# TencentARC/BlobCtrl

Measured on AMD Instinct MI355X. Metric: 512x512_50step_blobctrl_edits_per_sec, higher is better.
Workload: dtype fp16

## Files before the change

### blobctrl_amd/_lib.py

```python
import ctypes as C
import os

_HERE = os.path.dirname(os.path.abspath(__file__))
LIB_PATH = os.environ.get("BLOBCTRL_HIP_LIB") or os.path.join(_HERE, "libblobctrl_hip.so")

A_DENSE, A_CONV3X3 = 0, 1
ACT_NONE, ACT_GELU, ACT_GEGLU, ACT_SILU, ACT_QUICK_GELU = 0, 1, 2, 3, 4
OUT_F16, OUT_F16_T, OUT_F32 = 0, 1, 2
TILE_NAMES = ["auto", "256x128", "128x128_s3", "128x128_s2", "256x64_s2", "256x64_s3", "128x64", "64x64", "halo128x160", "wreg128x160",
              "gw64x128", "gw64x256", "gw64x320", "g256x256"]
TILE_HALO = 8
TILE_WREG = 9
TILE_GW64x128, TILE_GW64x256, TILE_GW64x320 = 10, 11, 12
TILE_G256 = 13
GW_TILES = {TILE_GW64x128: 2, TILE_GW64x256: 4, TILE_GW64x320: 5}


class BcGemm(C.Structure):
    _fields_ = [
        ("A", C.c_void_p), ("A2", C.c_void_p), ("a_mode", C.c_int),
        ("M", C.c_int), ("N", C.c_int), ("K", C.c_int),
        ("lda", C.c_int), ("lda2", C.c_int), ("C1", C.c_int), ("Cin", C.c_int),
        ("Hin", C.c_int), ("Win", C.c_int), ("Hv", C.c_int), ("Wv", C.c_int),
        ("Hout", C.c_int), ("Wout", C.c_int), ("stride", C.c_int), ("conv_nopad_lo", C.c_int),
        ("W", C.c_void_p), ("ldw", C.c_int),
        ("bias", C.c_void_p), ("rowvec", C.c_void_p), ("ld_rowvec", C.c_int), ("rows_per_batch", C.c_int),
        ("rowvec_idx", C.c_void_p), ("rowvec_step", C.c_int),
        ("act", C.c_int), ("colscale", C.c_void_p), ("alpha", C.c_float),
        ("alpha_dev", C.c_void_p), ("alpha_idx", C.c_void_p), ("alpha_bstride", C.c_int),
        ("R", C.c_void_p), ("ldr", C.c_int),
        ("R2", C.c_void_p), ("ldr2", C.c_int), ("r2_xmin", C.c_int), ("r2_bmod", C.c_int), ("out_w", C.c_int),
        ("out_mode", C.c_int), ("C", C.c_void_p), ("ldc", C.c_int),
        ("splitk", C.c_int), ("slab", C.c_void_p), ("gn_tot", C.c_void_p), ("tile_cfg", C.c_int),
        ("a_affine", C.c_void_p), ("a_act", C.c_int),
        ("a_tot1", C.c_void_p), ("a_tot2", C.c_void_p),
        ("a_gamma", C.c_void_p), ("a_beta", C.c_void_p), ("a_groups", C.c_int), ("a_eps", C.c_float),
        ("ln_colsum", C.c_void_p), ("ln_eps", C.c_float),
        ("C_t", C.c_void_p), ("ldc_t", C.c_int), ("n_t0", C.c_int),
        ("w_bstride", C.c_longlong), ("vec_bstride", C.c_int), ("sm_group", C.c_int), ("sm_valid", C.c_int), ("sm_keep", C.c_int),
        ("S", C.c_void_p), ("S2", C.c_void_p), ("lds", C.c_int), ("lds2", C.c_int), ("S1", C.c_int), ("Cs", C.c_int),
    ]


_SIGNATURES = {
    "bc_last_error": (C.c_char_p, []),
    "bc_version": (C.c_int, []),
    "bc_device_info": (C.c_int, [C.POINTER(C.c_int)]),
    "bc_gemm": (C.c_int, [C.POINTER(BcGemm), C.c_void_p]),
    "bc_sizeof_gemm": (C.c_int, []),
    "bc_gemm_plan": (C.c_int, [C.c_int, C.c_int, C.c_int, C.c_int, C.POINTER(C.c_int), C.POINTER(C.c_int),
                               C.POINTER(C.c_int), C.POINTER(C.c_int)]),
    "bc_conv_halo_eligible": (C.c_int, [C.c_int] * 8),
    "bc_conv_halo_max_chunks": (C.c_int, []),
    "bc_conv_wreg_pack": (C.c_int, [C.c_void_p, C.c_int, C.c_int, C.c_void_p, C.c_void_p]),
    "bc_conv_wreg_pack_sc": (C.c_int, [C.c_void_p, C.c_int, C.c_int, C.c_void_p, C.c_int, C.c_void_p, C.c_void_p]),
    "bc_conv_wreg_sc_eligible": (C.c_int, [C.c_int] * 7),
    "bc_conv_wreg_pack_host": (C.c_int, [C.c_void_p, C.c_int, C.c_int, C.c_void_p, C.c_int, C.c_void_p]),
    "bc_gemm_wreg_pack": (C.c_int, [C.c_void_p, C.c_int, C.c_int, C.c_int, C.c_int, C.c_void_p, C.c_void_p]),
    "bc_gemm_wreg_stream_elems": (C.c_longlong, [C.c_int, C.c_int]),
    "bc_gemm_wreg_eligible": (C.c_int, [C.c_int] * 5),
    "bc_gemm256_eligible": (C.c_int, [C.c_int] * 7),
    "bc_gn_stats": (C.c_int, [C.c_void_p, C.c_int, C.c_int, C.c_int, C.c_void_p, C.c_void_p]),
    "bc_gn_finalize": (C.c_int, [C.c_void_p, C.c_int, C.c_void_p, C.c_int, C.c_int, C.c_int, C.c_int,
                                 C.c_float, C.c_void_p, C.c_void_p, C.c_void_p, C.c_void_p]),
    "bc_gn_apply_fused": (C.c_int, [C.c_void_p, C.c_int, C.c_void_p, C.c_int, C.c_void_p, C.c_void_p,
                                    C.c_int, C.c_int, C.c_int, C.c_float, C.c_void_p, C.c_void_p, C.c_int, C.c_void_p,
                                    C.c_void_p]),
    "bc_memset_zero": (C.c_int, [C.c_void_p, C.c_longlong, C.c_void_p]),
    "bc_dup_halves": (C.c_int, [C.c_void_p, C.c_longlong] * 6 + [C.c_void_p]),
    "bc_gn_apply": (C.c_int, [C.c_void_p, C.c_int, C.c_void_p, C.c_int, C.c_int, C.c_int, C.c_void_p, C.c_int,
                              C.c_void_p, C.c_void_p]),
    "bc_softmax_rows": (C.c_int, [C.c_void_p, C.c_int, C.c_int, C.c_int, C.c_void_p]),
    "bc_gaussian_sample": (C.c_int, [C.c_void_p, C.c_void_p, C.c_int, C.c_int, C.c_int, C.c_float, C.c_void_p, C.c_void_p]),
    "bc_layernorm": (C.c_int, [C.c_void_p, C.c_int, C.c_int, C.c_int, C.c_void_p, C.c_void_p, C.c_float, C.c_void_p,
                               C.c_int, C.c_void_p]),
    "bc_attention": (C.c_int, [C.c_void_p, C.c_void_p, C.c_void_p, C.c_void_p, C.c_int, C.c_int, C.c_int, C.c_int,
                               C.c_int, C.c_int, C.c_int, C.c_int, C.c_int, C.c_longlong, C.c_longlong, C.c_longlong,
                               C.c_longlong, C.c_float, C.c_void_p]),
    "bc_attention_causal": (C.c_int, [C.c_void_p, C.c_void_p, C.c_void_p, C.c_void_p, C.c_int, C.c_int, C.c_int, C.c_int,
                                      C.c_int, C.c_int, C.c_int, C.c_int, C.c_int, C.c_longlong, C.c_longlong, C.c_longlong,
                                      C.c_longlong, C.c_float, C.c_void_p]),
    "bc_embed_tokens": (C.c_int, [C.c_void_p, C.c_void_p, C.c_void_p, C.c_int, C.c_int, C.c_int, C.c_int, C.c_void_p,
                                  C.c_void_p]),
    "bc_splat_scores": (C.c_int, [C.POINTER(C.c_double), C.c_int, C.c_int, C.c_int, C.c_void_p, C.c_void_p]),
    "bc_splat_maps": (C.c_int, [C.POINTER(C.c_double), C.c_int, C.c_int, C.c_int, C.c_void_p, C.c_void_p, C.c_void_p]),
    "bc_alpha_composite": (C.c_int, [C.c_void_p, C.c_longlong, C.c_int, C.c_void_p, C.c_void_p]),
    "bc_splat_from_scores": (C.c_int, [C.c_void_p, C.c_void_p, C.c_int, C.c_int, C.c_int, C.c_int, C.c_int, C.c_longlong, C.c_longlong,
                                       C.c_longlong, C.c_longlong, C.c_int, C.c_int, C.c_int, C.c_void_p, C.c_void_p]),
    "bc_resize_bilinear": (C.c_int, [C.c_void_p, C.c_longlong, C.c_int, C.c_int, C.c_int, C.c_int, C.c_int, C.c_void_p, C.c_void_p]),
    "bc_pack_rgb8": (C.c_int, [C.c_void_p, C.c_int, C.c_int, C.c_void_p, C.c_void_p]),
    "bc_assemble_input": (C.c_int, [C.c_void_p, C.c_int, C.c_void_p, C.c_void_p, C.c_void_p, C.c_int, C.c_int, C.c_int,
                                    C.c_int, C.c_int, C.c_int, C.c_int, C.c_void_p, C.c_void_p]),
    "bc_assemble_input_im2col": (C.c_int, [C.c_void_p, C.c_int, C.c_void_p, C.c_void_p, C.c_int, C.c_int, C.c_int, C.c_int, C.c_int,
                                           C.c_void_p, C.c_void_p]),
    "bc_timestep_embedding": (C.c_int, [C.c_void_p, C.c_void_p, C.c_float, C.c_int, C.c_int, C.c_void_p, C.c_void_p]),
    "bc_timestep_embedding_table": (C.c_int, [C.c_void_p, C.c_int, C.c_int, C.c_int, C.c_void_p, C.c_void_p]),
    "bc_silu": (C.c_int, [C.c_void_p, C.c_void_p, C.c_longlong, C.c_void_p]),
    "bc_cfg_scheduler_step": (C.c_int, [C.c_void_p, C.c_void_p, C.c_void_p, C.c_void_p, C.c_void_p, C.c_float, C.c_int,
                                        C.c_int, C.c_int, C.c_void_p, C.c_int, C.c_void_p]),
    "bc_cfg_scheduler_step_noise": (C.c_int, [C.c_void_p, C.c_void_p, C.c_void_p, C.c_void_p, C.c_void_p, C.c_float, C.c_int,
                                              C.c_int, C.c_int, C.c_void_p, C.c_int, C.c_void_p, C.c_int, C.c_void_p]),
    "bc_cfg_scheduler_step3": (C.c_int, [C.c_void_p, C.c_void_p, C.c_void_p, C.c_void_p, C.c_void_p, C.c_float, C.c_int, C.c_int,
                                         C.c_int, C.c_int, C.c_void_p, C.c_int, C.c_void_p]),
    "bc_nchw_to_nhwc_f16": (C.c_int, [C.c_void_p, C.c_int, C.c_int, C.c_int, C.c_int, C.c_int, C.c_void_p, C.c_void_p]),
    "bc_nhwc_to_nchw": (C.c_int, [C.c_void_p, C.c_int, C.c_int, C.c_int, C.c_int, C.c_void_p, C.c_int, C.c_void_p]),
    "bc_add_cls_pos": (C.c_int, [C.c_void_p, C.c_void_p, C.c_void_p, C.c_int, C.c_int, C.c_int, C.c_void_p, C.c_void_p]),
    "bc_patchify": (C.c_int, [C.c_void_p, C.c_int, C.c_int, C.c_int, C.c_int, C.c_int, C.c_void_p, C.c_void_p]),
    "bc_rowchain_supported": (C.c_int, [C.c_int, C.c_int, C.c_int]),
    "bc_rowchain_stream_frags": (C.c_longlong, [C.c_int, C.c_int, C.c_int, C.c_int]),
    "bc_rowchain": (C.c_int, [C.c_int, C.c_int, C.c_int, C.c_int, C.c_void_p, C.c_void_p, C.c_void_p, C.c_void_p, C.c_void_p, C.c_int, C.c_float,
                              C.c_void_p, C.c_void_p, C.c_void_p, C.c_int, C.c_int,
                              C.c_int, C.c_void_p, C.c_void_p, C.c_void_p, C.c_void_p, C.c_void_p, C.c_int, C.c_void_p, C.c_float,
                              C.c_float, C.c_void_p, C.c_void_p, C.c_int, C.c_void_p, C.c_int, C.c_void_p]),
    "bc_rowchain_sum": (C.c_int, [C.c_int, C.c_int, C.c_int, C.c_void_p, C.c_int, C.c_void_p, C.c_void_p, C.c_void_p, C.c_void_p]),
    "bc_rowchain_kv_frags": (C.c_longlong, [C.c_int]),
    "bc_rowchain_pack_kv": (C.c_int, [C.c_void_p, C.c_int, C.c_void_p, C.c_int, C.c_int, C.c_int, C.c_int, C.c_void_p, C.c_void_p]),
    "bc_ctx_fold": (C.c_int, [C.c_void_p, C.c_int, C.c_void_p, C.c_int, C.c_int, C.c_int, C.c_int, C.c_int, C.c_float, C.c_void_p, C.c_void_p,
                              C.c_void_p, C.c_void_p, C.c_void_p, C.c_void_p, C.c_void_p, C.c_void_p]),
    "bc_rowchain_midx": (C.c_int, [C.c_int, C.c_int, C.c_int, C.c_void_p, C.c_void_p, C.c_void_p, C.c_void_p, C.c_void_p, C.c_int, C.c_float,
                                   C.c_void_p, C.c_void_p, C.c_float, C.c_void_p]),
    "bc_plan_create": (C.c_int, [C.POINTER(C.c_void_p)]),
    "bc_plan_destroy": (C.c_int, [C.c_void_p]),
    "bc_plan_segment": (C.c_int, [C.c_void_p, C.c_char_p]),
    "bc_plan_find_segment": (C.c_int, [C.c_void_p, C.c_char_p]),
    "bc_plan_new_event": (C.c_int, [C.c_void_p]),
    "bc_plan_add_gemm": (C.c_int, [C.c_void_p, C.c_int, C.c_int, C.POINTER(BcGemm)]),
    "bc_plan_add_op": (C.c_int, [C.c_void_p, C.c_int, C.c_int, C.c_int, C.POINTER(C.c_uint64), C.c_int]),
    "bc_plan_set_slab": (C.c_int, [C.c_void_p, C.c_int, C.c_void_p]),
    "bc_plan_enable": (C.c_int, [C.c_void_p, C.c_int, C.c_int, C.c_int]),
    "bc_plan_num_launches": (C.c_int, [C.c_void_p, C.c_int]),
    "bc_step": (C.c_int, [C.c_void_p, C.c_int, C.POINTER(C.c_void_p), C.c_int]),
    "bc_plan_capture": (C.c_int, [C.c_void_p, C.c_int, C.POINTER(C.c_void_p), C.c_int]),
    "bc_plan_release": (C.c_int, [C.c_void_p, C.c_int]),
    "bc_plan_capture_loop": (C.c_int, [C.c_void_p, C.POINTER(C.c_int), C.c_int, C.POINTER(C.c_void_p), C.c_int, C.POINTER(C.c_void_p)]),
    "bc_plan_run_timed": (C.c_int, [C.c_void_p, C.c_int, C.c_void_p, C.POINTER(C.c_float)]),
    "bc_plan_run_timed_kernels": (C.c_int, [C.c_void_p, C.c_int, C.c_void_p, C.POINTER(C.c_float), C.POINTER(C.c_float)]),
    "bc_plan_run_marked": (C.c_int, [C.c_void_p, C.c_int, C.POINTER(C.c_void_p), C.c_int, C.POINTER(C.c_int), C.c_int, C.POINTER(C.c_float)]),
    "bc_plan_save": (C.c_int, [C.c_void_p, C.c_char_p, C.c_void_p, C.c_int]),
    "bc_plan_load": (C.c_int, [C.c_char_p, C.POINTER(C.c_void_p)]),
    "bc_plan_buffer": (C.c_int, [C.c_void_p, C.c_char_p, C.POINTER(C.c_void_p), C.POINTER(C.c_longlong)]),
    "bc_graph_begin": (C.c_int, [C.c_void_p]),
    "bc_graph_end": (C.c_int, [C.c_void_p, C.POINTER(C.c_void_p)]),
    "bc_graph_launch": (C.c_int, [C.c_void_p, C.c_void_p]),
    "bc_graph_destroy": (C.c_int, [C.c_void_p]),
    "bc_event_create": (C.c_int, [C.POINTER(C.c_void_p)]),
    "bc_event_create_sync": (C.c_int, [C.POINTER(C.c_void_p)]),
    "bc_stream_wait_event": (C.c_int, [C.c_void_p, C.c_void_p]),
    "bc_event_record": (C.c_int, [C.c_void_p, C.c_void_p]),
    "bc_event_elapsed_ms": (C.c_int, [C.c_void_p, C.c_void_p, C.POINTER(C.c_float)]),
    "bc_event_destroy": (C.c_int, [C.c_void_p]),
}

EXPORTED_SYMBOLS = tuple(_SIGNATURES.keys())

OPS = {"bc_gemm": 0, "bc_gn_stats": 1, "bc_gn_finalize": 2, "bc_gn_apply_fused": 3, "bc_gn_apply": 4, "bc_layernorm": 5,
       "bc_attention": 6, "bc_attention_causal": 7, "bc_assemble_input": 8, "bc_timestep_embedding": 9,
       "bc_timestep_embedding_table": 10, "bc_cfg_scheduler_step": 11, "bc_embed_tokens": 12, "bc_softmax_rows": 13,
       "bc_patchify": 14, "bc_add_cls_pos": 15, "bc_silu": 16, "bc_nchw_to_nhwc_f16": 17, "bc_nhwc_to_nchw": 18,
       "bc_gaussian_sample": 19, "bc_rowchain": 22, "bc_assemble_input_im2col": 23, "bc_memset_zero": 24,
       "bc_rowchain_midx": 25, "bc_rowchain_pack_kv": 26, "bc_rowchain_sum": 27, "bc_ctx_fold": 28, "bc_dup_halves": 29,
       "bc_cfg_scheduler_step_noise": 30, "bc_cfg_scheduler_step3": 31}
OP_SIGNAL, OP_WAIT = 20, 21
CHAIN_IN, CHAIN_MID, CHAIN_OUT, CHAIN_OUT_FF, CHAIN_OUT_TAIL, CHAIN_MIDX, CHAIN_OUT_FFP = 0, 1, 2, 3, 4, 5, 6
GN_TOT_WORDS = 6
_KIND = {C.c_void_p: "p", C.c_int: "i", C.c_float: "f", C.c_longlong: "l", C.c_char_p: "p"}


def op_signature(name):
    args = _SIGNATURES[name][1][:-1]
    return "".join("p" if (a not in _KIND) else _KIND[a] for a in args)


class BcPlanBuffer(C.Structure):
    _fields_ = [("name", C.c_char_p), ("address", C.c_void_p), ("bytes", C.c_longlong), ("host_data", C.c_void_p)]

_lib = None


class BlobCtrlHipError(RuntimeError):
    pass


def load():
    global _lib
    if _lib is not None:
        return _lib
    if not os.path.exists(LIB_PATH):
        raise BlobCtrlHipError(
            f"{LIB_PATH} not found: build it with `python -c 'import __graft_entry__ as g; g.build()'` "
            "(hipcc --offload-arch=gfx950).  blobctrl_amd has no CPU fallback.")
    try:
        import torch
    except ImportError:
        pass
    try:
        lib = C.CDLL(LIB_PATH)
    except OSError as e:
        raise BlobCtrlHipError(f"failed to load {LIB_PATH}: {e}") from e
    for name, (res, args) in _SIGNATURES.items():
        fn = getattr(lib, name)
        fn.restype = res
        fn.argtypes = args
    if lib.bc_sizeof_gemm() != C.sizeof(BcGemm):
        raise BlobCtrlHipError(f"BcGemm layout mismatch: C {lib.bc_sizeof_gemm()} vs ctypes {C.sizeof(BcGemm)}")
    _lib = lib
    return lib


def check(rc, what=""):
    if rc != 0:
        msg = load().bc_last_error()
        raise BlobCtrlHipError(f"{what} failed (rc={rc}): {msg.decode() if msg else ''}")
```

### blobctrl_amd/csrc/conv_wreg.hip

```cpp
#include <stdio.h>
#include <stdlib.h>
#include <algorithm>
#include <type_traits>
#include <vector>
#include "gemm_common.h"

using namespace bcg;

namespace {

__device__ __attribute__((aligned(16))) unsigned int g_zero_line_w[4] = {0u, 0u, 0u, 0u};

typedef const __attribute__((address_space(1))) void* gptr_t;
typedef __attribute__((address_space(3))) void* lptr_t;

__device__ __forceinline__ void glds16(const void* src, char* lds_dst) {
    __builtin_amdgcn_global_load_lds((gptr_t)src, (lptr_t)lds_dst, 16, 0, 0);
}

constexpr int TW = 16, TH = 8;
constexpr int HBM = TW * TH;
constexpr int HBN = 160;
constexpr int HSTR = TW + 2;
constexpr int HPIX = (TH + 2) * HSTR;
constexpr int HALO_BYTES = 24 * 1024;
constexpr int NBUF = 3;
constexpr int OFF_AB = NBUF * HALO_BYTES;
constexpr int MAX_CH = 40;
constexpr int TS = HBN + 4;
constexpr int LDS_LOOP = OFF_AB + MAX_CH * 512;
constexpr int LDS_EPI = 8 * 16384;
constexpr int OFF_EPI = LDS_LOOP > LDS_EPI ? LDS_LOOP : LDS_EPI;
constexpr int LDS_TOTAL = OFF_EPI + 2 * HBN * 4;
static_assert(LDS_TOTAL <= 160 * 1024 && HPIX * 128 <= HALO_BYTES && HBM * TS * 4 <= LDS_EPI, "LDS budget");
constexpr int FIN_MAX_CH = 2752;
constexpr int OFF_FIN = LDS_LOOP;
constexpr int LDS_TOTAL_FIN = OFF_FIN + FIN_MAX_CH * 16 + 1024 > LDS_TOTAL ? OFF_FIN + FIN_MAX_CH * 16 + 1024 : LDS_TOTAL;
static_assert(LDS_TOTAL_FIN <= 160 * 1024, "LDS budget (in-kernel finalize)");

template <int N>
__device__ __forceinline__ void wait_vm_c() { asm volatile("s_waitcnt vmcnt(%0)" ::"n"(N) : "memory"); }
typedef float f32x4v __attribute__((ext_vector_type(4)));
typedef unsigned int u32x4v __attribute__((ext_vector_type(4)));

template <int V> using IC = std::integral_constant<int, V>;

template <int AFFINE>
__global__ __launch_bounds__(512) void conv_wreg_kernel(const GemmArgs g) {
    extern __shared__ __attribute__((aligned(16))) char smem[];
    const BcGemm& p = g.p;
    const int tid = threadIdx.x;
    const int lane = tid & 63;
    const int wave = __builtin_amdgcn_readfirstlane(tid >> 6);
    const int kg = wave & 1;
    const int grp = ((wave >> 1) & 1) | ((wave >> 2) << 1);
    const bool three = grp == 0 || grp == 3;
    const int tile0 = grp == 0 ? 0 : grp == 1 ? 3 : grp == 2 ? 5 : 7;

    asm volatile("" ::"s"(p.A), "s"(p.A2), "s"(p.W), "s"(p.Hv), "s"(p.Wv), "s"(p.Hin), "s"(p.Win), "s"(p.lda), "s"(p.lda2), "s"(p.C1), "s"(p.Cin),
                 "s"(p.splitk), "s"(p.a_act), "s"(g.halo_tpi), "s"(g.halo_tx), "s"(g.halo_nch), "s"(g.halo_nsc), "s"(g.halo_cps), "s"(g.halo_cps_sc), "s"(g.nband), "s"(g.halo_stamps));
    asm volatile("" ::"s"(g.wr_plane.mul), "s"(g.wr_plane.shift), "s"(g.wr_plane.d), "s"(g.wr_gx.mul), "s"(g.wr_gx.shift), "s"(g.wr_gx.d), "s"(g.wr_gy.mul),
                 "s"(g.wr_gy.shift), "s"(g.wr_gy.d), "s"(g.wr_tpi.mul), "s"(g.wr_tpi.shift), "s"(g.wr_tx.mul), "s"(g.wr_tx.shift), "s"(p.bias), "s"(p.rowvec),
                 "s"(p.rowvec_idx), "s"(p.rowvec_step), "s"(p.ld_rowvec), "s"(g.halo_dbg), "s"(g.div_rpb.d));
    if (AFFINE == 2)
        asm volatile("" ::"s"(p.a_tot1), "s"(p.a_tot2), "s"(p.a_gamma), "s"(p.a_beta), "s"(p.a_groups), "s"(p.a_eps), "s"(g.wr_cpg.mul), "s"(g.wr_cpg.shift));
    const int plane = (int)g.wr_plane.d;
    const int lin3 = bc_xcd_remap(blockIdx.x + gridDim.x * (blockIdx.y + gridDim.y * blockIdx.z), plane * gridDim.z);
    const int split = (int)fdiv((unsigned)lin3, g.wr_plane);
    const int lin = lin3 - split * plane;
    const int q_gx = (int)fdiv((unsigned)lin, g.wr_gx), q_gy = (int)fdiv((unsigned)lin, g.wr_gy);
    const int tile = g.nband ? lin - q_gy * (int)g.wr_gy.d : q_gx;
    const int ntile = g.nband ? q_gy : lin - q_gx * (int)g.wr_gx.d;
    const int n0 = ntile * HBN;
    const int b = (int)fdiv((unsigned)tile, g.wr_tpi);
    const int tin = tile - b * g.halo_tpi;
    const int ty_ = (int)fdiv((unsigned)tin, g.wr_tx);
    const int ty0 = ty_ * TH, tx0 = (tin - ty_ * g.halo_tx) * TW;
    const int H = p.Hv, W = p.Wv;
    const bool ups2 = p.Hv != p.Hin;
    const int c_lo = split * g.halo_cps;
    const int n9 = max(0, min(g.halo_nch, c_lo + g.halo_cps) - c_lo);
    const int sc_begin = split * g.halo_cps_sc;
    const int nsc = max(0, min(g.halo_nsc, sc_begin + g.halo_cps_sc) - sc_begin);
    const bool dummy = n9 == 0;
    const int c_begin = dummy ? 0 : c_lo;
    const int nch = dummy ? 1 : n9;
    const long long tsl = (long long)(9 * g.halo_nch + g.halo_nsc) * 512;

    unsigned long long* const stamps = g.halo_stamps;
    auto stamp = [&](int i) {
        if (stamps && lane == 0 && (wave == 0 || wave == 2))
            stamps[((size_t)(blockIdx.x + gridDim.x * (blockIdx.y + gridDim.y * blockIdx.z)) * 2 + (wave >> 1)) * 16 + i] = __builtin_amdgcn_s_memtime();
    };
    stamp(0);

    const h16* __restrict__ A1 = reinterpret_cast<const h16*>(p.A);
    const h16* __restrict__ A2 = reinterpret_cast<const h16*>(p.A2);
    const h16* zero = reinterpret_cast<const h16*>(g_zero_line_w);

    const int sidx = ((wave >= 2 ? wave - 2 : 0) << 6) | lane;
    int pixv[6], csubv[6];
#pragma unroll
    for (int q = 0; q < 6; ++q) {
        const int hp = (sidx >> 3) + 32 * q;
        const int hy = hp / HSTR, hx = hp - hy * HSTR;
        const int gy = ty0 + hy - 1, gx = tx0 + hx - 1;
        const bool inh = hp < HPIX;
        const bool in_img = inh && (unsigned)gy < (unsigned)H && (unsigned)gx < (unsigned)W;
        pixv[q] = !in_img ? -1 : ups2 ? (b * p.Hin + (gy >> 1)) * p.Win + (gx >> 1) : (b * H + gy) * W + gx;
        csubv[q] = (sidx & 7) ^ (((hx >> 1) & 3) << 1);
    }
    auto issue_a = [&](int cl, int buf, bool valid) {
        const int k0 = (c_begin + cl) * 64;
        const bool second = A2 != nullptr && k0 >= p.C1;
        const h16* src = second ? A2 : A1;
        const int stride = second ? p.lda2 : p.lda;
        const int kin = second ? k0 - p.C1 : k0;
        char* dst = smem + buf * HALO_BYTES + (wave - 2) * 1024;
#pragma unroll
        for (int q = 0; q < 6; ++q) {
            const int off = pixv[q] * stride + kin + csubv[q] * 8;
            const h16* s = (valid && !dummy && pixv[q] >= 0) ? src + off : zero;
            glds16(s, dst + q * 4096);
        }
    };
    const unsigned lds0 = (unsigned)(size_t)(lptr_t)(smem);
    const unsigned slot_addr = lds0 + sidx * 16;
    const unsigned ab_base = lds0 + OFF_AB;
    struct Pending { u32x4v raw; f32x4v t0, t1, t2, t3; };
    auto tr_issue = [&](unsigned sa, unsigned ab_addr, Pending& pd) {
        asm volatile("ds_read_b128 %0, %1" : "=v"(pd.raw) : "v"(sa) : "memory");
        asm volatile("ds_read_b128 %0, %4\n\tds_read_b128 %1, %4 offset:16\n\tds_read_b128 %2, %4 offset:32\n\t"
                     "ds_read_b128 %3, %4 offset:48"
                     : "=&v"(pd.t0), "=&v"(pd.t1), "=&v"(pd.t2), "=&v"(pd.t3) : "v"(ab_addr) : "memory");
    };
    auto tr_finish = [&](unsigned sa, bool outside, bool store, Pending& pd) {
        asm volatile("s_waitcnt lgkmcnt(0)" : "+v"(pd.raw), "+v"(pd.t0), "+v"(pd.t1), "+v"(pd.t2), "+v"(pd.t3)::"memory");
        __builtin_amdgcn_sched_barrier(0);
        const float aa[8] = {pd.t0[0], pd.t0[2], pd.t1[0], pd.t1[2], pd.t2[0], pd.t2[2], pd.t3[0], pd.t3[2]};
        const float bb[8] = {pd.t0[1], pd.t0[3], pd.t1[1], pd.t1[3], pd.t2[1], pd.t2[3], pd.t3[1], pd.t3[3]};
        const u32x4v rawv = pd.raw;
        const h16* xin = reinterpret_cast<const h16*>(&rawv);
        u32x4v outraw;
        h16* o = reinterpret_cast<h16*>(&outraw);
#pragma unroll
        for (int j = 0; j < 8; ++j) {
            float v = fmaf((float)xin[j], aa[j], bb[j]);
            if (p.a_act == BC_ACT_SILU) v = v * __builtin_amdgcn_rcpf(1.0f + __builtin_amdgcn_exp2f(-1.4426950408889634f * v));
            o[j] = (h16)v;
        }
        if (outside || dummy) outraw = (u32x4v){0u, 0u, 0u, 0u};
        if (store) asm volatile("ds_write_b128 %0, %1" ::"v"(sa), "v"(outraw) : "memory");
    };
    unsigned tinfo = 0;
#pragma unroll
    for (int q = 0; q < 3; ++q) {
        const int hp = (tid >> 3) + 64 * q;
        const int hy = hp / HSTR, hx = hp - hy * HSTR;
        const int gy = ty0 + hy - 1, gx = tx0 + hx - 1;
        const unsigned inh = hp < HPIX, outside = !((unsigned)gy < (unsigned)H && (unsigned)gx < (unsigned)W);
        tinfo |= (inh | outside << 1 | (unsigned)((tid & 7) ^ (((hx >> 1) & 3) << 1)) << 2) << (8 * q);
    }
    const unsigned tslot = lds0 + tid * 16;
    auto transform_pair = [&](auto kxc, int cl, int buf) {
        constexpr int q0 = 2 * decltype(kxc)::value;
        Pending pa, pb;
        const unsigned sa = slot_addr + buf * HALO_BYTES + 4096 * q0, ab = ab_base + cl * 512;
        const bool in0 = (sidx >> 3) + 32 * q0 < HPIX, in1 = (sidx >> 3) + 32 * (q0 + 1) < HPIX;
        tr_issue(sa, ab + csubv[q0] * 64, pa);
        tr_issue(sa + 4096, ab + csubv[q0 + 1] * 64, pb);
        tr_finish(sa, pixv[q0] < 0, in0, pa);
        tr_finish(sa + 4096, pixv[q0 + 1] < 0, in1, pb);
        asm volatile("s_waitcnt lgkmcnt(0)" ::: "memory");
    };
    auto transform_first = [&]() {
        Pending pd[3];
#pragma unroll
        for (int q = 0; q < 3; ++q) tr_issue(tslot + 8192 * q, ab_base + ((tinfo >> (8 * q + 2)) & 7) * 64, pd[q]);
#pragma unroll
        for (int q = 0; q < 3; ++q) tr_finish(tslot + 8192 * q, (tinfo >> (8 * q + 1)) & 1, (tinfo >> (8 * q)) & 1, pd[q]);
        asm volatile("s_waitcnt lgkmcnt(0)" ::: "memory");
    };

    float* tilef = reinterpret_cast<float*>(smem);
    auto body = [&](auto ntc, auto stgc) {
        constexpr int NT = decltype(ntc)::value;
        constexpr bool STG = decltype(stgc)::value != 0;
        constexpr int G = 3 * NT;
        const long long per_chunk = 9 * 512;
        u32x4v ring[3 * G];
        const unsigned lane16 = lane * 16;
#define BC_WREG_LOAD_GROUP(GX, BASE)                                                                                                  \
    _Pragma("unroll") for (int f = 0; f < G; ++f) {                                                                                   \
        const h16* b4 = (BASE) + (((GX) * G + f) & ~3) * 512;                                                                          \
        asm volatile("global_load_dwordx4 %0, %1, %2 offset:%3" : "=v"(ring[(GX) * G + f]) : "v"(lane16), "s"(b4), "n"((((GX) * G + f) & 3) * 1024) : "memory"); \
    }
        const h16* const wstream = reinterpret_cast<const h16*>(p.W) + ((long long)ntile * 20 + 2 * tile0 + kg * NT) * tsl;
        const h16* wb = wstream + (long long)c_begin * NT * per_chunk;
        constexpr int FIN_T = 4;
        const int fin_cpg = AFFINE == 2 ? p.Cin / p.a_groups : 1;
        const int fin_k_lo = c_begin * 64, fin_k_hi = fin_k_lo + nch * 64;
        const int fin_g_lo = (int)fdiv((unsigned)fin_k_lo, g.wr_cpg), fin_g_hi = AFFINE == 2 ? min(p.a_groups, (int)fdiv((unsigned)(fin_k_hi + fin_cpg - 1), g.wr_cpg)) : 1;
        const int fin_c_lo = fin_g_lo * fin_cpg, fin_nc = fin_g_hi * fin_cpg - fin_c_lo;
        const bool fin_fast = AFFINE == 2 && fin_nc <= 256 * FIN_T && !(g.halo_dbg & 0x100);
        const int ft = ((wave < 2 ? wave : wave - 4) << 6) | lane;
        u32x4v fq[FIN_T][3];
        float fg[FIN_T], fb[FIN_T];
        if (AFFINE == 2 && !STG && fin_fast) {
            unsigned long long tp1 = (unsigned long long)p.a_tot1, tp2 = (unsigned long long)(p.A2 ? p.a_tot2 : p.a_tot1);
            asm volatile("" : "+s"(tp1), "+s"(tp2));
            const int C1s = p.A2 ? p.C1 : p.Cin, C2s = p.Cin - C1s;
#pragma unroll
            for (int j = 0; j < FIN_T; ++j) {
                const int cc = ft + 256 * j;
                const int c = fin_c_lo + (cc < fin_nc ? cc : 0);
                const bool second = c >= C1s;
                const unsigned long long ta = (second ? tp2 : tp1) + ((unsigned long long)((long long)b * (second ? C2s : C1s) + (second ? c - C1s : c))) * (BC_GN_TOT_WORDS * 8);
                const unsigned long long* t = reinterpret_cast<const unsigned long long*>(ta);
                asm volatile("global_load_dwordx4 %0, %3, off\n\tglobal_load_dwordx4 %1, %3, off offset:16\n\tglobal_load_dwordx4 %2, %3, off offset:32"
                             : "=&v"(fq[j][0]), "=&v"(fq[j][1]), "=&v"(fq[j][2]) : "v"(t) : "memory");
                const int i = ft + 256 * j;
                const int ci = fin_k_lo + (i < nch * 64 ? i : 0);
                asm volatile("global_load_dword %0, %2, off\n\tglobal_load_dword %1, %3, off" : "=&v"(fg[j]), "=&v"(fb[j]) : "v"(p.a_gamma + ci), "v"(p.a_beta + ci) : "memory");
            }
        }
        stamp(8);
        if (STG) {
            issue_a(0, 0, true);
            issue_a(1, 1, nch > 1);
        }
        BC_WREG_LOAD_GROUP(0, wb)
        stamp(9);
        if (AFFINE == 2 && fin_fast && !STG) {
#define BC_FIN_TIE(j) "+v"(fq[j][0]), "+v"(fq[j][1]), "+v"(fq[j][2])
            asm volatile("s_waitcnt vmcnt(%12)" : BC_FIN_TIE(0), BC_FIN_TIE(1), BC_FIN_TIE(2), BC_FIN_TIE(3) : "n"(G) : "memory");
            asm volatile("s_waitcnt vmcnt(%8)" : "+v"(fg[0]), "+v"(fg[1]), "+v"(fg[2]), "+v"(fg[3]), "+v"(fb[0]), "+v"(fb[1]), "+v"(fb[2]), "+v"(fb[3])
                         : "n"(G) : "memory");
#undef BC_FIN_TIE
        }
        stamp(10);
        unsigned rv_idx = 0;
        if (p.rowvec && p.rowvec_idx) asm volatile("s_load_dword %0, %1, 0x0\n\ts_waitcnt lgkmcnt(0)" : "=s"(rv_idx) : "s"(p.rowvec_idx) : "memory");
        const bool eok = p.splitk == 1 && tid < HBN;
        const float* epi_bp = (eok && p.bias) ? p.bias + n0 + tid : reinterpret_cast<const float*>(g_zero_line_w);
        const h16* epi_rp = (eok && p.rowvec) ? reinterpret_cast<const h16*>(p.rowvec) + (size_t)rv_idx * p.rowvec_step + (size_t)b * p.ld_rowvec + n0 + tid : zero;
        const float epi_bv = *epi_bp;
        const unsigned short epi_rraw = *reinterpret_cast<const unsigned short*>(epi_rp);
        if (AFFINE == 2 && fin_fast) {
            double* scr = reinterpret_cast<double*>(smem + OFF_FIN);
            float* stat = reinterpret_cast<float*>(scr + fin_nc * 2);
            if (!STG) {
#pragma unroll
                for (int j = 0; j < FIN_T; ++j) {
                    const int cc = ft + 256 * j;
                    if (cc < fin_nc) {
                        double s_, q_;
                        auto w64 = [](unsigned lo, unsigned hi) { return (unsigned long long)lo | ((unsigned long long)hi << 32); };
                        bc_gn_tot_decode(w64(fq[j][0][0], fq[j][0][1]), w64(fq[j][0][2], fq[j][0][3]), w64(fq[j][1][0], fq[j][1][1]),
                                         w64(fq[j][1][2], fq[j][1][3]), w64(fq[j][2][0], fq[j][2][1]), w64(fq[j][2][2], fq[j][2][3]), s_, q_);
                        scr[cc * 2] = s_;
                        scr[cc * 2 + 1] = q_;
                    }
                }
            }
            asm volatile("s_waitcnt lgkmcnt(0)" ::: "memory");
            __builtin_amdgcn_s_barrier();
            asm volatile("" ::: "memory");
            stamp(11);
            if (!STG) {
                const int sub = ft & 7;
                for (int gi = fin_g_lo + (ft >> 3); gi < fin_g_hi; gi += 32) {
                    double s_ = 0.0, q_ = 0.0;
                    for (int cj = sub; cj < fin_cpg; cj += 8) {
                        s_ += scr[((gi - fin_g_lo) * fin_cpg + cj) * 2];
                        q_ += scr[((gi - fin_g_lo) * fin_cpg + cj) * 2 + 1];
                    }
#pragma unroll
                    for (int o = 4; o > 0; o >>= 1) {
                        s_ += __shfl_xor(s_, o);
                        q_ += __shfl_xor(q_, o);
                    }
                    const double n = (double)g.div_rpb.d * fin_cpg;
                    const double mean = s_ / n;
                    double var = q_ / n - mean * mean;
                    if (var < 0.0) var = 0.0;
                    if (sub == 0) {
                        stat[(gi - fin_g_lo) * 2] = (float)mean;
                        stat[(gi - fin_g_lo) * 2 + 1] = (float)(1.0 / sqrt(var + (double)p.a_eps));
                    }
                }
            }
            asm volatile("s_waitcnt lgkmcnt(0)" ::: "memory");
            __builtin_amdgcn_s_barrier();
            asm volatile("" ::: "memory");
            stamp(12);
            if (!STG) {
                float* abt = reinterpret_cast<float*>(smem + OFF_AB);
#pragma unroll
                for (int j = 0; j < FIN_T; ++j) {
                    const int i = ft + 256 * j;
                    if (i < nch * 64) {
                        const int gi = (int)fdiv((unsigned)(fin_k_lo + i), g.wr_cpg) - fin_g_lo;
                        const float a = stat[gi * 2 + 1] * fg[j];
                        abt[i * 2] = a;
                        abt[i * 2 + 1] = fb[j] - stat[gi * 2] * a;
                    }
                }
            }
            stamp(13);
        } else if (AFFINE == 2) {
            const int cpg = p.Cin / p.a_groups;
            const int k_lo = c_begin * 64, k_hi = k_lo + nch * 64;
            const int g_lo = k_lo / cpg, g_hi = min(p.a_groups, (k_hi + cpg - 1) / cpg);
            const int c_lo = g_lo * cpg, nc = g_hi * cpg - c_lo;
            float gpre[2] = {0.f, 0.f}, bpre[2] = {0.f, 0.f};
#pragma unroll
            for (int j = 0; j < 2; ++j)
                if (tid + 512 * j < nch * 64) {
                    gpre[j] = p.a_gamma[k_lo + tid + 512 * j];
                    bpre[j] = p.a_beta[k_lo + tid + 512 * j];
                }
            double* scr = reinterpret_cast<double*>(smem + OFF_FIN);
            for (int cc = tid; cc < nc; cc += 512) {
                const int c = c_lo + cc;
                const bool second = p.A2 != nullptr && c >= p.C1;
                const int Cs = second ? p.Cin - p.C1 : (p.A2 ? p.C1 : p.Cin);
                const unsigned long long* t = (second ? p.a_tot2 : p.a_tot1) + ((size_t)b * Cs + (second ? c - p.C1 : c)) * BC_GN_TOT_WORDS;
                double s, q;
                bc_gn_tot_read(t, s, q);
                scr[cc * 2] = s;
                scr[cc * 2 + 1] = q;
            }
            __syncthreads();
            float* stat = reinterpret_cast<float*>(scr + nc * 2);
            {
                const int sub = tid & 7;
                for (int gi = g_lo + (tid >> 3); gi < g_hi; gi += 64) {
                    double s = 0.0, q = 0.0;
                    for (int cj = sub; cj < cpg; cj += 8) {
                        s += scr[((gi - g_lo) * cpg + cj) * 2];
                        q += scr[((gi - g_lo) * cpg + cj) * 2 + 1];
                    }
#pragma unroll
                    for (int o = 4; o > 0; o >>= 1) {
                        s += __shfl_xor(s, o);
                        q += __shfl_xor(q, o);
                    }
                    const double n = (double)g.div_rpb.d * cpg;
                    const double mean = s / n;
                    double var = q / n - mean * mean;
                    if (var < 0.0) var = 0.0;
                    if (sub == 0) {
                        stat[(gi - g_lo) * 2] = (float)mean;
                        stat[(gi - g_lo) * 2 + 1] = (float)(1.0 / sqrt(var + (double)p.a_eps));
                    }
                }
            }
            __syncthreads();
            float* abt = reinterpret_cast<float*>(smem + OFF_AB);
#pragma unroll
            for (int j = 0; j < 2; ++j) {
                const int i = tid + 512 * j;
                if (i < nch * 64) {
                    const int gi = (k_lo + i) / cpg - g_lo;
                    const float a = stat[gi * 2 + 1] * gpre[j];
                    abt[i * 2] = a;
                    abt[i * 2 + 1] = bpre[j] - stat[gi * 2] * a;
                }
            }
            for (int i = tid + 1024; i < nch * 64; i += 512) {
                const int c = k_lo + i;
                const int gi = c / cpg - g_lo;
                const float a = stat[gi * 2 + 1] * p.a_gamma[c];
                abt[i * 2] = a;
                abt[i * 2 + 1] = p.a_beta[c] - stat[gi * 2] * a;
            }
            __syncthreads();
        }
        if (AFFINE == 1) {
            const float4* src = reinterpret_cast<const float4*>(p.a_affine + ((size_t)b * p.Cin + (size_t)c_begin * 64) * 2);
            float4* dst = reinterpret_cast<float4*>(smem + OFF_AB);
            for (int i = tid; i < nch * 32; i += 512) dst[i] = src[i];
        }
        BC_WREG_LOAD_GROUP(1, wb)
        BC_WREG_LOAD_GROUP(2, wb)
        stamp(1);
        asm volatile("s_waitcnt vmcnt(%0)" ::"n"(2 * G) : "memory");
        asm volatile("s_waitcnt lgkmcnt(0)" ::: "memory");
        __builtin_amdgcn_s_barrier();
        asm volatile("" ::: "memory");
        stamp(6);
        if (AFFINE) transform_first();
        if (eok) {
            float* ev = reinterpret_cast<float*>(smem + OFF_EPI);
            ev[tid] = epi_bv;
            ev[HBN + tid] = (float)__builtin_bit_cast(h16, epi_rraw);
        }
        stamp(7);
        asm volatile("s_waitcnt lgkmcnt(0)" ::: "memory");
        __builtin_amdgcn_s_barrier();
        asm volatile("" ::: "memory");
        stamp(2);

        int a_off[3];
#pragma unroll
        for (int kx = 0; kx < 3; ++kx) {
            const int hx = (lane & 15) + kx;
            const int ch = 4 * kg + (lane >> 4);
            a_off[kx] = hx * 128 + ((ch ^ (((hx >> 1) & 3) << 1)) << 4);
        }
        f32x4v acc[8][NT];
#pragma unroll
        for (int i = 0; i < 8; ++i)
#pragma unroll
            for (int t = 0; t < NT; ++t) acc[i][t] = (f32x4v){0.f, 0.f, 0.f, 0.f};

#ifndef BC_WREG_PRIO
#define BC_WREG_PRIO 1
#endif
        if ((BC_WREG_PRIO == 1 && STG) || (BC_WREG_PRIO == 2 && !STG)) __builtin_amdgcn_s_setprio(3);
        int buf = 0;
        int cl = 0;
#pragma unroll
        for (int pass = 0; pass < 2; ++pass) {
        const bool more = pass == 0;
        const int cl_end = more ? nch - 1 : nch;
        for (; cl < cl_end; ++cl) {
            const int buf1 = buf + 1 == NBUF ? 0 : buf + 1;
            const int buf2 = buf1 + 1 == NBUF ? 0 : buf1 + 1;
            if (STG) issue_a(cl + 2, buf2, cl + 2 < nch);
            wb += 3 * G * 512;
#pragma unroll
            for (int kx = 0; kx < 3; ++kx) {
#define BC_WREG_WAIT(N)                                                                                                                 \
    if (NT == 3) asm volatile("s_waitcnt vmcnt(%9)" : "+v"(ring[kx * G]), "+v"(ring[kx * G + 1]), "+v"(ring[kx * G + 2]), "+v"(ring[kx * G + 3]), \
                              "+v"(ring[kx * G + 4]), "+v"(ring[kx * G + 5]), "+v"(ring[kx * G + 6]), "+v"(ring[kx * G + 7]),             \
                              "+v"(ring[kx * G + G - 1]) : "n"(N) : "memory");                                                          \
    else asm volatile("s_waitcnt vmcnt(%6)" : "+v"(ring[kx * G]), "+v"(ring[kx * G + 1]), "+v"(ring[kx * G + 2]), "+v"(ring[kx * G + 3]),       \
                      "+v"(ring[kx * G + 4]), "+v"(ring[kx * G + G - 1]) : "n"(N) : "memory");
                constexpr int D = STG ? 6 : 0;
                if (more || kx == 0) { BC_WREG_WAIT(2 * G + D) }
                else if (kx == 1) { BC_WREG_WAIT(G + D) }
                else { BC_WREG_WAIT(D) }
                const unsigned abase = lds0 + buf * HALO_BYTES + a_off[kx];
                u32x4v a[3];
                asm volatile("ds_read_b128 %0, %1" : "=v"(a[0]) : "v"(abase) : "memory");
                asm volatile("ds_read_b128 %0, %1 offset:%2" : "=v"(a[1]) : "v"(abase), "n"(HSTR * 128) : "memory");
#pragma unroll
                for (int r = 0; r < 10; ++r) {
                    if (r + 2 < 10) {
                        asm volatile("ds_read_b128 %0, %1 offset:%2" : "=v"(a[(r + 2) % 3]) : "v"(abase), "n"((r + 2) * HSTR * 128) : "memory");
                        asm volatile("s_waitcnt lgkmcnt(2)" : "+v"(a[r % 3])::"memory");
                    } else if (r + 1 < 10) {
                        asm volatile("s_waitcnt lgkmcnt(1)" : "+v"(a[r % 3])::"memory");
                    } else {
                        asm volatile("s_waitcnt lgkmcnt(0)" : "+v"(a[r % 3])::"memory");
                    }
                    __builtin_amdgcn_sched_barrier(0);
                    const h16x8 af = __builtin_bit_cast(h16x8, a[r % 3]);
#pragma unroll
                    for (int ky = 0; ky < 3; ++ky) {
                        const int i = r - ky;
                        if (i < 0 || i >= 8) continue;
#pragma unroll
                        for (int t = 0; t < NT; ++t)
                            acc[i][t] = __builtin_amdgcn_mfma_f32_16x16x32_f16(__builtin_bit_cast(h16x8, ring[(kx * 3 + ky) * NT + t]), af, acc[i][t], 0, 0, 0);
                    }
                    __builtin_amdgcn_sched_barrier(0);
                }
                if (STG && AFFINE && more) {
                    if (kx == 0) transform_pair(IC<0>{}, cl + 1, buf1);
                    else if (kx == 1) transform_pair(IC<1>{}, cl + 1, buf1);
                    else transform_pair(IC<2>{}, cl + 1, buf1);
                }
                if (more) { BC_WREG_LOAD_GROUP(kx, wb) }
                __builtin_amdgcn_sched_barrier(0);
            }
            if (STG) {
                if (more) wait_vm_c<3 * G>();
                else wait_vm_c<0>();
            }
            asm volatile("s_waitcnt lgkmcnt(0)" ::: "memory");
            __builtin_amdgcn_s_barrier();
            asm volatile("" ::: "memory");
            buf = buf1;
        }
        }

        stamp(14);
        if (nsc > 0) {
            constexpr int U = 4, NB2 = 5, D1 = STG ? 6 : 0;
            static_assert(NB2 * HALO_BYTES <= LDS_EPI && U < NB2 && U * 3 + 6 * U < 64, "shortcut phase: images below the epilogue vectors, vmcnt range");
            const h16* __restrict__ S1p = reinterpret_cast<const h16*>(p.S);
            const h16* __restrict__ S2p = reinterpret_cast<const h16*>(p.S2);
            const h16* const ws = wstream + ((long long)g.halo_nch * 9 + sc_begin) * NT * 512;
            u32x4v sr[U * NT];
            auto issue_s = [&](int sx, int bufi) {
                const int k0 = (sc_begin + sx) * 64;
                const bool second = S2p != nullptr && k0 >= p.S1;
                const h16* src = second ? S2p : S1p;
                const int stride = second ? p.lds2 : p.lds;
                const int kin = second ? k0 - p.S1 : k0;
                char* dst = smem + bufi * HALO_BYTES + (wave - 2) * 1024;
#pragma unroll
                for (int q = 0; q < 6; ++q) {
                    const int off = pixv[q] * stride + kin + csubv[q] * 8;
                    const h16* s_ = (sx < nsc && pixv[q] >= 0) ? src + off : zero;
                    glds16(s_, dst + q * 4096);
                }
            };
#define BC_WREG_LOAD_SC(J, SX)                                                                                                          \
    {                                                                                                                                   \
        const h16* b4 = ws + (long long)min((SX), nsc - 1) * (NT * 512);                                                                \
        _Pragma("unroll") for (int t = 0; t < NT; ++t)                                                                                  \
            asm volatile("global_load_dwordx4 %0, %1, %2 offset:%3" : "=v"(sr[(J) * NT + t]) : "v"(lane16), "s"(b4), "n"((t % NT) * 1024) : "memory"); \
    }
#pragma unroll
            for (int j = 0; j < U; ++j) {
                if (STG) issue_s(j, j);
                BC_WREG_LOAD_SC(j, j)
            }
            if (STG) wait_vm_c<U * NT + 6 * (U - 1)>();
            asm volatile("s_waitcnt lgkmcnt(0)" ::: "memory");
            __builtin_amdgcn_s_barrier();
            asm volatile("" ::: "memory");
            int sbuf = 0;
            for (int s0 = 0; s0 < nsc; s0 += U) {
#pragma unroll
                for (int j = 0; j < U; ++j) {
                    const int sx = s0 + j;
                    const int bufn = sbuf + U >= NB2 ? sbuf + U - NB2 : sbuf + U;
                    if (STG) issue_s(sx + U, bufn);
                    if (NT == 3) asm volatile("s_waitcnt vmcnt(%3)" : "+v"(sr[j * NT]), "+v"(sr[j * NT + 1]), "+v"(sr[j * NT + NT - 1]) : "n"((U - 1) * NT + U * D1) : "memory");
                    else asm volatile("s_waitcnt vmcnt(%2)" : "+v"(sr[j * NT]), "+v"(sr[j * NT + 1]) : "n"((U - 1) * NT + U * D1) : "memory");
                    const unsigned abase = lds0 + sbuf * HALO_BYTES + a_off[1];
                    u32x4v a8[8];
#pragma unroll
                    for (int i = 0; i < 8; ++i)
                        asm volatile("ds_read_b128 %0, %1 offset:%2" : "=v"(a8[i]) : "v"(abase), "n"((i + 1) * HSTR * 128) : "memory");
#pragma unroll
                    for (int i = 0; i < 8; ++i) {
                        asm volatile("s_waitcnt lgkmcnt(%1)" : "+v"(a8[i]) : "n"(7 - i) : "memory");
                        __builtin_amdgcn_sched_barrier(0);
                        const h16x8 af = __builtin_bit_cast(h16x8, a8[i]);
#pragma unroll
                        for (int t = 0; t < NT; ++t)
                            acc[i][t] = __builtin_amdgcn_mfma_f32_16x16x32_f16(__builtin_bit_cast(h16x8, sr[j * NT + t]), af, acc[i][t], 0, 0, 0);
                        __builtin_amdgcn_sched_barrier(0);
                    }
                    BC_WREG_LOAD_SC(j, sx + U)
                    if (STG) wait_vm_c<U * NT + 6 * (U - 1)>();
                    asm volatile("s_waitcnt lgkmcnt(0)" ::: "memory");
                    __builtin_amdgcn_s_barrier();
                    asm volatile("" ::: "memory");
                    sbuf = sbuf + 1 == NB2 ? 0 : sbuf + 1;
                }
            }
#pragma unroll
            for (int j = 0; j < U; ++j) {
                if (NT == 3) asm volatile("s_waitcnt vmcnt(0)" : "+v"(sr[j * NT]), "+v"(sr[j * NT + 1]), "+v"(sr[j * NT + NT - 1]) :: "memory");
                else asm volatile("s_waitcnt vmcnt(0)" : "+v"(sr[j * NT]), "+v"(sr[j * NT + 1]) :: "memory");
            }
            __builtin_amdgcn_s_barrier();
            asm volatile("" ::: "memory");
#undef BC_WREG_LOAD_SC
        }
        __builtin_amdgcn_s_setprio(0);
        stamp(3);
        char* xch = smem + tile0 * 8192;
        const int i_keep = kg * 4, i_send = 4 - i_keep;
#pragma unroll
        for (int ii = 0; ii < 4; ++ii)
#pragma unroll
            for (int t = 0; t < NT; ++t)
                *reinterpret_cast<f32x4v*>(xch + (((i_send + ii) * NT + t) * 64 + lane) * 16) = kg ? acc[ii][t] : acc[4 + ii][t];
        __syncthreads();
        f32x4v fin[4][NT];
#pragma unroll
        for (int ii = 0; ii < 4; ++ii)
#pragma unroll
            for (int t = 0; t < NT; ++t) {
                const f32x4v o = *reinterpret_cast<const f32x4v*>(xch + (((i_keep + ii) * NT + t) * 64 + lane) * 16);
                fin[ii][t] = (kg ? acc[4 + ii][t] : acc[ii][t]) + o;
            }
        __syncthreads();
        if (p.splitk > 1) {
#pragma unroll
            for (int ii = 0; ii < 4; ++ii)
#pragma unroll
                for (int t = 0; t < NT; ++t)
                    *reinterpret_cast<f32x4v*>(tilef + ((i_keep + ii) * 16 + (lane & 15)) * TS + tile0 * 16 + t * 16 + 4 * (lane >> 4)) = fin[ii][t];
            __syncthreads();
            return;
        }
        constexpr int RPP = NT == 3 ? 8 : 16, NP = 64 / RPP;
        char* const sl = smem + wave * 16384;
#pragma unroll
        for (int ii = 0; ii < 4; ++ii)
#pragma unroll
            for (int t = 0; t < NT; ++t) {
                const int row = ii * 16 + (lane & 15), ck = t * 4 + (lane >> 4);
                *reinterpret_cast<f32x4v*>(sl + row * 256 + ((ck ^ (row & 15)) << 4)) = fin[ii][t];
            }
        int cpos, rsub;
        bool lane_on = true;
        if (NT == 3) {
            cpos = lane & 7;
            rsub = lane >> 3;
            lane_on = cpos < 6;
            if (!lane_on) cpos = 5;
        } else {
            const int sub = (lane >> 2) & 3;
            cpos = lane & 3;
            rsub = 2 * (lane >> 4) + (sub & 1) + 8 * (sub >> 1);
        }
        const int ch0 = tile0 * 16 + cpos * 8, n_first = n0 + ch0;
        const int rpb = (int)g.div_rpb.d;
        const float alpha = scalar_alpha(p);
        const float* ev = reinterpret_cast<const float*>(smem + OFF_EPI) + ch0;
        float bias_v[8], rvec[8], cs[8];
#pragma unroll
        for (int j = 0; j < 8; ++j) {
            bias_v[j] = ev[j];
            rvec[j] = ev[HBN + j];
            cs[j] = (p.colscale ? p.colscale[n_first + j] : 1.0f) * alpha;
        }
        const float ab = p.alpha_bstride > 0 ? batch_alpha(g, b) : 1.0f;
        float gs[8], gq[8];
#pragma unroll
        for (int j = 0; j < 8; ++j) { gs[j] = 0.f; gq[j] = 0.f; }
        auto passes = [&](auto H2K, auto HRK) {
            constexpr bool H2 = decltype(H2K)::value, HR = decltype(HRK)::value;
            uint4 rr[NP];
            int mrow[NP];
#pragma unroll
            for (int j = 0; j < NP; ++j) {
                const int row = j * RPP + rsub;
                mrow[j] = b * rpb + (ty0 + i_keep + (row >> 4)) * W + tx0 + (row & 15);
                if (HR) rr[j] = bc_ld16(reinterpret_cast<const h16*>(p.R) + (size_t)mrow[j] * p.ldr + n_first);
            }
            if (!H2) __builtin_amdgcn_sched_barrier(0);
#pragma unroll H2 ? 1 : NP
            for (int j = 0; j < NP; ++j) {
                const int row = j * RPP + rsub;
                const f32x4v lo = *reinterpret_cast<const f32x4v*>(sl + row * 256 + (((2 * cpos) ^ (row & 15)) << 4));
                const f32x4v hi = *reinterpret_cast<const f32x4v*>(sl + row * 256 + (((2 * cpos + 1) ^ (row & 15)) << 4));
                float v[8] = {lo[0], lo[1], lo[2], lo[3], hi[0], hi[1], hi[2], hi[3]};
#pragma unroll
                for (int q = 0; q < 8; ++q) v[q] += bias_v[q];
                if (p.rowvec) {
#pragma unroll
                    for (int q = 0; q < 8; ++q) v[q] += rvec[q];
                }
                if (H2) {
                    if (p.act == BC_ACT_GELU) {
#pragma unroll
                        for (int q = 0; q < 8; ++q) v[q] = bc_gelu_f(v[q]);
                    } else if (p.act == BC_ACT_SILU) {
#pragma unroll
                        for (int q = 0; q < 8; ++q) v[q] = bc_silu_f(v[q]);
                    } else if (p.act == BC_ACT_QUICK_GELU) {
#pragma unroll
                        for (int q = 0; q < 8; ++q) v[q] = bc_quick_gelu_f(v[q]);
                    }
                }
#pragma unroll
                for (int q = 0; q < 8; ++q) v[q] *= cs[q];
                if (p.alpha_bstride > 0) {
#pragma unroll
                    for (int q = 0; q < 8; ++q) v[q] *= ab;
                }
                if (HR) {
                    const h16* rh = reinterpret_cast<const h16*>(&rr[j]);
#pragma unroll
                    for (int q = 0; q < 8; ++q) v[q] += (float)rh[q];
                }
                if (H2 && p.R) {
                    const uint4 r1 = bc_ld16(reinterpret_cast<const h16*>(p.R) + (size_t)mrow[j] * p.ldr + n_first);
                    const h16* rh = reinterpret_cast<const h16*>(&r1);
#pragma unroll
                    for (int q = 0; q < 8; ++q) v[q] += (float)rh[q];
                }
                if (H2 && p.R2) {
                    const int pix = mrow[j] - b * rpb;
                    const int x = pix - (int)fdiv((unsigned)pix, g.div_outw) * (int)g.div_outw.d;
                    if (x >= p.r2_xmin) {
                        const uint4 r2 = bc_ld16(reinterpret_cast<const h16*>(p.R2) + ((size_t)(b % p.r2_bmod) * rpb + pix) * p.ldr2 + n_first);
                        const h16* rh = reinterpret_cast<const h16*>(&r2);
#pragma unroll
                        for (int q = 0; q < 8; ++q) v[q] += (float)rh[q];
                    }
                }
                uint4 outraw;
                h16* o = reinterpret_cast<h16*>(&outraw);
#pragma unroll
                for (int q = 0; q < 8; ++q) {
                    o[q] = (h16)v[q];
                    const float f = lane_on ? (float)o[q] : 0.f;
                    gs[q] += f;
                    gq[q] += f * f;
                }
                bc_st16(reinterpret_cast<h16*>(p.C) + (size_t)mrow[j] * p.ldc + n_first, outraw);
            }
        };
        if (p.R2 || p.act != BC_ACT_NONE) passes(std::true_type{}, std::false_type{});
        else if (p.R) passes(std::false_type{}, std::true_type{});
        else passes(std::false_type{}, std::false_type{});
        if (p.gn_tot) {
            constexpr int X0 = NT == 3 ? 8 : 4, X1 = 2 * X0, X2 = 4 * X0;
            const bool b0 = lane & X0, b1 = lane & X1, b2 = lane & X2;
            auto scatter = [&](const float (&v)[8]) __attribute__((always_inline)) {
                float k4[4], k2[2];
#pragma unroll
                for (int k = 0; k < 4; ++k) k4[k] = (b0 ? v[4 + k] : v[k]) + __shfl_xor(b0 ? v[k] : v[4 + k], X0);
#pragma unroll
                for (int k = 0; k < 2; ++k) k2[k] = (b1 ? k4[2 + k] : k4[k]) + __shfl_xor(b1 ? k4[k] : k4[2 + k], X1);
                float t = (b2 ? k2[1] : k2[0]) + __shfl_xor(b2 ? k2[0] : k2[1], X2);
                if (NT == 2) t += __shfl_xor(t, 32);
                return t;
            };
            const float s_own = scatter(gs), q2_own = scatter(gq);
            const int q_own = (b0 ? 4 : 0) + (b1 ? 2 : 0) + (b2 ? 1 : 0);
            const bool owner = NT == 3 ? lane_on : lane < 32;
            float* sc = reinterpret_cast<float*>(smem + wave * 16384);
            if (owner) {
                sc[(cpos * 8 + q_own) * 2] = s_own;
                sc[(cpos * 8 + q_own) * 2 + 1] = q2_own;
            }
            __syncthreads();
            if (kg == 0 && owner) {
                const float* sp = reinterpret_cast<const float*>(smem + (wave | 1) * 16384);
                const int n_lo = n0 + tile0 * 16;
                bc_gn_tot_add_slot(p.gn_tot + (size_t)b * g.n_out * BC_GN_TOT_WORDS, n_first + q_own, n_lo, n_lo + NT * 16, bc_gn_cg(g.n_out), tin, [&](int k) {
                    const int c = k - n_lo;
                    return make_float2(sc[c * 2] + sp[c * 2], sc[c * 2 + 1] + sp[c * 2 + 1]);
                });
            }
        }
    };
    if (three) body(IC<3>{}, IC<0>{});
    else body(IC<2>{}, IC<1>{});
    stamp(4);
    if (p.splitk > 1) {
        const int col8 = tid % 20, row0 = tid / 20;
        const int rpb = (int)g.div_rpb.d;
        if (tid < 480) {
            float* slab = p.slab + (size_t)split * p.M * p.N;
            for (int row = row0; row < HBM; row += 24) {
                const int m = b * rpb + (ty0 + (row >> 4)) * W + tx0 + (row & 15);
                const float4 lo = *reinterpret_cast<const float4*>(tilef + row * TS + col8 * 8);
                const float4 hi = *reinterpret_cast<const float4*>(tilef + row * TS + col8 * 8 + 4);
                float* dst = slab + (size_t)m * p.N + n0 + col8 * 8;
                *reinterpret_cast<float4*>(dst) = lo;
                *reinterpret_cast<float4*>(dst + 4) = hi;
            }
        }
    }
    stamp(5);
}

__host__ __device__ inline long long conv_wreg_pack_src(long long idx, int Cin, int Cs, bool& sc) {
    const int nchunks = Cin / 64;
    const long long per_tile_stream = (long long)(nchunks * 9 + Cs / 64) * 64;
    const long long per_ntile = 20 * per_tile_stream;
    const int ntile = (int)(idx / per_ntile);
    long long rem = idx - (long long)ntile * per_ntile;
    const int ts = (int)(rem / per_tile_stream);
    int tile0, NT;
    if (ts < 6) { tile0 = 0; NT = 3; }
    else if (ts < 10) { tile0 = 3; NT = 2; }
    else if (ts < 14) { tile0 = 5; NT = 2; }
    else { tile0 = 7; NT = 3; }
    const long long in_grp = rem - (long long)2 * tile0 * per_tile_stream;
    const long long per_wave = per_tile_stream * NT;
    const int kg = (int)(in_grp / per_wave);
    long long s = in_grp - (long long)kg * per_wave;
    const int lane = (int)(s & 63);
    s >>= 6;
    sc = s >= (long long)nchunks * 9 * NT;
    if (sc) {
        s -= (long long)nchunks * 9 * NT;
        const int t = (int)(s % NT), chunk = (int)(s / NT);
        const int n = ntile * HBN + (tile0 + t) * 16 + (lane & 15);
        return (long long)n * Cs + chunk * 64 + kg * 32 + 8 * (lane >> 4);
    }
    const int t = (int)(s % NT);
    s /= NT;
    const int ky = (int)(s % 3);
    s /= 3;
    const int kx = (int)(s % 3);
    const int chunk = (int)(s / 3);
    const int n = ntile * HBN + (tile0 + t) * 16 + (lane & 15);
    const long long k = (long long)(ky * 3 + kx) * Cin + chunk * 64 + kg * 32 + 8 * (lane >> 4);
    return (long long)n * 9 * Cin + k;
}

__global__ void conv_wreg_pack_kernel(const h16* __restrict__ w, int N, int Cin, const h16* __restrict__ wsc, int Cs, h16* __restrict__ out) {
    const long long total = (long long)N * (9 * Cin + Cs) / 8;
    const long long idx = (long long)blockIdx.x * blockDim.x + threadIdx.x;
    if (idx >= total) return;
    bool sc;
    const long long src = conv_wreg_pack_src(idx, Cin, Cs, sc);
    *reinterpret_cast<uint4*>(out + idx * 8) = *reinterpret_cast<const uint4*>((sc ? wsc : w) + src);
}

}

extern "C" int bc_conv_wreg_pack_sc(const bc_half* w, int N, int Cin, const bc_half* wsc, int Cs, bc_half* out, bc_stream stream_) {
    hipStream_t stream = reinterpret_cast<hipStream_t>(stream_);
    BC_CHECK_ARG(w && out && N > 0 && N % HBN == 0 && Cin > 0 && Cin % 64 == 0, "bc_conv_wreg_pack: N %% 160 == 0 and Cin %% 64 == 0 (N=%d Cin=%d)", N, Cin);
    BC_CHECK_ARG((wsc == nullptr) == (Cs == 0) && Cs >= 0 && Cs % 64 == 0, "bc_conv_wreg_pack: shortcut weight and Cs %% 64 == 0 go together (Cs=%d)", Cs);
    BC_CHECK_ARG(((uintptr_t)w % 16 == 0) && ((uintptr_t)wsc % 16 == 0) && ((uintptr_t)out % 16 == 0) && w != out && wsc != out,
                 "bc_conv_wreg_pack: 16-byte aligned, out of place");
    const long long total = (long long)N * (9 * Cin + Cs) / 8;
    hipLaunchKernelGGL(conv_wreg_pack_kernel, dim3((unsigned)((total + 255) / 256)), dim3(256), 0, stream, reinterpret_cast<const h16*>(w), N, Cin,
                       reinterpret_cast<const h16*>(wsc), Cs, reinterpret_cast<h16*>(out));
    BC_CHECK_LAUNCH();
    return 0;
}

extern "C" int bc_conv_wreg_pack_host(const bc_half* w, int N, int Cin, const bc_half* wsc, int Cs, bc_half* out) {
    BC_CHECK_ARG(w && out && N > 0 && N % HBN == 0 && Cin > 0 && Cin % 64 == 0, "bc_conv_wreg_pack: N %% 160 == 0 and Cin %% 64 == 0 (N=%d Cin=%d)", N, Cin);
    BC_CHECK_ARG((wsc == nullptr) == (Cs == 0) && Cs >= 0 && Cs % 64 == 0, "bc_conv_wreg_pack: shortcut weight and Cs %% 64 == 0 go together (Cs=%d)", Cs);
    const long long total = (long long)N * (9 * Cin + Cs) / 8;
    const unsigned short* w_ = reinterpret_cast<const unsigned short*>(w);
    const unsigned short* s_ = reinterpret_cast<const unsigned short*>(wsc);
    unsigned short* o_ = reinterpret_cast<unsigned short*>(out);
    for (long long idx = 0; idx < total; ++idx) {
        bool sc;
        const long long src = conv_wreg_pack_src(idx, Cin, Cs, sc);
        std::copy_n((sc ? s_ : w_) + src, 8, o_ + idx * 8);
    }
    return 0;
}

extern "C" int bc_conv_wreg_pack(const bc_half* w, int N, int Cin, bc_half* out, bc_stream stream) {
    return bc_conv_wreg_pack_sc(w, N, Cin, nullptr, 0, out, stream);
}

int bc_conv_wreg_sc_ok(const BcGemm& p) {
    if (!p.S || p.R || p.Cs <= 0 || p.Cs % 64 != 0 || p.Hv != p.Hin || p.Wv != p.Win) return 0;
    if (p.S2 && (p.S1 <= 0 || p.S1 >= p.Cs || p.S1 % 64 != 0)) return 0;
    if (p.lds < (p.S2 ? p.S1 : p.Cs) || p.lds % 8 != 0 || (uintptr_t)p.S % 16 != 0) return 0;
    if (p.S2 && (p.lds2 < p.Cs - p.S1 || p.lds2 % 8 != 0 || (uintptr_t)p.S2 % 16 != 0)) return 0;
    return 1;
}

int bc_conv_wreg_launch(GemmArgs& g, hipStream_t stream) {
    BcGemm& p = g.p;
    g.halo_tx = p.Wout / TW;
    g.halo_tpi = g.halo_tx * (p.Hout / TH);
    g.halo_nch = p.Cin / 64;
    g.halo_nsc = p.S ? p.Cs / 64 : 0;
    g.halo_dbg = 0;
    g.halo_stamps = nullptr;
    int sk = std::max(1, std::min(p.splitk, g.halo_nch + g.halo_nsc));
    g.halo_cps = bc_ceil_div(g.halo_nch, sk);
    g.halo_cps_sc = bc_ceil_div(g.halo_nsc, sk);
    p.splitk = std::max(bc_ceil_div(g.halo_nch, g.halo_cps), g.halo_nsc ? bc_ceil_div(g.halo_nsc, g.halo_cps_sc) : 1);
    BC_CHECK_ARG(g.halo_cps <= MAX_CH, "bc_gemm(wreg conv): %d channel chunks per split exceed %d (raise splitk)", g.halo_cps, MAX_CH);
    BC_CHECK_ARG(p.splitk == 1 || p.slab != nullptr, "bc_gemm(wreg conv): splitk=%d needs a slab", p.splitk);
    const int B = p.M / (p.Hout * p.Wout);
    BC_CHECK_ARG((long long)p.M * std::max(p.lda, p.lda2) < 2147483647LL, "bc_gemm(wreg conv): activation of %d pixels x stride %d exceeds 32-bit element offsets",
                 p.M, std::max(p.lda, p.lda2));
    BC_CHECK_ARG(!p.S || (bc_conv_wreg_sc_ok(p) && (long long)p.M * std::max(p.lds, p.lds2) < 2147483647LL),
                 "bc_gemm(wreg conv): folded shortcut outside the kernel's limits (Cs=%d S1=%d)", p.Cs, p.S1);
    dim3 grid(p.N / HBN, B * g.halo_tpi, p.splitk);
    g.wr_plane = make_fastdiv(grid.x * grid.y);
    g.wr_gx = make_fastdiv(grid.x);
    g.wr_gy = make_fastdiv(grid.y);
    g.wr_tpi = make_fastdiv((unsigned)g.halo_tpi);
    g.wr_tx = make_fastdiv((unsigned)g.halo_tx);
    g.wr_cpg = make_fastdiv((unsigned)(p.a_tot1 && p.a_groups > 0 ? p.Cin / p.a_groups : 1));
    {
        g.nband = (double)p.N * 9 > (double)p.M && grid.x >= 4;
    }
    static const bool want_stamps = getenv("BC_WREG_STAMPS") != nullptr;
    static unsigned long long* stamp_buf = nullptr;
    const size_t nwg_s = (size_t)grid.x * grid.y * grid.z;
    if (want_stamps && nwg_s <= 4096) {
        if (!stamp_buf) BC_CHECK_HIP(hipMalloc(reinterpret_cast<void**>(&stamp_buf), 4096 * 32 * sizeof(unsigned long long)));
        BC_CHECK_HIP(hipMemsetAsync(stamp_buf, 0, nwg_s * 32 * sizeof(unsigned long long), stream));
        g.halo_stamps = stamp_buf;
    }
    struct StampReport {
        hipStream_t stream; size_t n; unsigned long long* buf; const BcGemm& p; int cps;
        ~StampReport() {
            if (!buf) return;
            if (hipStreamSynchronize(stream) != hipSuccess) return;
            std::vector<unsigned long long> h(n * 32);
            if (hipMemcpy(h.data(), buf, n * 32 * sizeof(unsigned long long), hipMemcpyDeviceToHost) != hipSuccess) return;
            for (int w = 0; w < 2; ++w) {
                double d[5] = {0, 0, 0, 0, 0};
                for (size_t i = 0; i < n; ++i)
                    for (int k = 0; k < 5; ++k) d[k] += (double)(h[(i * 2 + w) * 16 + k + 1] - h[(i * 2 + w) * 16 + k]);
                double e[3] = {0, 0, 0};
                for (size_t i = 0; i < n; ++i) {
                    const unsigned long long* q = &h[(i * 2 + w) * 16];
                    e[0] += (double)(q[6] - q[1]);
                    e[1] += (double)(q[7] - q[6]);
                    e[2] += (double)(q[2] - q[7]);
                }
                double pr[6] = {0, 0, 0, 0, 0, 0};
                for (size_t i = 0; i < n; ++i)
                    for (int k = 0; k < 6; ++k) {
                        const unsigned long long* q = &h[(i * 2 + w) * 16];
                        if (q[8 + k]) pr[k] += (double)(q[8 + k] - q[0]);
                    }
                fprintf(stderr, "[wreg stamps] prologue detail (ticks since entry): inputs requested %.0f, ring group 0 requested %.0f, totals landed %.0f, "
                        "barrier 1 %.0f, barrier 2 %.0f, table written %.0f\n", pr[0] / n, pr[1] / n, pr[2] / n, pr[3] / n, pr[4] / n, pr[5] / n);
                double scp = 0;
                for (size_t i = 0; i < n; ++i) scp += (double)(h[(i * 2 + w) * 16 + 3] - h[(i * 2 + w) * 16 + 14]);
                if (p.S) fprintf(stderr, "[wreg stamps] folded shortcut: Cs=%d, %.0f ticks per workgroup behind the nine-tap chunks (of the loop's %.0f)\n", p.Cs, scp / n, d[2] / n);
                fprintf(stderr, "[wreg stamps] M=%d N=%d Cin=%d sk=%d cps=%d wgs=%zu %s | avg ticks: setup+table %.0f, first halo %.0f (landing %.0f, pass %.0f, "
                        "next DMA + barrier %.0f), loop %.0f (%.0f per tap), k-half sum %.0f, stores %.0f\n", p.M, p.N, p.Cin, p.splitk, cps, n,
                        w ? "staging wave " : "3-tile wave  ", d[0] / n, d[1] / n, e[0] / n, e[1] / n, e[2] / n, d[2] / n, d[2] / n / (cps * 9), d[3] / n, d[4] / n);
            }
        }
    } report{stream, nwg_s, g.halo_stamps, p, g.halo_cps};
    static std::atomic<unsigned long long> set_a{0}, set_p{0}, set_f{0};
    if (p.a_tot1) {
        BC_CHECK_ARG(p.a_gamma && p.a_beta && p.a_groups > 0 && p.Cin % p.a_groups == 0 && (!p.A2 || p.a_tot2),
                     "bc_gemm(wreg conv): in-kernel GroupNorm finalize needs a_gamma, a_beta, a_groups | Cin and the partials of every source");
        const int cpg = p.Cin / p.a_groups;
        BC_CHECK_ARG(g.halo_cps * 64 + 2 * cpg <= FIN_MAX_CH && p.a_groups * 8 <= 1024,
                     "bc_gemm(wreg conv): channel span %d per workgroup too wide for the in-kernel GroupNorm finalize (max %d): use "
                     "bc_gn_finalize + a_affine or raise splitk", g.halo_cps * 64 + 2 * cpg, FIN_MAX_CH);
        BC_CHECK_HIP(bc_set_max_lds(set_f, reinterpret_cast<const void*>(&conv_wreg_kernel<2>), LDS_TOTAL_FIN));
        const int lds_fin = std::max(LDS_TOTAL, OFF_FIN + (g.halo_cps * 64 + 2 * cpg) * 16 + 1024);
        hipLaunchKernelGGL((conv_wreg_kernel<2>), grid, dim3(512), lds_fin, stream, g);
    } else if (p.a_affine) {
        BC_CHECK_HIP(bc_set_max_lds(set_a, reinterpret_cast<const void*>(&conv_wreg_kernel<1>), LDS_TOTAL));
        hipLaunchKernelGGL((conv_wreg_kernel<1>), grid, dim3(512), LDS_TOTAL, stream, g);
    } else {
        BC_CHECK_HIP(bc_set_max_lds(set_p, reinterpret_cast<const void*>(&conv_wreg_kernel<0>), LDS_TOTAL));
        hipLaunchKernelGGL((conv_wreg_kernel<0>), grid, dim3(512), LDS_TOTAL, stream, g);
    }
    BC_CHECK_LAUNCH();
    return 0;
}
```

### blobctrl_amd/engine.py

```python
import os
from dataclasses import dataclass
from typing import List, Optional, Tuple

import torch

from . import _lib
from .launch import Recorder
from .options import opt
from .weights import PackedTrunk, pad8


@dataclass
class TrunkConfig:
    in_channels: int
    block_out_channels: Tuple[int, ...] = (320, 640, 1280, 1280)
    layers_per_block: int = 2
    num_heads: int = 8
    norm_num_groups: int = 32
    cross_attention_dim: Optional[int] = 768
    out_channels: int = 4
    is_blobnet: bool = False


class Act:
    __slots__ = ("t", "C", "H", "W")

    def __init__(self, t, C, H, W):
        self.t, self.C, self.H, self.W = t, C, H, W


@dataclass
class Residuals:
    down: List[torch.Tensor]
    mid: torch.Tensor
    up: List[torch.Tensor]
    bmod: int
    events: Optional[dict] = None


class TrunkPlan:

    def __init__(self, rec: Recorder, pw: PackedTrunk, cfg: TrunkConfig, B: int, H: int, W: int):
        self.rec, self.pw, self.cfg, self.B, self.H, self.W = rec, pw, cfg, B, H, W
        self.G = cfg.norm_num_groups
        self.heads = cfg.num_heads

    def _r2(self, res_t, H, W):
        if res_t is None:
            return {}
        if self.res_events is not None:
            ev = self.res_events.get(res_t.data_ptr())
            if ev is not None:
                self.rec.wait(ev)
        xmin = 0 if W == H else W - H
        return dict(R2=res_t, ldr2=res_t.shape[-1], r2_xmin=xmin, r2_bmod=self.res_bmod, out_w=W)

    def halo_ok(self, Cin, C1, Cout, H, W):
        return opt("halo") and bool(self.rec.lib.bc_conv_halo_eligible(Cin, C1, Cout, H, W, H, W, 1))

    def conv3x3(self, x: Act, wname, Cout, stride=1, up_to=None, rowvec=None, R=None, r2=None, out_f32=False,
                kind="conv3x3", out=None, x2: Optional[Act] = None, affine=None, halo=False, tile_cfg=0, sc=None):
        rec, pw = self.rec, self.pw
        Hv, Wv = up_to if up_to is not None else (x.H, x.W)
        Hout, Wout = (Hv + 2 - 3) // stride + 1, (Wv + 2 - 3) // stride + 1
        M = self.B * Hout * Wout
        if out is None:
            out = rec.empty(self.B, Hout * Wout, Cout, dtype=torch.float32 if out_f32 else torch.float16)
        kw = {}
        if rowvec is not None:
            kw.update(rowvec=rowvec[0], ld_rowvec=rowvec[1])
            if len(rowvec) == 4:
                kw.update(rowvec_idx=rowvec[2], rowvec_step=rowvec[3])
        if R is not None:
            kw.update(R=R.t, ldr=R.C)
        kw.update(self._r2(r2, Hout, Wout))
        Cin = x.C + (x2.C if x2 is not None else 0)
        wkey = wname + ".weight"
        if halo:
            wreg = opt("wreg")
            kw.update(tile_cfg=_lib.TILE_WREG if wreg else _lib.TILE_HALO, lda=x.C)
            if wreg and sc is None:
                wkey = pw.wreg(wname + ".weight")
            if sc is not None:
                assert wreg and R is None
                wkey, bkey = pw.wreg_sc(wname, sc[0])
                s1, s2 = sc[1], sc[2]
                kw.update(S=s1.t, lds=s1.C, Cs=s1.C + (s2.C if s2 is not None else 0))
                if s2 is not None:
                    kw.update(S2=s2.t, lds2=s2.C, S1=s1.C)
            if x2 is not None:
                kw.update(A2=x2.t, C1=x.C, lda2=x2.C)
            if affine is not None:
                kw.update(a_act=affine[1], **({"a_gn": affine[0]} if isinstance(affine[0], dict) else {"a_affine": affine[0]}))
        else:
            assert x2 is None and affine is None and sc is None
            ups_wreg = up_to is not None and (Hv, Wv) == (2 * x.H, 2 * x.W) and stride == 1 and Cin % 64 == 0 and Cout % 160 == 0 and \
                Wv % 16 == 0 and Hv % 8 == 0 and opt("wreg")
            if ups_wreg:
                kw.update(tile_cfg=_lib.TILE_WREG, lda=x.C)
                wkey = pw.wreg(wname + ".weight")
            elif tile_cfg:
                kw.update(tile_cfg=tile_cfg)
        rec.gemm(A=x.t, W=pw.h[wkey], M=M, N=Cout, K=9 * Cin, out=out,
                 out_mode=_lib.OUT_F32 if out_f32 else _lib.OUT_F16,
                 conv=dict(Cin=Cin, Hin=x.H, Win=x.W, Hv=Hv, Wv=Wv, Hout=Hout, Wout=Wout, stride=stride),
                 bias=pw.f[bkey if sc is not None else wname + ".bias"], rows_per_batch=Hout * Wout, kind=kind, want_gn=not out_f32, **kw)
        return Act(out, Cout, Hout, Wout)

    def g256_tile(self, M, N, K, kw):
        if not opt("g256") or kw.get("tile_cfg") or kw.get("splitk") not in (None, 1):
            return 0
        if M % 256 or N % 256 or (M // 256) * (N // 256) < opt("g256_min_tiles"):
            return 0
        want_gn = 1 if kw.get("want_gn") else 0
        c1 = kw.get("C1", 0) if kw.get("A2") is not None else 0
        if kw.get("C_t") is not None and (kw.get("n_t0", 0) % 256 or kw.get("ldc_t", 0) % 8):
            return 0
        ok = self.rec.lib.bc_gemm256_eligible(M, N, K, c1, kw.get("out_mode", _lib.OUT_F16), kw.get("rows_per_batch", 0) or M, want_gn)
        return _lib.TILE_G256 if ok else 0

    def dense(self, x_t, M, K, wname, N, bias=True, out=None, kind="linear", wkey=None, **kw):
        rec, pw = self.rec, self.pw
        act = kw.get("act", _lib.ACT_NONE)
        n_out = N // 2 if act == _lib.ACT_GEGLU else N
        if out is None:
            out = rec.empty(M, n_out)
        g256 = self.g256_tile(M, N, K, kw)
        if g256:
            kw["tile_cfg"] = g256
        rec.gemm(A=x_t, W=pw.h[wkey or (wname + ".weight")], M=M, N=N, K=K, out=out,
                 bias=pw.f[wname + ".bias"] if bias else None, kind=kind, **kw)
        return out

    def gn_conv(self, x: Act, x2: Optional[Act], norm, eps, wname, Cout, **kw):
        pw = self.pw
        C2 = x2.C if x2 is not None else 0
        if self.halo_ok(x.C + C2, C2 and x.C, Cout, x.H, x.W):
            requests = self.B if self.cfg.is_blobnet else max(1, self.B // 2)
            if opt("gn_pass_min_requests") and requests >= opt("gn_pass_min_requests") and x.C + C2 >= opt("gn_pass_min_cin") and opt("wreg"):
                return self.conv3x3(self.groupnorm(x, x2, norm, eps, True), wname, Cout, halo=True, **kw)
            gn = dict(x1=x.t, C1=x.C, x2=x2.t if x2 is not None else None, C2=C2, B=self.B, HW=x.H * x.W, G=self.G, eps=eps,
                      gamma=pw.f[norm + ".weight"], beta=pw.f[norm + ".bias"])
            return self.conv3x3(x, wname, Cout, x2=x2, affine=(gn, _lib.ACT_SILU), halo=True, **kw)
        assert kw.get("sc") is None
        return self.conv3x3(self.groupnorm(x, x2, norm, eps, True), wname, Cout, **kw)

    def sc_fold_ok(self, Cmid, Cout, H, W, Cs, S1):
        return opt("sc_fold") and opt("wreg") and self.halo_ok(Cmid, 0, Cout, H, W) and \
            bool(self.rec.lib.bc_conv_wreg_sc_eligible(Cmid, Cout, H, W, Cs, S1, 0))

    def groupnorm(self, x: Act, x2: Optional[Act], name, eps, silu):
        pw = self.pw
        C2 = x2.C if x2 is not None else 0
        out = self.rec.groupnorm(x.t, x.C, x2.t if x2 is not None else None, C2, self.B, x.H * x.W, self.G, eps,
                                 pw.f[name + ".weight"], pw.f[name + ".bias"], silu)
        return Act(out, x.C + C2, x.H, x.W)

    def resnet(self, p, x: Act, skip: Optional[Act], Cout, r2=None, out=None):
        pw = self.pw
        Cin = x.C + (skip.C if skip is not None else 0)
        off, n = pw.temb_slices[p]
        assert n == Cout
        rowvec = (self.tproj.data_ptr() + off * 2, pw.temb_total) + getattr(self, "tproj_table", ())
        h = self.gn_conv(x, skip, p + "norm1", 1e-5, p + "conv1", Cout, rowvec=rowvec)
        M = self.B * x.H * x.W
        if (p + "conv_shortcut.weight") in pw.h and self.sc_fold_ok(Cout, Cout, x.H, x.W, Cin, x.C if skip is not None else 0):
            return self.gn_conv(h, None, p + "norm2", 1e-5, p + "conv2", Cout, sc=(p + "conv_shortcut", x, skip), r2=r2,
                                **({"out": out} if out is not None else {}))
        if (p + "conv_shortcut.weight") in pw.h:
            kw = {}
            if skip is not None:
                kw.update(A2=skip.t, C1=x.C, lda=x.C, lda2=skip.C)
            gw = self.gw_tile(M, Cout, Cin, x.C if skip is not None else 0) if Cout >= 1280 else 0
            if gw:
                w, _, b = pw.gw(p + "conv_shortcut.weight", gw, bias=p + "conv_shortcut.bias")
                sc_t = self.rec.empty(M, Cout)
                self.rec.gemm(A=x.t, W=w, M=M, N=Cout, K=Cin, out=sc_t, bias=b, tile_cfg=gw, kind="conv1x1", **kw)
                sc = Act(sc_t, Cout, x.H, x.W)
            else:
                sc = Act(self.dense(x.t, M, Cin, p + "conv_shortcut", Cout, kind="conv1x1", **kw), Cout, x.H, x.W)
        else:
            assert skip is None and Cin == Cout
            sc = x
        return self.gn_conv(h, None, p + "norm2", 1e-5, p + "conv2", Cout, R=sc, r2=r2, **({"out": out} if out is not None else {}))

    def rowchain_ok(self, Cc, M, HW, p=""):
        if not opt("rowchain") or not self.rec.lib.bc_rowchain_supported(Cc, M, HW):
            return False
        min_blocks = {320: 1, 640: opt("rowchain_min_blocks_640")}[Cc]
        if Cc == 640 and self.cfg.is_blobnet and p.startswith("up_blocks"):
            min_blocks = opt("rowchain_min_blocks_640_blob_up")
        return M // 64 >= min_blocks

    def rowchain_ff_split(self, Cc, M):
        blocks = M // 64
        if Cc == 640:
            dflt = 4 if self.rowchain_ffp() else 2
            if self.cfg.is_blobnet and opt("ff_split_640_blob"):
                return opt("ff_split_640_blob") if blocks <= 64 else 1
            return (opt("ff_split_640") or dflt) if blocks <= 64 else 1
        return opt("ff_split_320") if blocks <= 128 else 1

    def rowchain_ffp(self):
        if not opt("ffp"):
            return False
        return not self.cfg.is_blobnet or opt("ffp_blob")

    def transformer_rowchain(self, p, x: Act, r2=None, zero=None, fan_out=None):
        from .weights import pack_rowchain
        rec, pw, B = self.rec, self.pw, self.B
        Cc, HW = x.C, x.H * x.W
        M = B * HW
        d = Cc // self.heads
        scale = d ** -0.5
        bp = p + "transformer_blocks.0."
        cache = pw.__dict__.setdefault("_rowchain", {})

        def packed(kind, zname=None, nsplit=1):
            key = (p, kind, zname, nsplit)
            if key not in cache:
                cache[key] = pack_rowchain(pw, p, kind, zname, nsplit)
            return cache[key]
        if opt("gn_finalize_launch"):
            gnkw = dict(affine=rec.gn_affine(x.t, Cc, None, 0, B, HW, self.G, 1e-6, pw.f[p + "norm.weight"], pw.f[p + "norm.bias"]))
        else:
            gnkw = dict(gn_in=(rec.gn_sources(x.t, Cc, None, 0, B, HW, self.G)[0], pw.f[p + "norm.weight"], pw.f[p + "norm.bias"], self.G, 1e-6))
        ldvt = (HW + 63) // 64 * 64
        vt = rec.zeros(B, Cc, ldvt)
        mult = 2 if fan_out is not None else 1
        h0_all, a_all = rec.empty(mult * M, Cc), rec.empty(mult * M, Cc)
        h0, qk = h0_all[:M], rec.empty(M, 2 * Cc)
        w, v = packed(_lib.CHAIN_IN)
        rec.rowchain(_lib.CHAIN_IN, Cc, M, HW, x.t, w, v, h0, out1=qk, out2=vt, ldvt=ldvt, **gnkw)
        a = a_all[:M]
        rec.attention(qk, qk, vt, a, B, self.heads, d, HW, HW, 2 * Cc, 2 * Cc, ldvt, Cc, HW * 2 * Cc, HW * 2 * Cc, Cc * ldvt, HW * Cc,
                      scale, q_off=0, k_off=Cc)
        if fan_out is not None:
            x_full, extra = fan_out
            half = M * Cc * 2
            rec.dup_halves([(h0_all, half), (a_all, half), (x_full, half)] + list(extra))
            B, M = 2 * B, 2 * M
            h0, a, x = h0_all, a_all, Act(x_full, Cc, x.H, x.W)
        h = h0
        if pw.has_cross:
            h1 = rec.empty(M, Cc)
            w, v = packed(_lib.CHAIN_MID)
            ck, cvt, T, ldc_vt = self.ctx_kv[bp]
            kvs = getattr(self, "ctx_kvs", {}).get(bp)
            if kvs is not None:
                a2 = rec.empty(M, Cc)
                rec.rowchain_midx(Cc, M, HW, a, w, v, kvs, T, self.heads, scale, h1, a2, res=h0)
                a = a2
            else:
                q2 = rec.empty(M, Cc)
                rec.rowchain(_lib.CHAIN_MID, Cc, M, HW, a, w, v, h1, out1=q2, res=h0)
                a = rec.empty(M, Cc)
                rec.attention(q2, ck, cvt, a, B, self.heads, d, HW, T, Cc, Cc, ldc_vt, Cc, HW * Cc, T * Cc, Cc * ldc_vt, HW * Cc, scale)
            h = h1
        out = rec.empty(M, Cc)
        part = rec.new_tot(B, Cc)
        kw = {}
        r2kw = self._r2(r2, x.H, x.W)
        if r2kw:
            assert r2kw["ldr2"] == Cc
            kw.update(r2=r2kw["R2"], r2_xmin=r2kw["r2_xmin"], r2_bmod=r2kw["r2_bmod"], out_w=r2kw["out_w"])
        res_out = None
        if zero is not None:
            zname, alpha, alpha_dev, alpha_idx, alpha_bstride = zero
            res_out = rec.empty(M, Cc)
            kw.update(out1=res_out, alpha=alpha, alpha_dev=alpha_dev, alpha_idx=alpha_idx, alpha_bstride=alpha_bstride)
        zname = zero[0] if zero is not None else None
        nsplit = self.rowchain_ff_split(Cc, M)
        if nsplit > 1 and self.rowchain_ffp():
            pp = rec.empty((2 if zero is not None else 1) * nsplit, M, Cc)
            w, v = packed(_lib.CHAIN_OUT_FFP, zname, nsplit)
            kw2 = {k: v_ for k, v_ in kw.items() if k != "out1"}
            rec.rowchain(_lib.CHAIN_OUT_FFP, Cc, M, HW, a, w, v, None, out1=res_out, res=h, res2=x.t, part=pp, nsplit=nsplit, **kw2)
            rec.rowchain_sum(Cc, M, HW, pp, nsplit, out, gn_tot=part, out1=res_out)
        elif nsplit > 1:
            ffp = rec.empty(nsplit, M, Cc, dtype=torch.float32)
            w, v = packed(_lib.CHAIN_OUT_FF, zname, nsplit)
            rec.rowchain(_lib.CHAIN_OUT_FF, Cc, M, HW, a, w, v, None, res=h, part=ffp, nsplit=nsplit)
            w, v = packed(_lib.CHAIN_OUT_TAIL, zname)
            rec.rowchain(_lib.CHAIN_OUT_TAIL, Cc, M, HW, None, w, v, out, res2=x.t, gn_tot=part, part=ffp, nsplit=nsplit, **kw)
        else:
            w, v = packed(_lib.CHAIN_OUT, zname)
            rec.rowchain(_lib.CHAIN_OUT, Cc, M, HW, a, w, v, out, res=h, res2=x.t, gn_tot=part, **kw)
        rec.tots[out.data_ptr()] = part
        return Act(out, Cc, x.H, x.W), res_out

    def gw_tile(self, M, N, K, C1=0, prefer=None):
        if not opt("gw") or M > opt("gw_maxm"):
            return 0
        order = prefer or (_lib.TILE_GW64x128,)
        for cfg in order:
            if self.rec.lib.bc_gemm_wreg_eligible(M, N, K, C1, cfg):
                return cfg
        return 0

    def ctx_fold_ok(self, Cc, T):
        return (self.B <= opt("ctx_fold_maxb") and Cc % 320 == 0 and Cc not in (320, 640) and self.heads == 8 and T <= 80 and (Cc // self.heads) % 8 == 0 and Cc // self.heads <= 160
                and opt("ctx_fold") and opt("gw"))

    def transformer_gw(self, p, x: Act, r2=None):
        rec, pw, B = self.rec, self.pw, self.B
        Cc, HW = x.C, x.H * x.W
        M = B * HW
        d = Cc // self.heads
        scale = d ** -0.5
        bp = p + "transformer_blocks.0."
        G128, G256, G320 = _lib.TILE_GW64x128, _lib.TILE_GW64x256, _lib.TILE_GW64x320

        def proj(a_t, wname, N, K, cfg, ln=None, bias=True, extra=(), **kw):
            for c in (cfg, G128, G320, G256):
                bn = 64 * _lib.GW_TILES[c]
                if N % bn == 0 and kw.get("n_t0", 0) % bn == 0 and rec.lib.bc_gemm_wreg_eligible(M, N, K, kw.get("C1", 0), c):
                    cfg = c
                    break
            w, cs, b = pw.gw(wname + ".weight", cfg, ln=ln, bias=(wname + ".bias") if bias else None, extra=extra)
            n_out = N // 2 if kw.get("act") == _lib.ACT_GEGLU else N
            out = kw.pop("out", None)
            if out is None:
                out = rec.empty(M, kw.get("n_t0") or n_out)
            rec.gemm(A=a_t, W=w, M=M, N=N, K=K, out=out, bias=b, tile_cfg=cfg, ln_colsum=cs, **kw)
            return out
        gn = dict(x1=x.t, C1=Cc, B=B, HW=HW, G=self.G, eps=1e-6, gamma=pw.f[p + "norm.weight"], beta=pw.f[p + "norm.bias"])
        h = proj(x.t, p + "proj_in", Cc, Cc, G128, kind="conv1x1", a_gn=gn, rows_per_batch=HW)
        ldvt = (HW + 63) // 64 * 64
        vt = rec.zeros(B, Cc, ldvt)
        qk = proj(h, bp + "attn1.to_qk", 3 * Cc, Cc, G128, ln=bp + "norm1", bias=False, extra=(bp + "attn1.to_v.weight",), C_t=vt, ldc_t=ldvt,
                  n_t0=2 * Cc, rows_per_batch=HW, kind="qkv")
        a = rec.empty(M, Cc)
        rec.attention(qk, qk, vt, a, B, self.heads, d, HW, HW, 2 * Cc, 2 * Cc, ldvt, Cc, HW * 2 * Cc, HW * 2 * Cc, Cc * ldvt, HW * Cc,
                      scale, q_off=0, k_off=Cc)
        h = proj(a, bp + "attn1.to_out.0", Cc, Cc, G128, R=h, ldr=Cc, kind="attn_out")
        folded = getattr(self, "ctx_folded", {}).get(bp) if pw.has_cross else None
        if folded is not None and rec.lib.bc_gemm_wreg_eligible(M, 128 * self.heads, Cc, 0, G128) and rec.lib.bc_gemm_wreg_eligible(M, Cc, 80 * self.heads, 0, G128):
            wqk, cs, qb, vwo = folded
            T = self.ctx_kv[bp][2]
            N, Np = 128 * self.heads, 80 * self.heads
            pr = rec.empty(M, Np)
            rec.gemm(A=h, W=wqk, M=M, N=N, K=Cc, out=pr, ldc=Np, bias=qb, tile_cfg=G128, ln_colsum=cs, rows_per_batch=HW, w_bstride=wqk.shape[1],
                     vec_bstride=N, sm_group=128, sm_valid=T, sm_keep=80, kind="xattn")
            out = rec.empty(M, Cc)
            rec.gemm(A=pr, W=vwo, M=M, N=Cc, K=Np, out=out, bias=pw.f[bp + "attn2.to_out.0.bias"], tile_cfg=G128, R=h, ldr=Cc, rows_per_batch=HW,
                     w_bstride=vwo.shape[1], kind="xattn")
            h = out
        elif pw.has_cross:
            q = proj(h, bp + "attn2.to_q", Cc, Cc, G128, ln=bp + "norm2", bias=False, kind="qkv")
            ck, cvt, T, ldc_vt = self.ctx_kv[bp]
            a = rec.empty(M, Cc)
            rec.attention(q, ck, cvt, a, B, self.heads, d, HW, T, Cc, Cc, ldc_vt, Cc, HW * Cc, T * Cc, Cc * ldc_vt, HW * Cc, scale)
            h = proj(a, bp + "attn2.to_out.0", Cc, Cc, G128, R=h, ldr=Cc, kind="attn_out")
        if opt("gw_ff1_g256") and self.g256_tile(M, 8 * Cc, Cc, dict(act=_lib.ACT_GEGLU)):
            ln = rec.layernorm(h, M, Cc, pw.f[bp + "norm3.weight"], pw.f[bp + "norm3.bias"], 1e-5)
            g = self.dense(ln, M, Cc, bp + "ff.net.0.proj", 8 * Cc, act=_lib.ACT_GEGLU, kind="ff")
        else:
            g = proj(h, bp + "ff.net.0.proj", 8 * Cc, Cc, G128, ln=bp + "norm3", act=_lib.ACT_GEGLU, kind="ff")
        if rec.lib.bc_gemm_wreg_eligible(M, Cc, 5 * Cc, 4 * Cc, G128):
            k = pw.ff2_proj_out(p)
            out = proj(g, k, Cc, 5 * Cc, G128, A2=h, C1=4 * Cc, lda=4 * Cc, lda2=Cc, R=x.t, ldr=Cc, kind="ff", rows_per_batch=HW, want_gn=True,
                       **self._r2(r2, x.H, x.W))
            return Act(out, Cc, x.H, x.W), None
        h = proj(g, bp + "ff.net.2", Cc, 4 * Cc, G128, R=h, ldr=Cc, kind="ff")
        out = proj(h, p + "proj_out", Cc, Cc, G128, R=x.t, ldr=Cc, kind="conv1x1", rows_per_batch=HW, want_gn=True, **self._r2(r2, x.H, x.W))
        return Act(out, Cc, x.H, x.W), None

    def transformer(self, p, x: Act, r2=None, zero=None):
        rec, pw, B = self.rec, self.pw, self.B
        Cc, HW = x.C, x.H * x.W
        M = B * HW
        if self.rowchain_ok(Cc, M, HW, p):
            return self.transformer_rowchain(p, x, r2, zero)
        if Cc % 320 == 0 and HW % 64 == 0 and self.gw_tile(M, Cc, Cc):
            return self.transformer_gw(p, x, r2)
        d = Cc // self.heads
        scale = d ** -0.5
        bp = p + "transformer_blocks.0."
        n = self.groupnorm(x, None, p + "norm", 1e-6, False)
        h = self.dense(n.t, M, Cc, p + "proj_in", Cc, kind="conv1x1")
        ln = rec.layernorm(h, M, Cc, pw.f[bp + "norm1.weight"], pw.f[bp + "norm1.bias"], 1e-5)
        ldvt = (HW + 63) // 64 * 64
        vt = rec.zeros(B, Cc, ldvt)
        qkv_kw = dict(C_t=vt, ldc_t=ldvt, n_t0=2 * Cc, rows_per_batch=HW)
        if self.g256_tile(M, 3 * Cc, Cc, qkv_kw):
            qk = rec.empty(M, 2 * Cc)
            rec.gemm(A=ln, W=pw.h[pw.qkv_weight(bp)], M=M, N=3 * Cc, K=Cc, out=qk, tile_cfg=_lib.TILE_G256, kind="qkv", **qkv_kw)
        else:
            qk = self.dense(ln, M, Cc, None, 2 * Cc, bias=False, wkey=bp + "attn1.to_qk.weight", kind="qkv")
            self.dense(ln, M, Cc, None, Cc, bias=False, wkey=bp + "attn1.to_v.weight", out=vt, out_mode=_lib.OUT_F16_T,
                       ldc=ldvt, rows_per_batch=HW, kind="qkv")
        a = rec.empty(M, Cc)
        rec.attention(qk, qk, vt, a, B, self.heads, d, HW, HW, 2 * Cc, 2 * Cc, ldvt, Cc, HW * 2 * Cc, HW * 2 * Cc,
                      Cc * ldvt, HW * Cc, scale, q_off=0, k_off=Cc)
        h = self.dense(a, M, Cc, bp + "attn1.to_out.0", Cc, R=h, ldr=Cc, kind="attn_out")
        if pw.has_cross:
            ln = rec.layernorm(h, M, Cc, pw.f[bp + "norm2.weight"], pw.f[bp + "norm2.bias"], 1e-5)
            q = self.dense(ln, M, Cc, None, Cc, bias=False, wkey=bp + "attn2.to_q.weight", kind="qkv")
            ck, cvt, T, ldc_vt = self.ctx_kv[bp]
            a = rec.empty(M, Cc)
            rec.attention(q, ck, cvt, a, B, self.heads, d, HW, T, Cc, Cc, ldc_vt, Cc, HW * Cc, T * Cc, Cc * ldc_vt,
                          HW * Cc, scale)
            h = self.dense(a, M, Cc, bp + "attn2.to_out.0", Cc, R=h, ldr=Cc, kind="attn_out")
# ... 230 lines not shown
```

### blobctrl_amd/launch.py

```python
import ctypes as C
import json
import os
import struct
from typing import List, Optional

import torch

from . import _lib
from .options import opt
from ._lib import BcGemm


_TUNING_PATH = os.environ.get("BC_TUNING_FILE") or os.path.join(os.path.dirname(os.path.abspath(__file__)), "gemm_tuning.json")
_TUNING = None
_M64 = (1 << 64) - 1


def tuning_table():
    global _TUNING
    if _TUNING is None:
        _TUNING = {}
        if os.path.exists(_TUNING_PATH) and not os.environ.get("BC_NO_TUNING"):
            with open(_TUNING_PATH) as f:
                _TUNING = json.load(f).get("shapes", {})
    return _TUNING


def decode_gn_tot(tot: torch.Tensor) -> torch.Tensor:
    t = tot.to(torch.float64).cpu()
    w = torch.tensor([2.0 ** -60, 2.0 ** -20, 2.0 ** 20], dtype=torch.float64)
    out = torch.stack([(t[..., 0:3] * w).sum(-1), (t[..., 3:6] * w).sum(-1)], -1)
    poisoned = (tot[..., 2].cpu().abs() >= 2 ** 45) | (tot[..., 5].cpu().abs() >= 2 ** 45)
    out[poisoned] = float("nan")
    return out


def gn_tot_slots(sums: torch.Tensor) -> torch.Tensor:
    C = sums.shape[-2]
    cg = 10 if C % 320 == 0 else 1
    return sums.reshape(*sums.shape[:-2], C // cg, cg, 2).sum(-2)


def encode_gn_tot(sums: torch.Tensor) -> torch.Tensor:
    d = sums.to(torch.float64)
    h = torch.floor(d * 2.0 ** -20)
    r = d - h * 2.0 ** 20
    m = torch.floor(r * 2.0 ** 20)
    r2 = r - m * 2.0 ** -20
    sl = torch.stack([torch.floor(r2 * 2.0 ** 60), m, h], -1).to(torch.int64)
    return sl.reshape(*sums.shape[:-1], 6).contiguous()


def ptr(t: Optional[torch.Tensor]):
    return None if t is None else t.data_ptr()


def _stream_array(stream, side=None, extra=()):
    ss = [stream, side if side is not None else stream] + [e if e is not None else stream for e in extra]
    return (C.c_void_p * len(ss))(*ss), len(ss)


_MODULE_STREAMS = {}


def run_graphed(seg: "Segment", device):
    device = torch.device(device)
    cur = torch.cuda.current_stream(device)
    cs = _MODULE_STREAMS.get(device)
    if cs is None:
        cs = _MODULE_STREAMS[device] = torch.cuda.Stream(device)
    cs.wait_stream(cur)
    if not seg.captured and not os.environ.get("BC_NO_MODULE_GRAPHS"):
        seg.run(cs.cuda_stream)
        cs.synchronize()
        seg.capture(cs.cuda_stream)
    seg.run(cs.cuda_stream)
    cur.wait_stream(cs)


class Segment:

    def __init__(self, rec: "Recorder", name: str):
        self.rec, self.name = rec, name
        self.id = rec.lib.bc_plan_segment(rec.plan, name.encode())
        if self.id < 0:
            _lib.check(1, "bc_plan_segment")
        self.captured = False
        self.flops = 0
        self.kinds = {}
        self.meta = []

    def __len__(self):
        return len(self.meta)

    def run(self, stream: int, side: int = None, extra=()):
        arr, n = _stream_array(stream, side, extra)
        rc = self.rec.lib.bc_step(self.rec.plan, self.id, arr, n)
        if rc:
            _lib.check(rc, f"bc_step({self.name})")

    def capture(self, stream: int, side: int = None, extra=()):
        arr, n = _stream_array(stream, side, extra)
        _lib.check(self.rec.lib.bc_plan_capture(self.rec.plan, self.id, arr, n), f"bc_plan_capture({self.name})")
        self.captured = True

    def run_eager(self, stream: int, side: int = None, extra=()):
        if not self.captured:
            return self.run(stream, side, extra)
        self.release()
        try:
            self.run(stream, side, extra)
        finally:
            self.capture(stream, side, extra) if stream else None

    def run_timed(self, stream: int):
        n = len(self.meta)
        ms = (C.c_float * max(1, n))()
        _lib.check(self.rec.lib.bc_plan_run_timed(self.rec.plan, self.id, stream, ms), "bc_plan_run_timed")
        return [(m, ms[i]) for i, m in enumerate(self.meta)]

    def run_timed_kernels(self, stream: int):
        n = len(self.meta)
        a, b = (C.c_float * max(1, n))(), (C.c_float * max(1, n))()
        _lib.check(self.rec.lib.bc_plan_run_timed_kernels(self.rec.plan, self.id, stream, a, b), "bc_plan_run_timed_kernels")
        return [(m, a[i], b[i]) for i, m in enumerate(self.meta)]

    def run_marked(self, stream: int, side: int, extra, marks):
        arr, n = _stream_array(stream, side, extra)
        mk = (C.c_int * max(1, len(marks)))(*marks)
        ms = (C.c_float * max(1, len(marks)))()
        _lib.check(self.rec.lib.bc_plan_run_marked(self.rec.plan, self.id, arr, n, mk, len(marks), ms), "bc_plan_run_marked")
        return [ms[i] for i in range(len(marks))]

    def enable(self, index: int, on: bool):
        _lib.check(self.rec.lib.bc_plan_enable(self.rec.plan, self.id, index, 1 if on else 0), "bc_plan_enable")

    def release(self):
        if self.captured:
            self.rec.lib.bc_plan_release(self.rec.plan, self.id)
            self.captured = False


class Recorder:
    def __init__(self, device: torch.device):
        self.lib = _lib.load()
        self.device = torch.device(device)
        h = C.c_void_p()
        _lib.check(self.lib.bc_plan_create(C.byref(h)), "bc_plan_create")
        self.plan = h
        self.seg: Optional[Segment] = None
        self.segments: List[Segment] = []
        self.keep = []
        self._workspace = set()
        self._storages = {}
        self.named = {}
        self._slab = {}
        self._slab_elems = {}
        self.num_cu = 256
        if self.device.type == "cuda":
            info = (C.c_int * 4)()
            _lib.check(self.lib.bc_device_info(info), "bc_device_info")
            self.num_cu = info[0]
        self.bytes_allocated = 0
        self.tots = {}
        self.tots_per_channel = set()
        self._tot_chunk = {}
        self.sid = 0
        self.events = []
        self.loop_graphs = []

    def close(self):
        if self.plan is not None:
            for g in self.loop_graphs:
                self.lib.bc_graph_destroy(g)
            self.loop_graphs = []
            self.lib.bc_plan_destroy(self.plan)
            self.plan = None

    def empty(self, *shape, dtype=torch.float16, name=None):
        return self._track(torch.empty(*shape, dtype=dtype, device=self.device), name)

    def zeros(self, *shape, dtype=torch.float16, name=None):
        return self._track(torch.zeros(*shape, dtype=dtype, device=self.device), name)

    def _track(self, t, name=None):
        self.bytes_allocated += t.numel() * t.element_size()
        self._workspace.add(t.untyped_storage().data_ptr())
        return self.register(t, name)

    def register(self, t: torch.Tensor, name=None):
        if t is not None and torch.is_tensor(t):
            st = t.untyped_storage()
            key = st.data_ptr()
            if key not in self._storages and st.nbytes() > 0:
                self._storages[key] = torch.empty(0, dtype=torch.uint8, device=t.device).set_(st)
            if name:
                self.named[name] = t
        return t

    @property
    def buffers(self):
        return list(self._storages.values())

    def begin(self, name: str) -> Segment:
        self.seg = Segment(self, name)
        self.segments.append(self.seg)
        return self.seg

    def new_event(self):
        e = self.lib.bc_plan_new_event(self.plan)
        if e < 0:
            _lib.check(1, "bc_plan_new_event")
        self.events.append(e)
        return e

    def signal(self, ev):
        self._add_op(_lib.OP_SIGNAL, "i", (ev,), "event_record")
        self.seg.meta[-1]["ev"] = ev

    def wait(self, ev):
        self._add_op(_lib.OP_WAIT, "i", (ev,), "event_wait")
        self.seg.meta[-1]["ev"] = ev

    def _add_op(self, op, sig, args, kind, flops=0, variant="", shape=None, bytes_=0, rocprof=None):
        assert len(sig) == len(args), (op, sig, args)
        words = (C.c_uint64 * max(1, len(args)))()
        for k, (c, v) in enumerate(zip(sig, args)):
            if c == "p":
                words[k] = 0 if v is None else (self.register(v).data_ptr() if torch.is_tensor(v) else int(v))
            elif c == "f":
                words[k] = struct.unpack("<I", struct.pack("<f", float(v)))[0]
            else:
                words[k] = int(v) & _M64
        idx = self.lib.bc_plan_add_op(self.plan, self.seg.id, self.sid, op, words, len(args))
        if idx < 0 or idx != len(self.seg.meta):
            _lib.check(1, f"bc_plan_add_op({kind})")
        self._push(kind, flops, variant, shape, bytes_, rocprof)

    def _push(self, kind, flops=0, variant="", shape=None, bytes_=0, rocprof=None):
        self.seg.flops += flops
        self.seg.kinds[kind] = self.seg.kinds.get(kind, 0) + 1
        self.seg.meta.append(dict(kind=kind, flops=flops, variant=variant, shape=shape, bytes=bytes_, sid=self.sid, rocprof=rocprof or variant))

    def capture_loop(self, segments, stream, side=None, extra=()):
        ids = (C.c_int * len(segments))(*[sg.id for sg in segments])
        arr, n = _stream_array(stream, side, extra)
        g = C.c_void_p()
        _lib.check(self.lib.bc_plan_capture_loop(self.plan, ids, len(segments), arr, n, C.byref(g)), "bc_plan_capture_loop")
        self.loop_graphs.append(g)
        return g

    def destroy_loop_graph(self, g):
        self.lib.bc_graph_destroy(g)
        self.loop_graphs = [h for h in self.loop_graphs if h is not g]

    def save(self, path: str):
        for t in self._slab.values():
            self.register(t)
        bufs = self.buffers
        names = {}
        for n, t in self.named.items():
            assert t.data_ptr() == t.untyped_storage().data_ptr(), f"named buffer {n} must own its storage"
            names[t.data_ptr()] = n
        arr = (_lib.BcPlanBuffer * len(bufs))()
        hold = []
        for i, t in enumerate(bufs):
            nbytes = t.numel() * t.element_size()
            arr[i].name = names.get(t.data_ptr(), "").encode()
            arr[i].address = t.data_ptr()
            arr[i].bytes = nbytes
            if nbytes and t.data_ptr() not in self._workspace:
                host = t.detach().cpu().contiguous()
                hold.append(host)
                arr[i].host_data = host.data_ptr()
        _lib.check(self.lib.bc_plan_save(self.plan, path.encode(), arr, len(bufs)), "bc_plan_save")

    def reserve_slab(self, elems: int):
        sid = self.sid
        if elems > self._slab_elems.get(sid, 0):
            self._slab[sid] = torch.empty(elems, dtype=torch.float32, device=self.device)
            self._workspace.add(self._slab[sid].untyped_storage().data_ptr())
            self._slab_elems[sid] = elems
            _lib.check(self.lib.bc_plan_set_slab(self.plan, sid, self._slab[sid].data_ptr()), "bc_plan_set_slab")

    TOT_CHUNK_WORDS = 1 << 20

    def new_tot(self, B, Cc):
        n = B * Cc * _lib.GN_TOT_WORDS
        key = (self.seg.id, self.sid)
        ch = self._tot_chunk.get(key)
        if ch is None or ch[1] + n > ch[0].numel():
            t = self.zeros(max(self.TOT_CHUNK_WORDS, n), dtype=torch.int64)
            self.keep.append(t)
            self._op("bc_memset_zero", (t, t.numel() * 8), "memset", variant="memset_zero", shape=("memset", t.numel() * 8))
            ch = self._tot_chunk[key] = [t, 0]
        view = ch[0][ch[1]:ch[1] + n].view(B, Cc, _lib.GN_TOT_WORDS)
        ch[1] += (n + 31) // 32 * 32
        return view

    def dup_halves(self, items):
        assert 0 < len(items) <= 6
        args = []
        for t, nbytes in items:
            assert nbytes % 16 == 0 and t.numel() * t.element_size() >= 2 * nbytes
            args += [t, nbytes]
        args += [None, 0] * (6 - len(items))
        self.keep.append(tuple(t for t, _ in items))
        total = sum(b for _, b in items)
        self._op("bc_dup_halves", tuple(args), "dup_halves", variant="dup_halves_kernel", shape=("dup_halves", total), bytes_=2 * total)

    def plan_gemm(self, M, N, K, fast, mode, tile_cfg=0, splitk=None):
        sk = -1 if splitk is None else splitk
        if tile_cfg == 0 and splitk is None and fast:
            hit = tuning_table().get(f"{mode}|{M}|{N}|{K}")
            if hit:
                tile_cfg, sk = int(hit[0]), int(hit[1])
        c, s_, bm, bn = C.c_int(tile_cfg), C.c_int(sk), C.c_int(0), C.c_int(0)
        _lib.check(self.lib.bc_gemm_plan(M, N, K, 1 if fast else 0, C.byref(c), C.byref(s_), C.byref(bm), C.byref(bn)),
                   "bc_gemm_plan")
        return c.value, s_.value, bm.value, bn.value

    def gemm(self, *, A, W, M, N, K, out=None, out_mode=_lib.OUT_F16, ldc=None, A2=None, C1=0, lda=None, lda2=0,
             conv=None, bias=None, rowvec=None, ld_rowvec=0, rowvec_idx=None, rowvec_step=0, rows_per_batch=0, act=_lib.ACT_NONE, colscale=None,
             alpha=1.0, alpha_dev=None, alpha_idx=None, alpha_bstride=0, R=None, ldr=0, R2=None, ldr2=0, r2_xmin=0, r2_bmod=1,
             out_w=0, splitk=None, kind="gemm", a_offset=0, w_offset=0, out_offset=0, want_gn=False, tile_cfg=0, ldw=None,
             a_affine=None, a_act=_lib.ACT_NONE, a_gn=None, ln_colsum=None, ln_eps=1e-5, C_t=None, ldc_t=0, n_t0=0,
             w_bstride=0, vec_bstride=0, sm_group=0, sm_valid=0, sm_keep=0, gn_tot_out=None, S=None, S2=None, lds=0, lds2=0, S1=0, Cs=0):
        n_out = N // 2 if act == _lib.ACT_GEGLU else (N // sm_group * sm_keep if sm_group else N)
        g = BcGemm()
        g.A = A.data_ptr() + a_offset * A.element_size()
        g.A2 = ptr(A2)
        g.a_mode = _lib.A_CONV3X3 if conv else _lib.A_DENSE
        g.M, g.N, g.K = M, N, K
        g.lda = lda if lda is not None else (K if not conv else 0)
        g.lda2, g.C1 = lda2, C1
        g.a_affine, g.a_act = ptr(a_affine), a_act
        if conv:
            g.Cin, g.Hin, g.Win = conv["Cin"], conv["Hin"], conv["Win"]
            g.Hv, g.Wv = conv.get("Hv", conv["Hin"]), conv.get("Wv", conv["Win"])
            g.Hout, g.Wout, g.stride = conv["Hout"], conv["Wout"], conv.get("stride", 1)
            g.conv_nopad_lo = 1 if conv.get("nopad_lo") else 0
        g.W = W.data_ptr() + w_offset * W.element_size()
        g.ldw = ldw if ldw is not None else K
        g.bias = ptr(bias)
        g.rowvec = ptr(rowvec) if not isinstance(rowvec, int) else rowvec
        g.ld_rowvec, g.rows_per_batch = ld_rowvec, rows_per_batch
        g.rowvec_idx, g.rowvec_step = ptr(rowvec_idx), rowvec_step
        g.act = act
        g.colscale = ptr(colscale)
        g.alpha = alpha
        g.alpha_dev, g.alpha_idx, g.alpha_bstride = ptr(alpha_dev), ptr(alpha_idx), alpha_bstride
        g.R, g.ldr = (ptr(R) if not isinstance(R, int) else R), ldr
        g.R2, g.ldr2, g.r2_xmin, g.r2_bmod, g.out_w = ptr(R2), ldr2, r2_xmin, r2_bmod, out_w
        g.out_mode = out_mode
        g.C = out.data_ptr() + out_offset * out.element_size()
        g.ldc = ldc if ldc is not None else (n_t0 if C_t is not None else n_out)
        es = out.element_size()
        c_hi = g.C + (((M - 1) * g.ldc + n_out) * es if out_mode != _lib.OUT_F16_T else out.numel() * es - out_offset * es)
        for nm, t, ld, width in (("R", R, ldr, n_out), ("R2", R2, ldr2, n_out), ("S", S, lds, S1 or Cs), ("S2", S2, lds2, Cs - S1)):
            if t is None:
                continue
            lo = t if isinstance(t, int) else t.data_ptr()
            hi = lo + (((M - 1) * ld + width) * 2 if isinstance(t, int) or nm != "R2" else t.numel() * t.element_size())
            if lo < c_hi and g.C < hi:
                raise _lib.BlobCtrlHipError(f"bc_gemm({kind}): the output [{g.C:#x}, {c_hi:#x}) overlaps {nm} [{lo:#x}, {hi:#x})")
        g.ln_colsum, g.ln_eps = ptr(ln_colsum), ln_eps
        g.C_t, g.ldc_t, g.n_t0 = ptr(C_t), ldc_t, n_t0
        g.w_bstride, g.vec_bstride, g.sm_group, g.sm_valid, g.sm_keep = w_bstride, vec_bstride, sm_group, sm_valid, sm_keep
        if S is not None:
            assert tile_cfg == _lib.TILE_WREG and R is None and Cs % 64 == 0 and Cs > 0
            g.S, g.S2, g.lds, g.lds2, g.S1, g.Cs = ptr(S), ptr(S2), lds, lds2, S1, Cs
        fast = K % 64 == 0
        mode = "dense"
        if conv:
            hv, wv = conv.get("Hv", conv["Hin"]), conv.get("Wv", conv["Win"])
            ups = (hv, wv) != (conv["Hin"], conv["Win"])
            fast = fast and conv["Cin"] % 64 == 0 and (not ups or ((hv, wv) == (2 * conv["Hin"], 2 * conv["Win"])
                                                                  and conv.get("stride", 1) == 1))
            mode = "ups" if ups else f"conv{conv.get('stride', 1)}"
        elif A2 is not None:
            fast = fast and C1 % 64 == 0
        if os.environ.get("BC_GEMM_GENERIC"):
            fast = False
        if tile_cfg in (_lib.TILE_HALO, _lib.TILE_WREG):
            nch = conv["Cin"] // 64
            base = (M // 128) * (N // 160)
            explicit_sk, sk_req = splitk, None
            if splitk is None:
                target = opt("halo_ctas") or (128 if tile_cfg == _lib.TILE_WREG else 256)
                min_cps = opt("halo_min_cps") or (3 if tile_cfg == _lib.TILE_WREG else 2)
                full = opt("halo_full") or target * 2 // 3
                short = tile_cfg == _lib.TILE_WREG and base >= target // 2 and nch <= 5
                splitk = 1 if (base >= full or short) else max(1, min(nch // min_cps, -(-target // base)))
            splitk = max(splitk, -(-nch // self.lib.bc_conv_halo_max_chunks()))
            cps = -(-nch // max(1, splitk))
            cfg, sk, bm, bn = tile_cfg, -(-nch // cps), 128, 160
            if Cs:
                nsc = Cs // 64
                sk_req = min(sk if explicit_sk is None else splitk, nch + nsc)
                s2 = -(-(nch + nsc) // -(-(nch + nsc) // sk_req))
                cps = -(-nch // s2)
                sk = max(-(-nch // cps), -(-nsc // -(-nsc // s2)))
            fast, mode = True, "halo"
            sc_mode = "_sc" if S is not None else ""
            if a_gn is not None:
                G_ = a_gn["G"]
                span = cps * 64 + 2 * (conv["Cin"] // G_)
                t1, t2 = self.gn_sources(a_gn["x1"], a_gn["C1"], a_gn["x2"], a_gn["C2"], a_gn["B"], a_gn["HW"], a_gn["G"])
                fin_max = 2752 if tile_cfg == _lib.TILE_WREG else 712
                if span <= fin_max and not opt("gn_finalize_launch"):
                    g.a_tot1, g.a_tot2 = ptr(t1), ptr(t2)
                    g.a_gamma, g.a_beta, g.a_groups, g.a_eps = ptr(a_gn["gamma"]), ptr(a_gn["beta"]), G_, a_gn["eps"]
                    self.keep.append((t1, t2, a_gn["gamma"], a_gn["beta"]))
                    for t in (t1, t2, a_gn["gamma"], a_gn["beta"]):
                        self.register(t)
                    mode = "halo_gnfin"
                else:
                    a_affine = self.gn_affine(a_gn["x1"], a_gn["C1"], a_gn["x2"], a_gn["C2"], a_gn["B"], a_gn["HW"], G_, a_gn["eps"],
                                              a_gn["gamma"], a_gn["beta"])
                    g.a_affine = ptr(a_affine)
            mode += sc_mode
        elif tile_cfg in _lib.GW_TILES:
            assert not conv and a_affine is None and splitk in (None, 1) and rowvec is None
            cfg, sk, bm, bn = tile_cfg, 1, 64, 64 * _lib.GW_TILES[tile_cfg]
            fast, mode = True, "gw" + ("_ln" if ln_colsum is not None else "") + ("_qkv" if C_t is not None else "") + ("_gn" if a_gn is not None else "") + \
                ("_softmax" if sm_group else "") + ("_wimg" if w_bstride else "")
            if a_gn is not None:
                t1, _ = self.gn_sources(a_gn["x1"], a_gn["C1"], None, 0, a_gn["B"], a_gn["HW"], a_gn["G"])
                g.a_tot1 = ptr(t1)
                g.a_gamma, g.a_beta, g.a_groups, g.a_eps = ptr(a_gn["gamma"]), ptr(a_gn["beta"]), a_gn["G"], a_gn["eps"]
                self.keep.append((t1, a_gn["gamma"], a_gn["beta"]))
                for t in (t1, a_gn["gamma"], a_gn["beta"]):
                    self.register(t)
        elif tile_cfg == _lib.TILE_G256:
            assert not conv and a_affine is None and splitk in (None, 1)
            cfg, sk, bm, bn = tile_cfg, 1, 256, 256
            fast, mode = True, "g256" + ("_qkv" if C_t is not None else "") + ("_2src" if A2 is not None else "")
        else:
            assert a_affine is None and (not conv or A2 is None), "fused GroupNorm prologue / two-source conv need TILE_HALO / TILE_WREG"
            cfg, sk, bm, bn = self.plan_gemm(M, N, K, fast, mode, tile_cfg, splitk)
        g.splitk = sk
        if Cs:
            g.splitk = sk_req
        g.tile_cfg = cfg
        if sk > 1:
            self.reserve_slab(sk * M * N)
        part = None
        if want_gn:
            rpb = rows_per_batch if rows_per_batch > 0 else (conv["Hout"] * conv["Wout"] if conv else M)
            vec = out_mode == _lib.OUT_F16 and n_out % 8 == 0 and g.ldc % 8 == 0 and (R is None or ldr % 8 == 0) and \
                (R2 is None or ldr2 % 8 == 0)
            slab_rows = bm if sk == 1 else 32
            if vec and (fast or sk > 1) and N % 4 == 0 and rpb % slab_rows == 0 and M % rpb == 0 and \
                    not os.environ.get("BC_GEMM_TILE"):
                part = gn_tot_out if gn_tot_out is not None else self.new_tot(M // rpb, n_out)
                assert tuple(part.shape[:2]) == (M // rpb, n_out)
                g.gn_tot = part.data_ptr()
                self.tots[g.C] = part

        idx = self.lib.bc_plan_add_gemm(self.plan, self.seg.id, self.sid, C.byref(g))
        if idx < 0 or idx != len(self.seg.meta):
            _lib.check(1, "bc_plan_add_gemm")
        refs = (A, A2, W, out, bias, R, R2, rowvec, rowvec_idx, colscale, alpha_dev, alpha_idx, part, a_affine, ln_colsum, C_t, S, S2)
        self.keep.append(refs)
        for t in refs:
            self.register(t)
        variant = ("conv_halo_kernel<" if cfg == _lib.TILE_HALO else "conv_wreg_kernel<" if cfg == _lib.TILE_WREG else
                   "gemm_wreg_kernel<" if cfg in _lib.GW_TILES else "gemm256_kernel<" if cfg == _lib.TILE_G256 else "gemm_fast_kernel<" if fast else "gemm_kernel<") + _lib.TILE_NAMES[cfg] + "," + mode + ">" + \
            ("+splitk_reduce" if sk > 1 else "")
        FAST = {1: "256, 128, 4, 2, 3", 2: "128, 128, 2, 2, 3", 3: "128, 128, 2, 2, 2", 4: "256, 64, 4, 1, 2", 5: "256, 64, 4, 1, 3",
                6: "128, 64, 2, 2, 3", 7: "64, 64, 2, 2, 4"}
        if cfg in (_lib.TILE_HALO, _lib.TILE_WREG):
            rp = ("conv_wreg_kernel" if cfg == _lib.TILE_WREG else "conv_halo_kernel") + f"<{2 if g.a_tot1 else 1 if g.a_affine else 0}>"
        elif cfg == _lib.TILE_G256:
            rp = "gemm256_kernel"
        elif cfg in _lib.GW_TILES:
            rp = f"gemm_wreg_kernel<{_lib.GW_TILES[cfg]}, {10 if _lib.GW_TILES[cfg] == 5 else 20}, {'true' if sm_group else 'false'}>"
        elif fast:
            ups_ = bool(conv) and (conv.get("Hv", conv["Hin"]), conv.get("Wv", conv["Win"])) != (conv["Hin"], conv["Win"])
            rp = f"gemm_fast_kernel<{FAST[cfg]}, {'true' if conv else 'false'}, {'true' if ups_ else 'false'}>"
        else:
            rp = "gemm_kernel<" + ("256, 64, 4, 1" if bn == 64 else "128, 128, 2, 2") + ">"
        a_elems = (M // (conv["Hout"] * conv["Wout"])) * conv["Hin"] * conv["Win"] * conv["Cin"] if conv else M * K
        alg_bytes = 2 * (a_elems + N * K + M * n_out) + (2 * M * n_out if R is not None else 0) + 2 * (M + N) * Cs
        self._push(kind, 2 * M * N * (K + Cs), variant, (mode, M, N, K + Cs, sk), alg_bytes, rp)
        return out

    def _op(self, name, args, kind, **meta):
        self._add_op(_lib.OPS[name], _lib.op_signature(name), args, kind, **meta)

    def gn_sources(self, x1, C1, x2, C2, B, HW, G):
        srcs = []
        c2_ = C2 if x2 is not None else 0
        cpg = (C1 + c2_) // G
        for x, c, off in ((x1, C1, 0), (x2, c2_, C1)):
            if x is None:
                srcs.append(None)
                continue
            hit = self.tots.get(x.data_ptr())
            blocks_ok = c % 320 != 0 or id(hit) in self.tots_per_channel or (cpg % 10 == 0 and off % 10 == 0)
            if hit is not None and hit.shape[1] == c and blocks_ok:
                srcs.append(hit)
            else:
                tot = self.new_tot(B, c)
                self.keep.append((x, tot))
                self._op("bc_gn_stats", (x, c, B, HW, tot), "gn_stats", variant="gn_stats_kernel",
                         shape=("gn_stats", B, HW, c), bytes_=B * HW * c * 2)
                self.tots[x.data_ptr()] = tot
                self.tots_per_channel.add(id(tot))
                srcs.append(tot)
        return tuple(srcs)

    def groupnorm(self, x1, C1, x2, C2, B, HW, G, eps, gamma, beta, silu, out=None):
        c2 = C2 if x2 is not None else 0
        Cc = C1 + c2
        if out is None:
            out = self.empty(B, HW, Cc)
        n_before = self.seg.kinds.get("gn_stats", 0)
        t1, t2 = self.gn_sources(x1, C1, x2, c2, B, HW, G)
        own_stats = self.seg.kinds.get("gn_stats", 0) > n_before
        fused = not os.environ.get("BC_GN_UNFUSED") and Cc // G <= 96
        self.keep.append((x1, x2, t1, t2, gamma, beta, out))
        kind = "groupnorm" + ("" if own_stats else "_fused_stats")
        if fused:
            self._op("bc_gn_apply_fused", (t1, C1, t2, c2, x1, x2, B, HW, G, eps, gamma, beta, 1 if silu else 0, out), kind,
                     variant="gn_apply_fused_kernel", shape=("gn", B, HW, Cc), bytes_=2 * B * HW * Cc * 2)
        else:
            ab = self.empty(B, Cc, 2, dtype=torch.float32)
            self.keep.append(ab)
            self._op("bc_gn_finalize", (t1, C1, t2, c2, B, HW, G, eps, gamma, beta, ab), "gn_finalize",
                     variant="gn_finalize_kernel", shape=("gn_ab", B, HW, Cc))
            self._op("bc_gn_apply", (x1, C1, x2, c2, B, HW, ab, 1 if silu else 0, out), kind, variant="gn_apply_kernel",
                     shape=("gn", B, HW, Cc), bytes_=2 * B * HW * Cc * 2)
        return out

    def gn_affine(self, x1, C1, x2, C2, B, HW, G, eps, gamma, beta):
        c2 = C2 if x2 is not None else 0
        Cc = C1 + c2
        ab = self.empty(B, Cc, 2, dtype=torch.float32)
        t1, t2 = self.gn_sources(x1, C1, x2, c2, B, HW, G)
        self.keep.append((x1, x2, t1, t2, ab, gamma, beta))
        self._op("bc_gn_finalize", (t1, C1, t2, c2, B, HW, G, eps, gamma, beta, ab), "gn_finalize",
                 variant="gn_finalize_kernel", shape=("gn_ab", B, HW, Cc))
        return ab

    def layernorm(self, x, rows, Cc, gamma, beta, eps, out=None, ldx=None, ldy=None):
        if out is None:
            out = self.empty(rows, Cc)
        self.keep.append((x, gamma, beta, out))
        self._op("bc_layernorm", (x, rows, Cc, ldx or Cc, gamma, beta, eps, out, ldy or Cc), "layernorm", variant="layernorm_kernel",
                 shape=("ln", rows, Cc), bytes_=2 * rows * Cc * 2)
        return out

    def attention(self, Q, K, Vt, out, B, heads, d, Nq, Nkv, ldq, ldk, ldvt, ldo, qbs, kbs, vbs, obs, scale,
                  q_off=0, k_off=0, causal=False):
        self.keep.append((Q, K, Vt, out))
        self._op("bc_attention_causal" if causal else "bc_attention",
                 (Q.data_ptr() + q_off * 2, K.data_ptr() + k_off * 2, Vt, out, B, heads, d, Nq, Nkv, ldq, ldk, ldvt, ldo, qbs, kbs, vbs,
                  obs, scale), "attention", flops=4 * B * heads * Nq * Nkv * d, variant=f"attn_fwd_kernel<{d}>",
                 shape=(B, heads, d, Nq, Nkv), bytes_=2 * B * heads * d * (2 * Nq + 2 * Nkv))
        return out

    def rowchain(self, kind, Cc, M, rows_per_batch, x, wstream, vec, out0, out1=None, out2=None, ldvt=0, affine=None, gn_in=None, res=None, res2=None,
                 r2=None, r2_xmin=0, r2_bmod=1, out_w=0, gn_tot=None, ln_eps=1e-5, alpha=1.0, alpha_dev=None, alpha_idx=None,
                 alpha_bstride=0, part=None, nsplit=1):
        mult = {_lib.CHAIN_IN: 4, _lib.CHAIN_MID: 2, _lib.CHAIN_OUT: 14 + (1 if out1 is not None else 0), _lib.CHAIN_OUT_FF: 13,
                _lib.CHAIN_OUT_TAIL: 1 + (1 if out1 is not None else 0), _lib.CHAIN_OUT_FFP: 14 + (1 if out1 is not None else 0)}[kind]
        g_tot, g_gamma, g_beta, g_groups, g_eps = gn_in if gn_in is not None else (None, None, None, 0, 0.0)
        refs = (x, wstream, vec, out0, out1, out2, affine, res, res2, r2, gn_tot, alpha_dev, alpha_idx, part, g_tot, g_gamma, g_beta)
        self.keep.append(refs)
        for t in refs:
            self.register(t)
        name = {_lib.CHAIN_IN: "in", _lib.CHAIN_MID: "mid", _lib.CHAIN_OUT: "out", _lib.CHAIN_OUT_FF: f"out_ff/{nsplit}", _lib.CHAIN_OUT_TAIL: "out_tail",
                _lib.CHAIN_OUT_FFP: f"out_ffp/{nsplit}"}[kind]
        zk = (_lib.CHAIN_OUT, _lib.CHAIN_OUT_TAIL, _lib.CHAIN_OUT_FFP)
        self._op("bc_rowchain", (kind, Cc, M, rows_per_batch, x, affine, g_tot, g_gamma, g_beta, g_groups, g_eps, res, res2, r2, r2_xmin, r2_bmod, out_w, wstream, vec, out0, out1, out2,
                                 ldvt, gn_tot, ln_eps, alpha, alpha_dev, alpha_idx, alpha_bstride, part, nsplit), "rowchain",
                 flops=2 * M * Cc * Cc * mult,
                 variant=f"rowchain_kernel<{name}{',zero' if kind in zk and out1 is not None else ''}>",
                 shape=("rowchain_" + name, M, Cc, mult * Cc), bytes_=2 * (mult * Cc * Cc + 2 * M * Cc),
                 rocprof=f"rowchain_kernel<{Cc}, {kind}, {'true' if kind in zk and out1 is not None else 'false'}>")
        return out0

    def rowchain_sum(self, Cc, M, rows_per_batch, part, nsplit, out0, gn_tot=None, out1=None):
        refs = (part, out0, gn_tot, out1)
        self.keep.append(refs)
        for t in refs:
            self.register(t)
        nout = 2 if out1 is not None else 1
        self._op("bc_rowchain_sum", (Cc, M, rows_per_batch, part, nsplit, out0, gn_tot, out1), "rowchain_sum", variant="rowchain_sum_kernel",
                 shape=("rowchain_sum", M, Cc, nsplit), bytes_=2 * nout * (nsplit + 1) * M * Cc, rocprof=f"rowchain_sum_kernel<{Cc}>")
        return out0

    def rowchain_kv_stream(self, ck, cvt, B, T, Cc, ldvt):
        frags = self.lib.bc_rowchain_kv_frags(Cc)
        if frags < 0:
            _lib.check(1, "bc_rowchain_kv_frags")
        out = self.empty(B * (Cc // 80) * frags * 64 * 8)
        self.keep.append((ck, cvt, out))
        self._op("bc_rowchain_pack_kv", (ck, Cc, cvt, ldvt, B, T, Cc, out), "pack_kv", variant="rowchain_pack_kv_kernel",
                 shape=("pack_kv", B, T, Cc), bytes_=2 * (2 * B * T * Cc) + out.numel() * 2, rocprof=f"rowchain_pack_kv_kernel<{Cc}>")
        return out

    def ctx_fold(self, ck, cvt, B, T, Cc, ldvt, heads, scale, wq, bq, wo):
        N = 128 * heads
        s_qk, s_vo = self.lib.bc_gemm_wreg_stream_elems(N, Cc), self.lib.bc_gemm_wreg_stream_elems(Cc, 80 * heads)
        wqk, vwo = self.zeros(B, s_qk), self.zeros(B, s_vo)
        cs, qb = self.zeros(B, N, dtype=torch.float32), self.zeros(B, N, dtype=torch.float32)
        refs = (ck, cvt, wq, bq, wo, wqk, cs, qb, vwo)
        self.keep.append(refs)
        for t in refs:
            self.register(t)
        self._op("bc_ctx_fold", (ck, Cc, cvt, ldvt, B, T, Cc, heads, scale, wq, bq, wo, wqk, cs, qb, vwo), "ctx_fold", variant="ctx_fold_kernel",
                 flops=2 * 2 * B * 80 * heads * Cc * (Cc // heads), shape=("ctx_fold", B, T, Cc), bytes_=2 * (2 * Cc * Cc + B * (N + 80 * heads) * Cc),
                 rocprof="ctx_fold_qk_kernel")
        return wqk, cs, qb, vwo

    def rowchain_midx(self, Cc, M, rows_per_batch, x, wstream, vec, kvstream, n_ctx, heads, scale, out0, out1, res, ln_eps=1e-5):
        assert heads * (Cc // heads) == Cc and heads == 8, "CHAIN_MIDX is laid out for 8 heads"
        refs = (x, wstream, vec, kvstream, out0, out1, res)
        self.keep.append(refs)
        for t in refs:
            self.register(t)
        B = M // rows_per_batch
        self._op("bc_rowchain_midx", (Cc, M, rows_per_batch, x, res, wstream, vec, kvstream, n_ctx, scale, out0, out1, ln_eps), "rowchain",
                 flops=2 * M * Cc * Cc * 2 + 4 * M * n_ctx * Cc, variant="rowchain_kernel<midx>",
                 shape=("rowchain_midx", M, Cc, 2 * Cc), bytes_=2 * (2 * Cc * Cc + 3 * M * Cc + 2 * B * n_ctx * Cc),
                 rocprof=f"rowchain_kernel<{Cc}, {_lib.CHAIN_MIDX}, false>")
        return out1

    def call(self, name, *args, kind=None, keep=()):
        self.keep.append(keep)
        for t in keep if isinstance(keep, (tuple, list)) else (keep,):
            self.register(t)
        self._op(name, args, kind or name)
```

### blobctrl_amd/options.py

```python
import os

TABLE = {
    "rowchain": (True, "transformer blocks of 320 / 640 channels on csrc/rowchain.hip (0: GroupNorm / LayerNorm / GEMM launch list)"),
    "midx": (True, "cross-attention of the 320 / 640-channel blocks inside the row-chain's MID launch (0: MID + bc_attention)"),
    "ffp": (True, "UNet's split 640-channel block end as OUT_FFP + sum (0: OUT_FF + OUT_TAIL)"),
    "ffp_blob": (False, "BlobNet's split block end as OUT_FFP + sum too"),
    "gw": (True, "1280-channel projections at M <= gw_maxm on csrc/gemm_wreg.hip (0: LDS-DMA tiles + LayerNorm launches)"),
    "ctx_fold": (True, "cross-attention of the 1280-channel blocks folded over the prompt (0: to_q + bc_attention + to_out)"),
    "g256": (True, "large-M dense projections on csrc/gemm256.hip from g256_min_tiles tiles on (0: gemm_fast tiles)"),
    "gw_ff1_g256": (True, "ff.net.0 of the 1280-channel blocks at M <= gw_maxm as LayerNorm + gemm256.hip where it has >= g256_min_tiles tiles"),
    "cfg_prefix": (True, "CFG-invariant prefix of the UNet once per image pair (0: every launch at the full CFG batch)"),
    "wreg": (True, "ResBlock convolutions on csrc/conv_wreg.hip (0: csrc/conv_halo.hip)"),
    "sc_fold": (True, "a ResBlock's 1x1 shortcut folded into conv2's K loop on csrc/conv_wreg.hip (0: a conv1x1 launch + residual read)"),
    "halo": (True, "ResBlock convolutions with the fused GroupNorm prologue at all (0: GroupNorm pass + implicit GEMM)"),
    "gn_finalize_launch": (False, "a bc_gn_finalize launch per GroupNorm instead of the finalize in the consumer's prologue"),
    "halo_ctas": (0, "workgroups a split-K convolution pass aims for (0: 128 on conv_wreg, 256 on conv_halo)"),
    "halo_min_cps": (0, "fewest 64-channel chunks per workgroup of a split pass (0: 3 on conv_wreg, 2 on conv_halo)"),
    "halo_full": (0, "workgroups from which a pass runs unsplit (0: two thirds of halo_ctas)"),
    "rowchain_min_blocks_640": (64, "fewest 64-row blocks for the 640-channel row-chain"),
    "rowchain_min_blocks_640_blob_up": (32, "... for BlobNet's up blocks"),
    "ff_split_640": (0, "workgroups per row block of the 640-channel block end up to 64 row blocks (0: 4 with OUT_FFP, 2 without)"),
    "ff_split_640_blob": (0, "... for BlobNet (0: as ff_split_640)"),
    "ff_split_320": (1, "workgroups per row block of the 320-channel block end up to 128 row blocks"),
    "gw_maxm": (1024, "largest M of a projection on gemm_wreg.hip"),
    "ctx_fold_maxb": (2, "largest UNet batch that takes the prompt-folded cross-attention"),
    "gn_pass_min_requests": (4, "edit requests per batch from which a ResBlock convolution runs as GroupNorm pass + plain conv_wreg (0: never)"),
    "gn_pass_min_cin": (320, "... and fewest input channels of such a convolution"),
    "g256_min_tiles": (64, "fewest 256 x 256 tiles for gemm256.hip (a quarter of the CUs: the other queue has the rest)"),
}


def _parse(text):
    out = {}
    for item in (text or "").replace(";", ",").split(","):
        item = item.strip()
        if not item:
            continue
        if "=" not in item:
            raise ValueError(f"BC_PLAN: '{item}' is not key=value")
        k, v = (s.strip() for s in item.split("=", 1))
        if k not in TABLE:
            raise ValueError(f"BC_PLAN: unknown key '{k}' (known: {', '.join(sorted(TABLE))})")
        try:
            iv = int(v)
        except ValueError:
            raise ValueError(f"BC_PLAN: {k}={v} is not an integer") from None
        out[k] = bool(iv) if isinstance(TABLE[k][0], bool) else iv
    return out


def effective():
    vals = {k: d for k, (d, _) in TABLE.items()}
    vals.update(_parse(os.environ.get("BC_PLAN")))
    return vals


def opt(key):
    if key not in TABLE:
        raise KeyError(key)
    return effective()[key]


def non_default():
    return {k: v for k, v in effective().items() if v != TABLE[k][0]}
```

### blobctrl_amd/weights.py

```python
from collections import OrderedDict
from typing import Dict, Optional

import torch


def pad8(n: int) -> int:
    return (n + 7) // 8 * 8


def merge_lora(sd: Dict[str, torch.Tensor], lora: Dict[str, torch.Tensor], alphas: Optional[Dict[str, float]] = None,
               adapter_scale: float = 1.0) -> Dict[str, torch.Tensor]:
    out = OrderedDict((k, v.clone()) for k, v in sd.items())
    for key in list(lora.keys()):
        if not key.endswith(".lora_A.weight"):
            continue
        mod = key[: -len(".lora_A.weight")]
        a = lora[key].float()
        b = lora[mod + ".lora_B.weight"].float()
        r = b.shape[1]
        alpha = float(alphas.get(mod, r)) if alphas else float(r)
        w = out[mod + ".weight"]
        delta = (b.flatten(1) @ a.flatten(1)).reshape(w.shape)
        out[mod + ".weight"] = w + (adapter_scale * alpha / r) * delta
    return out


def pack_conv3x3(w: torch.Tensor) -> torch.Tensor:
    co, ci = w.shape[:2]
    cip = pad8(ci)
    p = torch.zeros(co, 3, 3, cip, dtype=torch.float32)
    p[..., :ci] = w.permute(0, 2, 3, 1)
    return p.reshape(co, 9 * cip)


WREG_TILES = ((0, 3), (3, 2), (5, 2), (7, 3))


def pack_conv_wreg(w: torch.Tensor, wsc: Optional[torch.Tensor] = None) -> torch.Tensor:
    N, K = w.shape
    Cin = K // 9
    assert N % 160 == 0 and Cin % 64 == 0 and K == 9 * Cin, (N, K)
    nch = Cin // 64
    v = w.reshape(N // 160, 10, 16, 3, 3, nch, 2, 4, 8)
    Cs = 0
    if wsc is not None:
        Cs = wsc.shape[1]
        assert wsc.shape[0] == N and Cs % 64 == 0 and Cs > 0, tuple(wsc.shape)
        vs = wsc.reshape(N // 160, 10, 16, Cs // 64, 2, 4, 8)
    parts = []
    for blk in range(N // 160):
        for t0, nt in WREG_TILES:
            g = v[blk, t0:t0 + nt]
            g = g.permute(5, 4, 3, 2, 0, 6, 1, 7)
            if wsc is None:
                parts.append(g.reshape(-1))
                continue
            s = vs[blk, t0:t0 + nt].permute(3, 2, 0, 4, 1, 5)
            for kg in range(2):
                parts += [g[kg].reshape(-1), s[kg].reshape(-1)]
    return torch.cat(parts).reshape(N, K + Cs)


def pack_matrix(w: torch.Tensor) -> torch.Tensor:
    w = w.reshape(w.shape[0], -1)
    co, ci = w.shape
    cip = pad8(ci)
    if cip == ci:
        return w.contiguous()
    p = torch.zeros(co, cip, dtype=torch.float32)
    p[:, :ci] = w
    return p


def interleave_geglu(w: torch.Tensor, b: torch.Tensor):
    n = w.shape[0] // 2
    assert n % 32 == 0, "GEGLU inner dim must be a multiple of 32"
    wv, wg = w[:n].reshape(n // 32, 32, -1), w[n:].reshape(n // 32, 32, -1)
    bv, bg = b[:n].reshape(n // 32, 32), b[n:].reshape(n // 32, 32)
    return torch.cat([wv, wg], dim=1).reshape(2 * n, -1).contiguous(), torch.cat([bv, bg], dim=1).reshape(2 * n).contiguous()


def pack_gemm_wreg(w: torch.Tensor, nt: int) -> torch.Tensor:
    N, K = w.shape
    assert N % (64 * nt) == 0 and K % 32 == 0, (N, K, nt)
    v = w.reshape(N // (64 * nt), 4, nt, 16, K // 32, 4, 8)
    v = v.permute(0, 1, 4, 2, 5, 3, 6).reshape(-1)
    return torch.cat([v, torch.zeros(32 * 512, dtype=w.dtype, device=w.device)])


def fold_layernorm(w: torch.Tensor, bias: Optional[torch.Tensor], gamma: torch.Tensor, beta: torch.Tensor):
    wf = w.float()
    w2 = (wf * gamma.float()[None, :]).half()
    cs = w2.float().sum(1)
    b2 = wf @ beta.float()
    if bias is not None:
        b2 = b2 + bias.float()
    return w2, cs.contiguous(), b2.contiguous()


def fold_cross_attention(k: torch.Tensor, vt: torch.Tensor, T: int, heads: int, scale: float, wq: torch.Tensor, bq: torch.Tensor, wo: torch.Tensor):
    B, _, C = k.shape
    D = C // heads
    kh = torch.zeros(B, heads, 128, D, dtype=torch.float32, device=k.device)
    kh[:, :, :T] = k[:, :T].float().reshape(B, T, heads, D).permute(0, 2, 1, 3)
    qk = (torch.einsum("bhjd,hdc->bhjc", kh, wq.float().reshape(heads, D, C)) * scale).half().reshape(B, heads * 128, C)
    qb = (torch.einsum("bhjd,hd->bhj", kh, bq.float().reshape(heads, D)) * scale).reshape(B, heads * 128)
    vh = torch.zeros(B, heads, D, 80, dtype=torch.float32, device=k.device)
    vh[..., :T] = vt[:, :, :T].float().reshape(B, heads, D, T)
    vo = torch.einsum("nhd,bhdj->bnhj", wo.float().reshape(C, heads, D), vh).half().reshape(B, C, heads * 80)
    return qk, qk.float().sum(-1), qb, vo


class PackedTrunk:

    def gw(self, key: str, tile_cfg: int, ln: Optional[str] = None, bias: Optional[str] = None, extra=()):
        from . import _lib
        nt = _lib.GW_TILES[tile_cfg]
        ck = ("gw", key, tuple(extra), nt, ln)
        cache = self.__dict__.setdefault("_gw", {})
        if ck not in cache:
            w = self.h[key] if not extra else torch.cat([self.h[key]] + [self.h[e] for e in extra], 0)
            b = self.f[bias] if bias else None
            cs = None
            if ln is not None:
                w, cs, b = fold_layernorm(w, b, self.f[ln + ".weight"], self.f[ln + ".bias"])
            cache[ck] = (pack_gemm_wreg(w, nt), cs, b)
        return cache[ck]

    def ff2_proj_out(self, p: str) -> str:
        k = p + "ff2_proj_out"
        if k + ".weight" not in self.h:
            bp = p + "transformer_blocks.0."
            P = self.h[p + "proj_out.weight"].float()
            F2 = self.h[bp + "ff.net.2.weight"].float()
            self.h[k + ".weight"] = torch.cat([P @ F2, P], 1).half().contiguous()
            self.f[k + ".bias"] = (P @ self.f[bp + "ff.net.2.bias"].float() + self.f[p + "proj_out.bias"].float()).contiguous()
        return k

    def qkv_weight(self, bp: str) -> str:
        k = bp + "attn1.to_qkv.weight"
        if k not in self.h:
            self.h[k] = torch.cat([self.h[bp + "attn1.to_qk.weight"], self.h[bp + "attn1.to_v.weight"]], 0).contiguous()
        return k

    def ctx_fold_weights(self, bp: str):
        cache = self.__dict__.setdefault("_ctx_fold", {})
        if bp not in cache:
            wq, _, bq = fold_layernorm(self.h[bp + "attn2.to_q.weight"], None, self.f[bp + "norm2.weight"], self.f[bp + "norm2.bias"])
            cache[bp] = (wq.contiguous(), bq)
        return cache[bp] + (self.h[bp + "attn2.to_out.0.weight"],)

    def wreg(self, key: str) -> str:
        k2 = key + "_wreg"
        if k2 not in self.h:
            self.h[k2] = pack_conv_wreg(self.h[key])
        return k2

    def wreg_sc(self, conv: str, sc: str):
        k2, kb = conv + ".weight+sc_wreg", conv + ".bias+sc"
        if k2 not in self.h:
            self.h[k2] = pack_conv_wreg(self.h[conv + ".weight"], self.h[sc + ".weight"])
            self.f[kb] = (self.f[conv + ".bias"].float() + self.f[sc + ".bias"].float()).contiguous()
        return k2, kb

    def __init__(self, sd: Dict[str, torch.Tensor], device, block_out_channels, layers_per_block=2):
        self.device = device
        self.h: Dict[str, torch.Tensor] = {}
        self.f: Dict[str, torch.Tensor] = {}
        self.boc = tuple(block_out_channels)
        sd = {k: v.detach().float().cpu() for k, v in sd.items()}
        self.has_cross = any(".attn2." in k for k in sd)
        temb_w, temb_b, self.temb_slices = [], [], {}
        off = 0
        for k, v in sd.items():
            if k.endswith(".bias") or (v.ndim == 1):
                if ".time_emb_proj." in k or ".ff.net.0.proj." in k:
                    continue
                self.f[k] = v.to(device)
                continue
            if ".time_emb_proj.weight" in k:
                p = k[: -len("time_emb_proj.weight")]
                temb_w.append(v)
                temb_b.append(sd[p + "time_emb_proj.bias"])
                self.temb_slices[p] = (off, v.shape[0])
                off += v.shape[0]
            elif ".ff.net.0.proj.weight" in k:
                w, b = interleave_geglu(v, sd[k[:-6] + "bias"])
                self.h[k] = w.half().to(device)
                self.f[k[:-6] + "bias"] = b.to(device)
            elif k.endswith("attn1.to_q.weight"):
                p = k[: -len("to_q.weight")]
                self.h[p + "to_qk.weight"] = torch.cat([v, sd[p + "to_k.weight"]], 0).half().to(device)
            elif k.endswith("attn1.to_k.weight"):
                continue
            elif v.ndim == 4 and v.shape[-1] == 3:
                self.h[k] = pack_conv3x3(v).half().to(device)
            else:
                self.h[k] = pack_matrix(v).half().to(device)
        self.temb_total = off
        w_in = sd["conv_in.weight"]
        co = w_in.shape[0]

        def k128(w8ch):
            out = torch.zeros(co, 128)
            out[:, :72] = w8ch.reshape(co, 72)
            return out
        if w_in.shape[1] <= 8:
            base = torch.zeros(co, 3, 3, 8)
            base[..., : w_in.shape[1]] = w_in.permute(0, 2, 3, 1)
            self.h["conv_in.weight_k128"] = k128(base).half().to(device)
        if w_in.shape[1] > 8:
            base = torch.zeros(co, 3, 3, 8)
            base[..., :5] = w_in[:, :5].permute(0, 2, 3, 1)
            self.h["conv_in.weight8"] = k128(base).half().to(device)
            fm = torch.zeros(co, 16, w_in.shape[1] - 5)
            fm[:, :9] = w_in[:, 5:].permute(0, 2, 3, 1).reshape(co, 9, -1)
            self.h["conv_in.featmat"] = pack_matrix(fm.reshape(co * 16, -1)).half().to(device)
        self.h["temb_all.weight"] = torch.cat(temb_w, 0).half().to(device)
        self.f["temb_all.bias"] = torch.cat(temb_b, 0).to(device)
        self._to_arenas()

    @staticmethod
    def _layout(tensors, align_elems):
        layout, off = [], 0
        for k, t in tensors.items():
            layout.append((k, tuple(t.shape), off))
            off += (t.numel() + align_elems - 1) // align_elems * align_elems
        return layout, off

    def _to_arenas(self):
        self.h_layout, hn = self._layout(self.h, 128)
        self.f_layout, fn = self._layout(self.f, 64)
        self.h_arena = torch.zeros(hn, dtype=torch.float16, device=self.device)
        self.f_arena = torch.zeros(fn, dtype=torch.float32, device=self.device)
        self._view(copy_from=(self.h, self.f))

    def _view(self, copy_from=None):
        h, f = {}, {}
        for (k, shape, off) in self.h_layout:
            n = 1
            for d in shape:
                n *= d
            h[k] = self.h_arena[off:off + n].view(shape)
            if copy_from is not None:
                h[k].copy_(copy_from[0][k])
        for (k, shape, off) in self.f_layout:
            n = 1
            for d in shape:
                n *= d
            f[k] = self.f_arena[off:off + n].view(shape)
            if copy_from is not None:
                f[k].copy_(copy_from[1][k])
        self.h, self.f = h, f

    def meta(self):
        return dict(h_layout=self.h_layout, f_layout=self.f_layout, temb_slices=self.temb_slices,
                    temb_total=self.temb_total, has_cross=self.has_cross, boc=self.boc,
                    h_elems=self.h_arena.numel(), f_elems=self.f_arena.numel())

    @classmethod
    def from_meta(cls, meta, device):
        self = cls.__new__(cls)
        self.device = device
        self.h_layout, self.f_layout = meta["h_layout"], meta["f_layout"]
        self.temb_slices, self.temb_total = meta["temb_slices"], meta["temb_total"]
        self.has_cross, self.boc = meta["has_cross"], meta["boc"]
        self.h_arena = torch.zeros(meta["h_elems"], dtype=torch.float16, device=device)
        self.f_arena = torch.zeros(meta["f_elems"], dtype=torch.float32, device=device)
        self._view()
        return self

    def derived_nbytes(self):
        n = sum(t.numel() * t.element_size() for k, t in self.h.items() if k.endswith("_wreg"))
        for cache in (self.__dict__.get("_gw", {}), self.__dict__.get("_rowchain", {}), self.__dict__.get("_ctx_fold", {})):
            for v in cache.values():
                n += sum(t.numel() * t.element_size() for t in v if torch.is_tensor(t))
        return n

    def nbytes(self):
        return self.h_arena.numel() * 2 + self.f_arena.numel() * 4 + self.derived_nbytes()


RC_HC, RC_RPAD = 128, 20
RC_CHANNELS = (320, 640)


def _frag_stream(w: torch.Tensor, row_starts, k0: int = 0, k1: int = None) -> torch.Tensor:
    k1 = w.shape[1] if k1 is None else k1
    rs = torch.as_tensor(row_starts, device=w.device)
    nw, nt = rs.shape
    rows = rs[:, :, None] + torch.arange(16, device=w.device)
    x = w[rows.reshape(-1), k0:k1].reshape(nw, nt, 16, (k1 - k0) // 32, 4, 8)
    return x.permute(0, 3, 1, 4, 2, 5).reshape(nw, -1, 64, 8).contiguous()


def pack_rowchain_kv(k: torch.Tensor, vt: torch.Tensor, T: int, pad_frags: int = 20) -> torch.Tensor:
    B, _, C = k.shape
    D = C // 8
    hpw, qks, vtiles = 80 // D, (2 if D == 40 else 3), (3 if D == 40 else 5)
    fr_head = 5 * qks + 3 * vtiles
    nw = C // 80
    out = torch.zeros(B, nw, hpw * fr_head + pad_frags, 64, 8, dtype=torch.float16, device=k.device)
    kp = torch.zeros(B, 80, C + 64, dtype=torch.float16, device=k.device)
    kp[:, :T, :C] = k[:, :T]
    vp = torch.zeros(B, C, 96, dtype=torch.float16, device=k.device)
    vp[:, :, :T] = vt[:, :, :T]
    lane = torch.arange(64, device=k.device)
    m, q = lane % 16, lane // 16
    j = torch.arange(8, device=k.device)
    for w in range(nw):
        for hh in range(hpw):
            c_h = 80 * w + D * hh
            s0 = c_h // 32
            f0 = hh * fr_head
            for ks in range(qks):
                for t in range(5):
                    ch = 32 * (s0 + ks) + 8 * q[:, None] + j[None, :]
                    val = kp[:, (16 * t + m)[:, None].expand(64, 8), ch]
                    inside = (ch >= c_h) & (ch < c_h + D)
                    out[:, w, f0 + ks * 5 + t] = torch.where(inside[None], val, torch.zeros_like(val))
            tlo = 2 if (D == 40 and hh == 1) else 0
            for ks in range(3):
                for tv in range(vtiles):
                    chv = 80 * w + 16 * (tlo + tv) + m
                    key = 32 * ks + 8 * q[:, None] + j[None, :]
                    val = vp[:, chv[:, None].expand(64, 8), key]
                    inside = ((chv >= c_h) & (chv < c_h + D))[:, None].expand(64, 8)
                    out[:, w, f0 + 5 * qks + ks * vtiles + tv] = torch.where(inside[None], val, torch.zeros_like(val))
    return out


def pack_rowchain(pw: "PackedTrunk", p: str, kind: int, zero_name: Optional[str] = None, nsplit: int = 1):
    h, f = pw.h, pw.f
    bp = p + "transformer_blocks.0."
    C = h[p + "proj_in.weight"].shape[0]
    assert C in RC_CHANNELS, C
    nw = C // 80
    nC = [[80 * w + 16 * t for t in range(5)] for w in range(nw)]
    segs, vec = [], []
    if kind == 0:
        qk = h[bp + "attn1.to_qk.weight"]
        segs = [_frag_stream(h[p + "proj_in.weight"], nC), _frag_stream(qk[:C], nC), _frag_stream(qk[C:], nC),
                _frag_stream(h[bp + "attn1.to_v.weight"], nC)]
        vec = [f[p + "proj_in.bias"], f[bp + "norm1.weight"], f[bp + "norm1.bias"]]
    elif kind == 1:
        segs = [_frag_stream(h[bp + "attn1.to_out.0.weight"], nC), _frag_stream(h[bp + "attn2.to_q.weight"], nC)]
        vec = [f[bp + "attn1.to_out.0.bias"], f[bp + "norm2.weight"], f[bp + "norm2.bias"]]
    else:
        att = "attn2" if pw.has_cross else "attn1"
        w1i, b1i = h[bp + "ff.net.0.proj.weight"], f[bp + "ff.net.0.proj.bias"]
        hid = 4 * C
        w1 = w1i.reshape(hid // 32, 2, 32, C)
        b1 = b1i.reshape(hid // 32, 2, 32)
        wv, wg = w1[:, 0].reshape(hid, C), w1[:, 1].reshape(hid, C)
        bv, bg = b1[:, 0].reshape(hid), b1[:, 1].reshape(hid)
        w1o = torch.cat([wv, wg], 0)
        w2 = h[bp + "ff.net.2.weight"]
        seg_to_out = _frag_stream(h[bp + att + ".to_out.0.weight"], nC)
        ffb, chunks = [], []
        hpw = RC_HC // nw
        for c in range(hid // RC_HC):
            cs = []
            for tp in range(hpw // 16):
                cs.append(_frag_stream(w1o, [[RC_HC * c + hpw * w + 16 * tp, hid + RC_HC * c + hpw * w + 16 * tp] for w in range(nw)]))
            cs.append(_frag_stream(w2, nC, RC_HC * c, RC_HC * (c + 1)))
            chunks.append(cs)
            for w in range(nw):
                for tp in range(hpw // 16):
                    j0 = RC_HC * c + hpw * w + 16 * tp
                    ffb += [bv[j0:j0 + 16], bg[j0:j0 + 16]]
        seg_proj_out = _frag_stream(h[p + "proj_out.weight"], nC)
        if kind == 2:
            segs = [seg_to_out] + [x for cs in chunks for x in cs] + [seg_proj_out]
        elif kind == 4:
            segs = [seg_proj_out]
        vec = [f[bp + att + ".to_out.0.bias"], f[bp + "norm3.weight"], f[bp + "norm3.bias"], torch.cat(ffb), f[bp + "ff.net.2.bias"],
               f[p + "proj_out.bias"]]
        seg_zero = None
        if zero_name is not None:
            seg_zero = _frag_stream(h[zero_name + ".weight"], nC)
            if kind not in (3, 6):
                segs.append(seg_zero)
            vec.append(f[zero_name + ".bias"])
        if kind in (3, 6):
            nchunks = len(chunks)
            assert nchunks % nsplit == 0, (nchunks, nsplit)
            pad = torch.zeros(nw, RC_RPAD, 64, 8, dtype=torch.float16, device=seg_to_out.device)
            per = nchunks // nsplit
            tail = ([seg_proj_out] + ([seg_zero] if seg_zero is not None else [])) if kind == 6 else []
            slices = [torch.cat([seg_to_out] + [x for cs in chunks[z * per:(z + 1) * per] for x in cs] + tail + [pad], 1) for z in range(nsplit)]
            return torch.stack(slices).contiguous(), torch.cat([v.reshape(-1).float() for v in vec]).contiguous()
    pad = torch.zeros(nw, RC_RPAD, 64, 8, dtype=torch.float16, device=segs[0].device)
    return torch.cat(segs + [pad], 1).contiguous(), torch.cat([v.reshape(-1).float() for v in vec]).contiguous()
```

### include/blobctrl_hip.h

```cpp
#ifndef BLOBCTRL_HIP_H
#define BLOBCTRL_HIP_H

#include <stdint.h>

#ifdef __cplusplus
extern "C" {
#endif

typedef uint16_t bc_half;
typedef void*    bc_stream;

const char* bc_last_error(void);
int bc_version(void);
int bc_device_info(int* out4);

enum { BC_A_DENSE = 0, BC_A_CONV3X3 = 1 };
enum { BC_ACT_NONE = 0, BC_ACT_GELU = 1, BC_ACT_GEGLU = 2, BC_ACT_SILU = 3, BC_ACT_QUICK_GELU = 4  };
enum { BC_OUT_F16 = 0, BC_OUT_F16_T = 1, BC_OUT_F32 = 2 };

typedef struct BcGemm {
    const bc_half* A;
    const bc_half* A2;
    int a_mode;
    int M, N, K;
    int lda, lda2;
    int C1;
    int Cin;
    int Hin, Win;
    int Hv, Wv;
    int Hout, Wout;
    int stride;
    int conv_nopad_lo;
    const bc_half* W;
    int ldw;
    const float*   bias;
    const bc_half* rowvec;
    int ld_rowvec;
    int rows_per_batch;
    const int* rowvec_idx;
    int rowvec_step;
    int act;
    const float*   colscale;
    float alpha;
    const float*   alpha_dev;
    const int*     alpha_idx;
    int alpha_bstride;
    const bc_half* R;
    int ldr;
    const bc_half* R2;
    int ldr2, r2_xmin, r2_bmod, out_w;
    int out_mode;
    void* C;
    int ldc;
    int splitk;
    float* slab;
    unsigned long long* gn_tot;
    int tile_cfg;
    const float* a_affine;
    int a_act;
    const unsigned long long* a_tot1;
    const unsigned long long* a_tot2;
    const float* a_gamma; const float* a_beta;
    int a_groups; float a_eps;
    const float* ln_colsum; float ln_eps;
    void* C_t; int ldc_t, n_t0;
    long long w_bstride; int vec_bstride;
    int sm_group, sm_valid, sm_keep;
    const bc_half* S; const bc_half* S2;
    int lds, lds2, S1, Cs;
} BcGemm;

int bc_gemm(const BcGemm* p, bc_stream stream);
int bc_sizeof_gemm(void);
enum { BC_TILE_AUTO = 0, BC_TILE_256x128 = 1, BC_TILE_128x128_S3 = 2, BC_TILE_128x128_S2 = 3, BC_TILE_256x64_S2 = 4,
       BC_TILE_256x64_S3 = 5, BC_TILE_128x64 = 6, BC_TILE_64x64 = 7, BC_TILE_COUNT = 8,
       BC_TILE_HALO = 8,
       BC_TILE_WREG = 9,
       BC_TILE_GW64x128 = 10, BC_TILE_GW64x256 = 11, BC_TILE_GW64x320 = 12,
       BC_TILE_G256 = 13 };
int bc_gemm_wreg_pack(const bc_half* w, int ldw, int N, int K, int tile_cfg, bc_half* out, bc_stream stream);
long long bc_gemm_wreg_stream_elems(int N, int K);
int bc_gemm_wreg_eligible(int M, int N, int K, int C1, int tile_cfg);
int bc_gemm256_eligible(int M, int N, int K, int C1, int out_mode, int rows_per_batch, int want_gn);
int bc_conv_wreg_pack(const bc_half* w, int N, int Cin, bc_half* out, bc_stream stream);
int bc_conv_wreg_pack_sc(const bc_half* w, int N, int Cin, const bc_half* wsc, int Cs, bc_half* out, bc_stream stream);
int bc_conv_wreg_pack_host(const bc_half* w, int N, int Cin, const bc_half* wsc, int Cs, bc_half* out);
int bc_conv_wreg_sc_eligible(int Cin, int N, int H, int W, int Cs, int S1, int reserved);
int bc_conv_halo_eligible(int Cin, int C1, int N, int Hin, int Win, int Hout, int Wout, int stride);
int bc_conv_halo_max_chunks(void);
int bc_gemm_plan(int M, int N, int K, int fast, int* tile_cfg, int* splitk, int* bm, int* bn);

enum { BC_GN_TOT_WORDS = 6 };
int bc_gn_stats(const bc_half* x, int C, int B, int HW, unsigned long long* tot, bc_stream stream);
int bc_gn_finalize(const unsigned long long* tot1, int C1, const unsigned long long* tot2, int C2, int B, int HW, int G,
                   float eps, const float* gamma, const float* beta, float* ab, bc_stream stream);
int bc_gn_apply(const bc_half* x1, int C1, const bc_half* x2, int C2, int B, int HW,
                const float* ab, int silu, bc_half* y, bc_stream stream);
int bc_gn_apply_fused(const unsigned long long* tot1, int C1, const unsigned long long* tot2, int C2,
                      const bc_half* x1, const bc_half* x2, int B, int HW, int G, float eps, const float* gamma,
                      const float* beta, int silu, bc_half* y, bc_stream stream);
int bc_memset_zero(void* ptr, long long bytes, bc_stream stream);
int bc_dup_halves(void* p0, long long bytes0, void* p1, long long bytes1, void* p2, long long bytes2, void* p3, long long bytes3,
                  void* p4, long long bytes4, void* p5, long long bytes5, bc_stream stream);

int bc_softmax_rows(bc_half* x, int rows, int cols, int ld, bc_stream stream);

int bc_embed_tokens(const long long* ids, const bc_half* tok_emb, const float* pos_emb, int B, int T, int D, int vocab,
                    bc_half* out, bc_stream stream);

int bc_gaussian_sample(const bc_half* moments, const float* noise, int B, int Cz, int HW, float scale, float* out,
                       bc_stream stream);

int bc_layernorm(const bc_half* x, int rows, int C, int ldx, const float* gamma, const float* beta, float eps,
                 bc_half* y, int ldy, bc_stream stream);

int bc_attention(const bc_half* Q, const bc_half* K, const bc_half* Vt, bc_half* O,
                 int B, int heads, int d, int Nq, int Nkv,
                 int ldq, int ldk, int ldvt, int ldo,
                 long long q_bstride, long long k_bstride, long long vt_bstride, long long o_bstride,
                 float scale, bc_stream stream);
int bc_attention_causal(const bc_half* Q, const bc_half* K, const bc_half* Vt, bc_half* O,
                        int B, int heads, int d, int Nq, int Nkv,
                        int ldq, int ldk, int ldvt, int ldo,
                        long long q_bstride, long long k_bstride, long long vt_bstride, long long o_bstride,
                        float scale, bc_stream stream);

int bc_splat_scores(const double* params_host, int n, int h, int w, double* out, bc_stream stream);

int bc_splat_maps(const double* params_host, int n, int h, int w, double* raw, double* composed, bc_stream stream);
int bc_alpha_composite(const double* raw, long long npix, int K, double* out, bc_stream stream);
int bc_splat_from_scores(const void* S, const void* F, int N, int M, int C, int Hin, int Win, long long s_n, long long s_m,
                         long long s_y, long long s_x, int Hout, int Wout, int is_f32, void* out, bc_stream stream);
int bc_resize_bilinear(const void* in, long long planes, int Hin, int Win, int Hout, int Wout, int is_f32, void* out,
                       bc_stream stream);
int bc_pack_rgb8(const double* img, int H, int W, unsigned char* out, bc_stream stream);

int bc_assemble_input(const float* latents, int Blat, const float* img_lat, const float* score, const float* feat,
                      int Bimg, int F, int Bout, int h, int w, int Cpad, int dup_score, bc_half* X, bc_stream stream);
int bc_assemble_input_im2col(const float* latents, int Blat, const float* img_lat, const float* score, int Bimg, int Bout,
                             int h, int w, int dup_score, bc_half* X, bc_stream stream);

int bc_timestep_embedding(const float* t_table, const int* t_idx, float t_value, int rows, int dim, bc_half* out,
                          bc_stream stream);
int bc_timestep_embedding_table(const float* t_table, int nsteps, int rows_per_step, int dim, bc_half* out, bc_stream stream);

int bc_silu(const bc_half* x, bc_half* y, long long n, bc_stream stream);

int bc_cfg_scheduler_step(const float* eps, float* latents, const float* coef, int* step_idx, float* hist,
                          float guidance_scale, int B, int h, int w, float* eps_out, int advance, bc_stream stream);

int bc_cfg_scheduler_step_noise(const float* eps, float* latents, const float* coef, int* step_idx, float* hist,
                                float guidance_scale, int B, int h, int w, const float* noise, int nsteps, float* eps_out,
                                int advance, bc_stream stream);

int bc_cfg_scheduler_step3(const float* eps, float* latents, const float* coef, int* step_idx, float* hist,
                           float guidance_scale, int B, int h, int w, int nsteps, float* eps_out, int advance, bc_stream stream);

enum { BC_CHAIN_IN = 0, BC_CHAIN_MID = 1, BC_CHAIN_OUT = 2, BC_CHAIN_OUT_FF = 3, BC_CHAIN_OUT_TAIL = 4, BC_CHAIN_MIDX = 5, BC_CHAIN_OUT_FFP = 6 };
int bc_rowchain_supported(int channels, int M, int rows_per_batch);
long long bc_rowchain_stream_frags(int channels, int kind, int blobnet, int nsplit);
int bc_rowchain(int kind, int channels, int M, int rows_per_batch, const bc_half* x, const float* affine,
                const unsigned long long* gn_in, const float* gn_gamma, const float* gn_beta, int gn_groups, float gn_eps, const bc_half* res,
                const bc_half* res2, const bc_half* r2, int r2_xmin, int r2_bmod, int out_w, const bc_half* wstream,
                const float* vec, bc_half* out0, bc_half* out1, bc_half* out2, int ldvt, unsigned long long* gn_tot, float ln_eps,
                float alpha, const float* alpha_dev, const int* alpha_idx, int alpha_bstride, float* part, int nsplit, bc_stream stream);
int bc_rowchain_sum(int channels, int M, int rows_per_batch, const bc_half* part, int nsplit, bc_half* out0, unsigned long long* gn_tot,
                    bc_half* out1, bc_stream stream);
long long bc_rowchain_kv_frags(int channels);
int bc_rowchain_pack_kv(const bc_half* k, int ldk, const bc_half* vt, int ldvt, int B, int T, int channels, bc_half* out, bc_stream stream);

int bc_ctx_fold(const bc_half* k, int ldk, const bc_half* vt, int ldvt, int B, int T, int channels, int heads, float scale,
                const bc_half* wq, const float* bq, const bc_half* wo, bc_half* wqk, float* qk_colsum, float* qk_bias, bc_half* vwo,
                bc_stream stream);
int bc_rowchain_midx(int channels, int M, int rows_per_batch, const bc_half* x, const bc_half* res, const bc_half* wstream, const float* vec,
                     const bc_half* kvstream, int n_ctx, float attn_scale, bc_half* out0, bc_half* out1, float ln_eps, bc_stream stream);

int bc_nchw_to_nhwc_f16(const void* src, int src_is_f32, int B, int C, int HW, int Cpad, bc_half* dst, bc_stream stream);
int bc_nhwc_to_nchw(const bc_half* src, int B, int C, int HW, int ldsrc, void* dst, int dst_is_f32, bc_stream stream);
int bc_add_cls_pos(const bc_half* patches, const float* cls, const float* pos, int B, int T, int D, bc_half* out,
                   bc_stream stream);
int bc_patchify(const float* pixels, int B, int H, int W, int patch, int Kpad, bc_half* out, bc_stream stream);

int bc_graph_begin(bc_stream stream);
int bc_graph_end(bc_stream stream, void** graph_exec_out);
int bc_graph_launch(void* graph_exec, bc_stream stream);
int bc_graph_destroy(void* graph_exec);

int bc_event_create_sync(void** ev);
int bc_stream_wait_event(bc_stream stream, void* ev);

int bc_event_create(void** ev);
int bc_event_record(void* ev, bc_stream stream);
int bc_event_elapsed_ms(void* start, void* stop, float* ms);
int bc_event_destroy(void* ev);

typedef struct BcPlan BcPlan;
enum { BC_OP_GEMM = 0, BC_OP_GN_STATS = 1, BC_OP_GN_FINALIZE = 2, BC_OP_GN_APPLY_FUSED = 3, BC_OP_GN_APPLY = 4, BC_OP_LAYERNORM = 5,
       BC_OP_ATTENTION = 6, BC_OP_ATTENTION_CAUSAL = 7, BC_OP_ASSEMBLE_INPUT = 8, BC_OP_TIMESTEP_EMBEDDING = 9,
       BC_OP_TIMESTEP_EMBEDDING_TABLE = 10, BC_OP_CFG_SCHEDULER_STEP = 11, BC_OP_EMBED_TOKENS = 12, BC_OP_SOFTMAX_ROWS = 13,
       BC_OP_PATCHIFY = 14, BC_OP_ADD_CLS_POS = 15, BC_OP_SILU = 16, BC_OP_NCHW_TO_NHWC_F16 = 17, BC_OP_NHWC_TO_NCHW = 18,
       BC_OP_GAUSSIAN_SAMPLE = 19, BC_OP_SIGNAL = 20 , BC_OP_WAIT = 21 , BC_OP_ROWCHAIN = 22, BC_OP_ASSEMBLE_IM2COL = 23,
       BC_OP_MEMSET_ZERO = 24, BC_OP_ROWCHAIN_MIDX = 25, BC_OP_ROWCHAIN_PACK_KV = 26, BC_OP_ROWCHAIN_SUM = 27, BC_OP_CTX_FOLD = 28, BC_OP_DUP_HALVES = 29,
       BC_OP_CFG_SCHEDULER_STEP_NOISE = 30, BC_OP_CFG_SCHEDULER_STEP3 = 31, BC_OP_COUNT = 32 };
typedef struct BcPlanBuffer {
    const char* name;
    const void* address;
    long long   bytes;
    const void* host_data;
} BcPlanBuffer;

int bc_plan_create(BcPlan** out);
int bc_plan_destroy(BcPlan* plan);
int bc_plan_segment(BcPlan* plan, const char* name);
int bc_plan_find_segment(BcPlan* plan, const char* name);
int bc_plan_new_event(BcPlan* plan);
int bc_plan_add_gemm(BcPlan* plan, int seg, int stream_id, const BcGemm* g);
int bc_plan_add_op(BcPlan* plan, int seg, int stream_id, int op, const uint64_t* args, int nargs);
int bc_plan_set_slab(BcPlan* plan, int stream_id, float* slab);
int bc_plan_enable(BcPlan* plan, int seg, int index, int enabled);
int bc_plan_num_launches(BcPlan* plan, int seg);
int bc_step(BcPlan* plan, int seg, const bc_stream* streams, int nstreams);
int bc_plan_capture(BcPlan* plan, int seg, const bc_stream* streams, int nstreams);
int bc_plan_release(BcPlan* plan, int seg);
int bc_plan_capture_loop(BcPlan* plan, const int* seg_sequence, int n, const bc_stream* streams, int nstreams, void** graph_exec_out);
int bc_plan_run_timed(BcPlan* plan, int seg, bc_stream stream, float* ms_out );
int bc_plan_run_timed_kernels(BcPlan* plan, int seg, bc_stream stream, float* ms_main, float* ms_reduce);
int bc_plan_run_marked(BcPlan* plan, int seg, const bc_stream* streams, int nstreams, const int* marks, int nmarks, float* ms_out);
int bc_plan_save(BcPlan* plan, const char* path, const BcPlanBuffer* buffers, int nbuffers);
int bc_plan_load(const char* path, BcPlan** out);
int bc_plan_buffer(BcPlan* plan, const char* name, void** ptr, long long* bytes);

#ifdef __cplusplus
}
#endif
#endif
```

Baseline: 2.388.

## Run 2x-upsample convolutions as four 2x2-tap phase convolutions on conv_wreg

A 3x3 convolution over a nearest-neighbour 2x upsampled image is rewritten as four sub-pixel phase convolutions. Each phase uses pre-summed 2x2-tap weights over the source image, so the kernel does 4 taps per channel chunk instead of 9. Packed phase weights, a phase-indexed weight stream, output-row remapping and GroupNorm slot indexing are added to the wreg kernel, gated by an option and a minimum-row threshold. This cuts the K-loop MFMA and weight traffic of the upsample convs. In exchange it adds a kernel variant, more weight storage, and a small fp16 rounding change from the summed weights.

```diff
diff --git a/blobctrl_amd/_lib.py b/blobctrl_amd/_lib.py
--- a/blobctrl_amd/_lib.py
+++ b/blobctrl_amd/_lib.py
@@ -39,6 +39,7 @@
         ("C_t", C.c_void_p), ("ldc_t", C.c_int), ("n_t0", C.c_int),
         ("w_bstride", C.c_longlong), ("vec_bstride", C.c_int), ("sm_group", C.c_int), ("sm_valid", C.c_int), ("sm_keep", C.c_int),
         ("S", C.c_void_p), ("S2", C.c_void_p), ("lds", C.c_int), ("lds2", C.c_int), ("S1", C.c_int), ("Cs", C.c_int),
+        ("ups_phase", C.c_int),
     ]
 
 
@@ -56,6 +57,8 @@
     "bc_conv_wreg_pack_sc": (C.c_int, [C.c_void_p, C.c_int, C.c_int, C.c_void_p, C.c_int, C.c_void_p, C.c_void_p]),
     "bc_conv_wreg_sc_eligible": (C.c_int, [C.c_int] * 7),
     "bc_conv_wreg_pack_host": (C.c_int, [C.c_void_p, C.c_int, C.c_int, C.c_void_p, C.c_int, C.c_void_p]),
+    "bc_conv_wreg_pack_ups": (C.c_int, [C.c_void_p, C.c_int, C.c_int, C.c_void_p, C.c_void_p]),
+    "bc_conv_wreg_pack_ups_host": (C.c_int, [C.c_void_p, C.c_int, C.c_int, C.c_void_p]),
     "bc_gemm_wreg_pack": (C.c_int, [C.c_void_p, C.c_int, C.c_int, C.c_int, C.c_int, C.c_void_p, C.c_void_p]),
     "bc_gemm_wreg_stream_elems": (C.c_longlong, [C.c_int, C.c_int]),
     "bc_gemm_wreg_eligible": (C.c_int, [C.c_int] * 5),
diff --git a/blobctrl_amd/csrc/conv_wreg.hip b/blobctrl_amd/csrc/conv_wreg.hip
--- a/blobctrl_amd/csrc/conv_wreg.hip
+++ b/blobctrl_amd/csrc/conv_wreg.hip
@@ -1,5 +1,6 @@
 #include <stdio.h>
 #include <stdlib.h>
+#include <string.h>
 #include <algorithm>
 #include <type_traits>
 #include <vector>
@@ -59,6 +60,7 @@
 
     asm volatile("" ::"s"(p.A), "s"(p.A2), "s"(p.W), "s"(p.Hv), "s"(p.Wv), "s"(p.Hin), "s"(p.Win), "s"(p.lda), "s"(p.lda2), "s"(p.C1), "s"(p.Cin),
                  "s"(p.splitk), "s"(p.a_act), "s"(g.halo_tpi), "s"(g.halo_tx), "s"(g.halo_nch), "s"(g.halo_nsc), "s"(g.halo_cps), "s"(g.halo_cps_sc), "s"(g.nband), "s"(g.halo_stamps));
+    if (AFFINE == 0) asm volatile("" ::"s"(p.ups_phase));
     asm volatile("" ::"s"(g.wr_plane.mul), "s"(g.wr_plane.shift), "s"(g.wr_plane.d), "s"(g.wr_gx.mul), "s"(g.wr_gx.shift), "s"(g.wr_gx.d), "s"(g.wr_gy.mul),
                  "s"(g.wr_gy.shift), "s"(g.wr_gy.d), "s"(g.wr_tpi.mul), "s"(g.wr_tpi.shift), "s"(g.wr_tx.mul), "s"(g.wr_tx.shift), "s"(p.bias), "s"(p.rowvec),
                  "s"(p.rowvec_idx), "s"(p.rowvec_step), "s"(p.ld_rowvec), "s"(g.halo_dbg), "s"(g.div_rpb.d));
@@ -70,14 +72,17 @@
     const int lin = lin3 - split * plane;
     const int q_gx = (int)fdiv((unsigned)lin, g.wr_gx), q_gy = (int)fdiv((unsigned)lin, g.wr_gy);
     const int tile = g.nband ? lin - q_gy * (int)g.wr_gy.d : q_gx;
-    const int ntile = g.nband ? q_gy : lin - q_gx * (int)g.wr_gx.d;
+    const int ntile_x = g.nband ? q_gy : lin - q_gx * (int)g.wr_gx.d;
+    const bool ph = AFFINE == 0 && p.ups_phase != 0;
+    const int pa = ph ? (ntile_x >> 1) & 1 : 0, pb = ph ? ntile_x & 1 : 0;
+    const int ntile = ph ? ntile_x >> 2 : ntile_x;
     const int n0 = ntile * HBN;
     const int b = (int)fdiv((unsigned)tile, g.wr_tpi);
     const int tin = tile - b * g.halo_tpi;
     const int ty_ = (int)fdiv((unsigned)tin, g.wr_tx);
     const int ty0 = ty_ * TH, tx0 = (tin - ty_ * g.halo_tx) * TW;
-    const int H = p.Hv, W = p.Wv;
-    const bool ups2 = p.Hv != p.Hin;
+    const int H = ph ? p.Hin : p.Hv, W = ph ? p.Win : p.Wv;
+    const bool ups2 = !ph && p.Hv != p.Hin;
     const int c_lo = split * g.halo_cps;
     const int n9 = max(0, min(g.halo_nch, c_lo + g.halo_cps) - c_lo);
     const int sc_begin = split * g.halo_cps_sc;
@@ -85,7 +90,7 @@
     const bool dummy = n9 == 0;
     const int c_begin = dummy ? 0 : c_lo;
     const int nch = dummy ? 1 : n9;
-    const long long tsl = (long long)(9 * g.halo_nch + g.halo_nsc) * 512;
+    const long long tsl = (long long)((ph ? 4 : 9) * g.halo_nch + g.halo_nsc) * 512;
 
     unsigned long long* const stamps = g.halo_stamps;
     auto stamp = [&](int i) {
@@ -183,19 +188,21 @@
     };
 
     float* tilef = reinterpret_cast<float*>(smem);
-    auto body = [&](auto ntc, auto stgc) {
+    auto body = [&](auto ntc, auto stgc, auto phc) {
         constexpr int NT = decltype(ntc)::value;
         constexpr bool STG = decltype(stgc)::value != 0;
-        constexpr int G = 3 * NT;
-        const long long per_chunk = 9 * 512;
-        u32x4v ring[3 * G];
+        constexpr bool PH = decltype(phc)::value != 0;
+        constexpr int NG = PH ? 2 : 3, NK = PH ? 2 : 3, NR = PH ? 9 : 10;
+        constexpr int G = NK * NT;
+        const long long per_chunk = NG * NK * 512;
+        u32x4v ring[NG * G];
         const unsigned lane16 = lane * 16;
 #define BC_WREG_LOAD_GROUP(GX, BASE)                                                                                                  \
     _Pragma("unroll") for (int f = 0; f < G; ++f) {                                                                                   \
         const h16* b4 = (BASE) + (((GX) * G + f) & ~3) * 512;                                                                          \
         asm volatile("global_load_dwordx4 %0, %1, %2 offset:%3" : "=v"(ring[(GX) * G + f]) : "v"(lane16), "s"(b4), "n"((((GX) * G + f) & 3) * 1024) : "memory"); \
     }
-        const h16* const wstream = reinterpret_cast<const h16*>(p.W) + ((long long)ntile * 20 + 2 * tile0 + kg * NT) * tsl;
+        const h16* const wstream = reinterpret_cast<const h16*>(p.W) + ((long long)((PH ? (2 * pa + pb) * ((int)g.wr_gx.d >> 2) : 0) + ntile) * 20 + 2 * tile0 + kg * NT) * tsl;
         const h16* wb = wstream + (long long)c_begin * NT * per_chunk;
         constexpr int FIN_T = 4;
         const int fin_cpg = AFFINE == 2 ? p.Cin / p.a_groups : 1;
@@ -383,9 +390,9 @@
             for (int i = tid; i < nch * 32; i += 512) dst[i] = src[i];
         }
         BC_WREG_LOAD_GROUP(1, wb)
-        BC_WREG_LOAD_GROUP(2, wb)
+        if constexpr (NG == 3) { BC_WREG_LOAD_GROUP(2, wb) }
         stamp(1);
-        asm volatile("s_waitcnt vmcnt(%0)" ::"n"(2 * G) : "memory");
+        asm volatile("s_waitcnt vmcnt(%0)" ::"n"((NG - 1) * G) : "memory");
         asm volatile("s_waitcnt lgkmcnt(0)" ::: "memory");
         __builtin_amdgcn_s_barrier();
         asm volatile("" ::: "memory");
@@ -405,9 +412,9 @@
         int a_off[3];
 #pragma unroll
         for (int kx = 0; kx < 3; ++kx) {
-            const int hx = (lane & 15) + kx;
+            const int hx = (lane & 15) + kx + (PH ? pb : 0);
             const int ch = 4 * kg + (lane >> 4);
-            a_off[kx] = hx * 128 + ((ch ^ (((hx >> 1) & 3) << 1)) << 4);
+            a_off[kx] = hx * 128 + ((ch ^ (((hx >> 1) & 3) << 1)) << 4) + (PH ? pa * (HSTR * 128) : 0);
         }
         f32x4v acc[8][NT];
 #pragma unroll
@@ -429,29 +436,30 @@
             const int buf1 = buf + 1 == NBUF ? 0 : buf + 1;
             const int buf2 = buf1 + 1 == NBUF ? 0 : buf1 + 1;
             if (STG) issue_a(cl + 2, buf2, cl + 2 < nch);
-            wb += 3 * G * 512;
-#pragma unroll
-            for (int kx = 0; kx < 3; ++kx) {
+            wb += NG * G * 512;
+#pragma unroll
+            for (int kx = 0; kx < NG; ++kx) {
 #define BC_WREG_WAIT(N)                                                                                                                 \
-    if (NT == 3) asm volatile("s_waitcnt vmcnt(%9)" : "+v"(ring[kx * G]), "+v"(ring[kx * G + 1]), "+v"(ring[kx * G + 2]), "+v"(ring[kx * G + 3]), \
+    if constexpr (G == 4) asm volatile("s_waitcnt vmcnt(%4)" : "+v"(ring[kx * G]), "+v"(ring[kx * G + 1]), "+v"(ring[kx * G + 2]), "+v"(ring[kx * G + G - 1]) : "n"(N) : "memory"); \
+    else if constexpr (G == 9) asm volatile("s_waitcnt vmcnt(%9)" : "+v"(ring[kx * G]), "+v"(ring[kx * G + 1]), "+v"(ring[kx * G + 2]), "+v"(ring[kx * G + 3]), \
                               "+v"(ring[kx * G + 4]), "+v"(ring[kx * G + 5]), "+v"(ring[kx * G + 6]), "+v"(ring[kx * G + 7]),             \
                               "+v"(ring[kx * G + G - 1]) : "n"(N) : "memory");                                                          \
     else asm volatile("s_waitcnt vmcnt(%6)" : "+v"(ring[kx * G]), "+v"(ring[kx * G + 1]), "+v"(ring[kx * G + 2]), "+v"(ring[kx * G + 3]),       \
                       "+v"(ring[kx * G + 4]), "+v"(ring[kx * G + G - 1]) : "n"(N) : "memory");
                 constexpr int D = STG ? 6 : 0;
-                if (more || kx == 0) { BC_WREG_WAIT(2 * G + D) }
-                else if (kx == 1) { BC_WREG_WAIT(G + D) }
-                else { BC_WREG_WAIT(D) }
+                if (more || kx == 0) { BC_WREG_WAIT((NG - 1) * G + D) }
+                else if (kx == NG - 1) { BC_WREG_WAIT(D) }
+                else { BC_WREG_WAIT(G + D) }
                 const unsigned abase = lds0 + buf * HALO_BYTES + a_off[kx];
                 u32x4v a[3];
                 asm volatile("ds_read_b128 %0, %1" : "=v"(a[0]) : "v"(abase) : "memory");
                 asm volatile("ds_read_b128 %0, %1 offset:%2" : "=v"(a[1]) : "v"(abase), "n"(HSTR * 128) : "memory");
 #pragma unroll
-                for (int r = 0; r < 10; ++r) {
-                    if (r + 2 < 10) {
+                for (int r = 0; r < NR; ++r) {
+                    if (r + 2 < NR) {
                         asm volatile("ds_read_b128 %0, %1 offset:%2" : "=v"(a[(r + 2) % 3]) : "v"(abase), "n"((r + 2) * HSTR * 128) : "memory");
                         asm volatile("s_waitcnt lgkmcnt(2)" : "+v"(a[r % 3])::"memory");
-                    } else if (r + 1 < 10) {
+                    } else if (r + 1 < NR) {
                         asm volatile("s_waitcnt lgkmcnt(1)" : "+v"(a[r % 3])::"memory");
                     } else {
                         asm volatile("s_waitcnt lgkmcnt(0)" : "+v"(a[r % 3])::"memory");
@@ -459,12 +467,12 @@
                     __builtin_amdgcn_sched_barrier(0);
                     const h16x8 af = __builtin_bit_cast(h16x8, a[r % 3]);
 #pragma unroll
-                    for (int ky = 0; ky < 3; ++ky) {
+                    for (int ky = 0; ky < NK; ++ky) {
                         const int i = r - ky;
                         if (i < 0 || i >= 8) continue;
 #pragma unroll
                         for (int t = 0; t < NT; ++t)
-                            acc[i][t] = __builtin_amdgcn_mfma_f32_16x16x32_f16(__builtin_bit_cast(h16x8, ring[(kx * 3 + ky) * NT + t]), af, acc[i][t], 0, 0, 0);
+                            acc[i][t] = __builtin_amdgcn_mfma_f32_16x16x32_f16(__builtin_bit_cast(h16x8, ring[(kx * NK + ky) * NT + t]), af, acc[i][t], 0, 0, 0);
                     }
                     __builtin_amdgcn_sched_barrier(0);
                 }
@@ -477,7 +485,7 @@
                 __builtin_amdgcn_sched_barrier(0);
             }
             if (STG) {
-                if (more) wait_vm_c<3 * G>();
+                if (more) wait_vm_c<NG * G>();
                 else wait_vm_c<0>();
             }
             asm volatile("s_waitcnt lgkmcnt(0)" ::: "memory");
@@ -488,7 +496,7 @@
         }
 
         stamp(14);
-        if (nsc > 0) {
+        if (!PH && nsc > 0) {
             constexpr int U = 4, NB2 = 5, D1 = STG ? 6 : 0;
             static_assert(NB2 * HALO_BYTES <= LDS_EPI && U < NB2 && U * 3 + 6 * U < 64, "shortcut phase: images below the epilogue vectors, vmcnt range");
             const h16* __restrict__ S1p = reinterpret_cast<const h16*>(p.S);
@@ -636,7 +644,8 @@
 #pragma unroll
             for (int j = 0; j < NP; ++j) {
                 const int row = j * RPP + rsub;
-                mrow[j] = b * rpb + (ty0 + i_keep + (row >> 4)) * W + tx0 + (row & 15);
+                const int oy = ty0 + i_keep + (row >> 4), ox = tx0 + (row & 15);
+                mrow[j] = PH ? b * rpb + (2 * oy + pa) * p.Wv + 2 * ox + pb : b * rpb + oy * W + ox;
                 if (HR) rr[j] = bc_ld16(reinterpret_cast<const h16*>(p.R) + (size_t)mrow[j] * p.ldr + n_first);
             }
             if (!H2) __builtin_amdgcn_sched_barrier(0);
@@ -731,15 +740,25 @@
             if (kg == 0 && owner) {
                 const float* sp = reinterpret_cast<const float*>(smem + (wave | 1) * 16384);
                 const int n_lo = n0 + tile0 * 16;
-                bc_gn_tot_add_slot(p.gn_tot + (size_t)b * g.n_out * BC_GN_TOT_WORDS, n_first + q_own, n_lo, n_lo + NT * 16, bc_gn_cg(g.n_out), tin, [&](int k) {
+                bc_gn_tot_add_slot(p.gn_tot + (size_t)b * g.n_out * BC_GN_TOT_WORDS, n_first + q_own, n_lo, n_lo + NT * 16, bc_gn_cg(g.n_out), PH ? 4 * tin + 2 * pa + pb : tin, [&](int k) {
                     const int c = k - n_lo;
                     return make_float2(sc[c * 2] + sp[c * 2], sc[c * 2 + 1] + sp[c * 2 + 1]);
                 });
             }
         }
     };
-    if (three) body(IC<3>{}, IC<0>{});
-    else body(IC<2>{}, IC<1>{});
+    if constexpr (AFFINE == 0) {
+        if (ph) {
+            if (three) body(IC<3>{}, IC<0>{}, IC<1>{});
+            else body(IC<2>{}, IC<1>{}, IC<1>{});
+        } else {
+            if (three) body(IC<3>{}, IC<0>{}, IC<0>{});
+            else body(IC<2>{}, IC<1>{}, IC<0>{});
+        }
+    } else {
+        if (three) body(IC<3>{}, IC<0>{}, IC<0>{});
+        else body(IC<2>{}, IC<1>{}, IC<0>{});
+    }
     stamp(4);
     if (p.splitk > 1) {
         const int col8 = tid % 20, row0 = tid / 20;
@@ -804,6 +823,104 @@
     *reinterpret_cast<uint4*>(out + idx * 8) = *reinterpret_cast<const uint4*>((sc ? wsc : w) + src);
 }
 
+
+__host__ __device__ inline void conv_wreg_ups_slot(long long idx, int N, int Cin, int& a, int& b, int& dy, int& dx, int& n, int& c0) {
+    const int nchunks = Cin / 64;
+    const long long per_tile_stream = (long long)nchunks * 4 * 64;
+    const long long per_ntile = 20 * per_tile_stream;
+    const long long per_phase = (long long)(N / HBN) * per_ntile;
+    const int phase = (int)(idx / per_phase);
+    a = phase >> 1;
+    b = phase & 1;
+    long long rem = idx - (long long)phase * per_phase;
+    const int ntile = (int)(rem / per_ntile);
+    rem -= (long long)ntile * per_ntile;
+    const int ts = (int)(rem / per_tile_stream);
+    int tile0, NT;
+    if (ts < 6) { tile0 = 0; NT = 3; }
+    else if (ts < 10) { tile0 = 3; NT = 2; }
+    else if (ts < 14) { tile0 = 5; NT = 2; }
+    else { tile0 = 7; NT = 3; }
+    const long long in_grp = rem - (long long)2 * tile0 * per_tile_stream;
+    const long long per_wave = per_tile_stream * NT;
+    const int kg = (int)(in_grp / per_wave);
+    long long s = in_grp - (long long)kg * per_wave;
+    const int lane = (int)(s & 63);
+    s >>= 6;
+    const int t = (int)(s % NT);
+    s /= NT;
+    dy = (int)(s & 1);
+    dx = (int)((s >> 1) & 1);
+    const int chunk = (int)(s >> 2);
+    n = ntile * HBN + (tile0 + t) * 16 + (lane & 15);
+    c0 = chunk * 64 + kg * 32 + 8 * (lane >> 4);
+}
+__host__ __device__ inline void conv_wreg_ups_taps(int bit, int d, int& lo, int& hi) {
+    lo = bit == 0 ? (d == 0 ? 0 : 1) : (d == 0 ? 0 : 2);
+    hi = bit == 0 ? (d == 0 ? 0 : 2) : (d == 0 ? 1 : 2);
+}
+inline float bc_h2f_host(unsigned short h) {
+    const unsigned sign = (unsigned)(h & 0x8000) << 16, e = (h >> 10) & 31, m = h & 1023;
+    unsigned u;
+    if (e == 0) {
+        if (m == 0) u = sign;
+        else {
+            int sh = 0;
+            unsigned mm = m;
+            while (!(mm & 1024)) { mm <<= 1; ++sh; }
+            u = sign | (unsigned)(113 - sh) << 23 | (mm & 1023) << 13;
+        }
+    } else if (e == 31) u = sign | 0x7f800000u | m << 13;
+    else u = sign | (e + 112) << 23 | m << 13;
+    float f;
+    memcpy(&f, &u, 4);
+    return f;
+}
+inline unsigned short bc_f2h_host(float f) {
+    unsigned u;
+    memcpy(&u, &f, 4);
+    const unsigned sign = (u >> 16) & 0x8000;
+    u &= 0x7fffffffu;
+    if (u >= 0x7f800000u) return (unsigned short)(sign | 0x7c00 | (u > 0x7f800000u ? 0x200 : 0));
+    if (u >= 0x477ff000u) return (unsigned short)(sign | 0x7c00);
+    if (u < 0x38800000u) {
+        if (u < 0x33000000u) return (unsigned short)sign;
+        const int e = (int)(u >> 23);
+        const unsigned sig = (u & 0x7fffffu) | 0x800000u;
+        const int sh = 126 - e;
+        const unsigned q = sig >> sh, r = sig & ((1u << sh) - 1), half = 1u << (sh - 1);
+        return (unsigned short)(sign | (q + (r > half || (r == half && (q & 1)))));
+    }
+    const unsigned q = (u - 0x38000000u) >> 13, r = u & 0x1fff;
+    return (unsigned short)(sign | (q + (r > 0x1000 || (r == 0x1000 && (q & 1)))));
+}
+
+__global__ void conv_wreg_pack_ups_kernel(const h16* __restrict__ w, int N, int Cin, h16* __restrict__ out) {
+    const long long total = (long long)N * 16 * Cin / 8;
+    const long long idx = (long long)blockIdx.x * blockDim.x + threadIdx.x;
+    if (idx >= total) return;
+    int a, b, dy, dx, n, c0, ky0, ky1, kx0, kx1;
+    conv_wreg_ups_slot(idx, N, Cin, a, b, dy, dx, n, c0);
+    conv_wreg_ups_taps(a, dy, ky0, ky1);
+    conv_wreg_ups_taps(b, dx, kx0, kx1);
+    float v[8];
+    for (int ky = ky0; ky <= ky1; ++ky) {
+        float rowsum[8];
+        for (int kx = kx0; kx <= kx1; ++kx) {
+            const uint4 raw = *reinterpret_cast<const uint4*>(w + (long long)n * 9 * Cin + (long long)(ky * 3 + kx) * Cin + c0);
+            const h16* x = reinterpret_cast<const h16*>(&raw);
+#pragma unroll
+            for (int e = 0; e < 8; ++e) rowsum[e] = kx == kx0 ? (float)x[e] : rowsum[e] + (float)x[e];
+        }
+#pragma unroll
+        for (int e = 0; e < 8; ++e) v[e] = ky == ky0 ? rowsum[e] : v[e] + rowsum[e];
+    }
+    uint4 o;
+    h16* oh = reinterpret_cast<h16*>(&o);
+#pragma unroll
+    for (int e = 0; e < 8; ++e) oh[e] = (h16)v[e];
+    *reinterpret_cast<uint4*>(out + idx * 8) = o;
+}
 }
 
 extern "C" int bc_conv_wreg_pack_sc(const bc_half* w, int N, int Cin, const bc_half* wsc, int Cs, bc_half* out, bc_stream stream_) {
@@ -834,6 +951,43 @@
     return 0;
 }
 
+extern "C" int bc_conv_wreg_pack_ups(const bc_half* w, int N, int Cin, bc_half* out, bc_stream stream_) {
+    hipStream_t stream = reinterpret_cast<hipStream_t>(stream_);
+    BC_CHECK_ARG(w && out && N > 0 && N % HBN == 0 && Cin > 0 && Cin % 64 == 0, "bc_conv_wreg_pack_ups: N %% 160 == 0 and Cin %% 64 == 0 (N=%d Cin=%d)", N, Cin);
+    BC_CHECK_ARG(((uintptr_t)w % 16 == 0) && ((uintptr_t)out % 16 == 0) && w != out, "bc_conv_wreg_pack_ups: 16-byte aligned, out of place");
+    const long long total = (long long)N * 16 * Cin / 8;
+    hipLaunchKernelGGL(conv_wreg_pack_ups_kernel, dim3((unsigned)((total + 255) / 256)), dim3(256), 0, stream, reinterpret_cast<const h16*>(w), N, Cin,
+                       reinterpret_cast<h16*>(out));
+    BC_CHECK_LAUNCH();
+    return 0;
+}
+
+extern "C" int bc_conv_wreg_pack_ups_host(const bc_half* w, int N, int Cin, bc_half* out) {
+    BC_CHECK_ARG(w && out && N > 0 && N % HBN == 0 && Cin > 0 && Cin % 64 == 0, "bc_conv_wreg_pack_ups: N %% 160 == 0 and Cin %% 64 == 0 (N=%d Cin=%d)", N, Cin);
+    const long long total = (long long)N * 16 * Cin / 8;
+    const unsigned short* w_ = reinterpret_cast<const unsigned short*>(w);
+    unsigned short* o_ = reinterpret_cast<unsigned short*>(out);
+    for (long long idx = 0; idx < total; ++idx) {
+        int a, b, dy, dx, n, c0, ky0, ky1, kx0, kx1;
+        conv_wreg_ups_slot(idx, N, Cin, a, b, dy, dx, n, c0);
+        conv_wreg_ups_taps(a, dy, ky0, ky1);
+        conv_wreg_ups_taps(b, dx, kx0, kx1);
+        for (int e = 0; e < 8; ++e) {
+            float v = 0.f;
+            for (int ky = ky0; ky <= ky1; ++ky) {
+                float rowsum = 0.f;
+                for (int kx = kx0; kx <= kx1; ++kx) {
+                    const float x = bc_h2f_host(w_[(long long)n * 9 * Cin + (long long)(ky * 3 + kx) * Cin + c0 + e]);
+                    rowsum = kx == kx0 ? x : rowsum + x;
+                }
+                v = ky == ky0 ? rowsum : v + rowsum;
+            }
+            o_[idx * 8 + e] = bc_f2h_host(v);
+        }
+    }
+    return 0;
+}
+
 extern "C" int bc_conv_wreg_pack(const bc_half* w, int N, int Cin, bc_half* out, bc_stream stream) {
     return bc_conv_wreg_pack_sc(w, N, Cin, nullptr, 0, out, stream);
 }
@@ -848,8 +1002,15 @@
 
 int bc_conv_wreg_launch(GemmArgs& g, hipStream_t stream) {
     BcGemm& p = g.p;
-    g.halo_tx = p.Wout / TW;
-    g.halo_tpi = g.halo_tx * (p.Hout / TH);
+    const bool ph = p.ups_phase != 0;
+    if (ph) {
+        BC_CHECK_ARG(p.Hv == 2 * p.Hin && p.Wv == 2 * p.Win && p.Hout == p.Hv && p.Wout == p.Wv && p.Win % TW == 0 && p.Hin % TH == 0,
+                     "bc_gemm(wreg conv): ups_phase needs an exact 2x upsample of a source of whole 8 x 16 tiles (%dx%d -> %dx%d)", p.Hin, p.Win, p.Hv, p.Wv);
+        BC_CHECK_ARG(!p.a_affine && !p.a_tot1 && !p.A2 && !p.S, "bc_gemm(wreg conv): ups_phase takes a plain single-source convolution");
+        BC_CHECK_ARG(p.splitk <= 1, "bc_gemm(wreg conv): the phase form of an upsample convolution runs unsplit (splitk=%d)", p.splitk);
+    }
+    g.halo_tx = (ph ? p.Win : p.Wout) / TW;
+    g.halo_tpi = g.halo_tx * ((ph ? p.Hin : p.Hout) / TH);
     g.halo_nch = p.Cin / 64;
     g.halo_nsc = p.S ? p.Cs / 64 : 0;
     g.halo_dbg = 0;
@@ -861,11 +1022,12 @@
     BC_CHECK_ARG(g.halo_cps <= MAX_CH, "bc_gemm(wreg conv): %d channel chunks per split exceed %d (raise splitk)", g.halo_cps, MAX_CH);
     BC_CHECK_ARG(p.splitk == 1 || p.slab != nullptr, "bc_gemm(wreg conv): splitk=%d needs a slab", p.splitk);
     const int B = p.M / (p.Hout * p.Wout);
+    BC_CHECK_ARG(!ph || p.splitk == 1, "bc_gemm(wreg conv): the phase form of an upsample convolution runs unsplit (splitk=%d)", p.splitk);
     BC_CHECK_ARG((long long)p.M * std::max(p.lda, p.lda2) < 2147483647LL, "bc_gemm(wreg conv): activation of %d pixels x stride %d exceeds 32-bit element offsets",
                  p.M, std::max(p.lda, p.lda2));
     BC_CHECK_ARG(!p.S || (bc_conv_wreg_sc_ok(p) && (long long)p.M * std::max(p.lds, p.lds2) < 2147483647LL),
                  "bc_gemm(wreg conv): folded shortcut outside the kernel's limits (Cs=%d S1=%d)", p.Cs, p.S1);
-    dim3 grid(p.N / HBN, B * g.halo_tpi, p.splitk);
+    dim3 grid((ph ? 4 : 1) * (p.N / HBN), B * g.halo_tpi, p.splitk);
     g.wr_plane = make_fastdiv(grid.x * grid.y);
     g.wr_gx = make_fastdiv(grid.x);
     g.wr_gy = make_fastdiv(grid.y);
@@ -873,7 +1035,7 @@
     g.wr_tx = make_fastdiv((unsigned)g.halo_tx);
     g.wr_cpg = make_fastdiv((unsigned)(p.a_tot1 && p.a_groups > 0 ? p.Cin / p.a_groups : 1));
     {
-        g.nband = (double)p.N * 9 > (double)p.M && grid.x >= 4;
+        g.nband = (double)p.N * 9 > (double)p.M && p.N / HBN >= 4;
     }
     static const bool want_stamps = getenv("BC_WREG_STAMPS") != nullptr;
     static unsigned long long* stamp_buf = nullptr;
@@ -914,7 +1076,7 @@
                 if (p.S) fprintf(stderr, "[wreg stamps] folded shortcut: Cs=%d, %.0f ticks per workgroup behind the nine-tap chunks (of the loop's %.0f)\n", p.Cs, scp / n, d[2] / n);
                 fprintf(stderr, "[wreg stamps] M=%d N=%d Cin=%d sk=%d cps=%d wgs=%zu %s | avg ticks: setup+table %.0f, first halo %.0f (landing %.0f, pass %.0f, "
                         "next DMA + barrier %.0f), loop %.0f (%.0f per tap), k-half sum %.0f, stores %.0f\n", p.M, p.N, p.Cin, p.splitk, cps, n,
-                        w ? "staging wave " : "3-tile wave  ", d[0] / n, d[1] / n, e[0] / n, e[1] / n, e[2] / n, d[2] / n, d[2] / n / (cps * 9), d[3] / n, d[4] / n);
+                        p.ups_phase ? (w ? "staging wave, phase form " : "3-tile wave, phase form  ") : w ? "staging wave " : "3-tile wave  ", d[0] / n, d[1] / n, e[0] / n, e[1] / n, e[2] / n, d[2] / n, d[2] / n / (cps * (p.ups_phase ? 4 : 9)), d[3] / n, d[4] / n);
             }
         }
     } report{stream, nwg_s, g.halo_stamps, p, g.halo_cps};
diff --git a/blobctrl_amd/engine.py b/blobctrl_amd/engine.py
--- a/blobctrl_amd/engine.py
+++ b/blobctrl_amd/engine.py
@@ -98,7 +98,12 @@
                 Wv % 16 == 0 and Hv % 8 == 0 and opt("wreg")
             if ups_wreg:
                 kw.update(tile_cfg=_lib.TILE_WREG, lda=x.C)
-                wkey = pw.wreg(wname + ".weight")
+                if opt("ups_phase") and M >= opt("ups_phase_min_rows") and x.H % 8 == 0 and x.W % 16 == 0 and \
+                        rec.conv_splitk(M, Cout, Cin, _lib.TILE_WREG) == 1:
+                    kw.update(ups_phase=True)
+                    wkey = pw.wreg_ups(wname + ".weight")
+                else:
+                    wkey = pw.wreg(wname + ".weight")
             elif tile_cfg:
                 kw.update(tile_cfg=tile_cfg)
         rec.gemm(A=x.t, W=pw.h[wkey], M=M, N=Cout, K=9 * Cin, out=out,
diff --git a/blobctrl_amd/launch.py b/blobctrl_amd/launch.py
--- a/blobctrl_amd/launch.py
+++ b/blobctrl_amd/launch.py
@@ -320,12 +320,20 @@
                    "bc_gemm_plan")
         return c.value, s_.value, bm.value, bn.value
 
+    def conv_splitk(self, M, N, Cin, tile_cfg):
+        nch, base = Cin // 64, (M // 128) * (N // 160)
+        target = opt("halo_ctas") or (128 if tile_cfg == _lib.TILE_WREG else 256)
+        min_cps = opt("halo_min_cps") or (3 if tile_cfg == _lib.TILE_WREG else 2)
+        full = opt("halo_full") or target * 2 // 3
+        short = tile_cfg == _lib.TILE_WREG and base >= target // 2 and nch <= 5
+        return 1 if (base >= full or short) else max(1, min(nch // min_cps, -(-target // base)))
+
     def gemm(self, *, A, W, M, N, K, out=None, out_mode=_lib.OUT_F16, ldc=None, A2=None, C1=0, lda=None, lda2=0,
              conv=None, bias=None, rowvec=None, ld_rowvec=0, rowvec_idx=None, rowvec_step=0, rows_per_batch=0, act=_lib.ACT_NONE, colscale=None,
              alpha=1.0, alpha_dev=None, alpha_idx=None, alpha_bstride=0, R=None, ldr=0, R2=None, ldr2=0, r2_xmin=0, r2_bmod=1,
              out_w=0, splitk=None, kind="gemm", a_offset=0, w_offset=0, out_offset=0, want_gn=False, tile_cfg=0, ldw=None,
              a_affine=None, a_act=_lib.ACT_NONE, a_gn=None, ln_colsum=None, ln_eps=1e-5, C_t=None, ldc_t=0, n_t0=0,
-             w_bstride=0, vec_bstride=0, sm_group=0, sm_valid=0, sm_keep=0, gn_tot_out=None, S=None, S2=None, lds=0, lds2=0, S1=0, Cs=0):
+             w_bstride=0, vec_bstride=0, sm_group=0, sm_valid=0, sm_keep=0, gn_tot_out=None, S=None, S2=None, lds=0, lds2=0, S1=0, Cs=0, ups_phase=False):
         n_out = N // 2 if act == _lib.ACT_GEGLU else (N // sm_group * sm_keep if sm_group else N)
         g = BcGemm()
         g.A = A.data_ptr() + a_offset * A.element_size()
@@ -387,11 +395,7 @@
             base = (M // 128) * (N // 160)
             explicit_sk, sk_req = splitk, None
             if splitk is None:
-                target = opt("halo_ctas") or (128 if tile_cfg == _lib.TILE_WREG else 256)
-                min_cps = opt("halo_min_cps") or (3 if tile_cfg == _lib.TILE_WREG else 2)
-                full = opt("halo_full") or target * 2 // 3
-                short = tile_cfg == _lib.TILE_WREG and base >= target // 2 and nch <= 5
-                splitk = 1 if (base >= full or short) else max(1, min(nch // min_cps, -(-target // base)))
+                splitk = self.conv_splitk(M, N, conv["Cin"], tile_cfg)
             splitk = max(splitk, -(-nch // self.lib.bc_conv_halo_max_chunks()))
             cps = -(-nch // max(1, splitk))
             cfg, sk, bm, bn = tile_cfg, -(-nch // cps), 128, 160
@@ -402,7 +406,13 @@
                 cps = -(-nch // s2)
                 sk = max(-(-nch // cps), -(-nsc // -(-nsc // s2)))
             fast, mode = True, "halo"
-            sc_mode = "_sc" if S is not None else ""
+            if ups_phase:
+                if tile_cfg != _lib.TILE_WREG or sk > 1 or S is not None or A2 is not None or a_affine is not None or a_gn is not None or \
+                        (conv.get("Hv"), conv.get("Wv")) != (2 * conv["Hin"], 2 * conv["Win"]) or conv["Hin"] % 8 or conv["Win"] % 16:
+                    raise _lib.BlobCtrlHipError(f"bc_gemm({kind}): the phase form of an upsample convolution needs an unsplit plain BC_TILE_WREG launch "
+                                                f"over an exact 2x upsample of whole 8 x 16 source tiles (splitk={sk})")
+                g.ups_phase = 1
+            sc_mode = "_sc" if S is not None else "_ph" if ups_phase else ""
             if a_gn is not None:
                 G_ = a_gn["G"]
                 span = cps * 64 + 2 * (conv["Cin"] // G_)
@@ -483,7 +493,8 @@
             rp = "gemm_kernel<" + ("256, 64, 4, 1" if bn == 64 else "128, 128, 2, 2") + ">"
         a_elems = (M // (conv["Hout"] * conv["Wout"])) * conv["Hin"] * conv["Win"] * conv["Cin"] if conv else M * K
         alg_bytes = 2 * (a_elems + N * K + M * n_out) + (2 * M * n_out if R is not None else 0) + 2 * (M + N) * Cs
-        self._push(kind, 2 * M * N * (K + Cs), variant, (mode, M, N, K + Cs, sk), alg_bytes, rp)
+        k_exec = K * 4 // 9 if ups_phase else K
+        self._push(kind, 2 * M * N * (k_exec + Cs), variant, (mode, M, N, K + Cs, sk), alg_bytes, rp)
         return out
 
     def _op(self, name, args, kind, **meta):
diff --git a/blobctrl_amd/options.py b/blobctrl_amd/options.py
--- a/blobctrl_amd/options.py
+++ b/blobctrl_amd/options.py
@@ -12,6 +12,7 @@
     "cfg_prefix": (True, "CFG-invariant prefix of the UNet once per image pair (0: every launch at the full CFG batch)"),
     "wreg": (True, "ResBlock convolutions on csrc/conv_wreg.hip (0: csrc/conv_halo.hip)"),
     "sc_fold": (True, "a ResBlock's 1x1 shortcut folded into conv2's K loop on csrc/conv_wreg.hip (0: a conv1x1 launch + residual read)"),
+    "ups_phase": (True, "aligned 2x-upsample convolutions as four 2x2-tap phase convolutions on csrc/conv_wreg.hip (0: nine taps over the virtual image)"),
     "halo": (True, "ResBlock convolutions with the fused GroupNorm prologue at all (0: GroupNorm pass + implicit GEMM)"),
     "gn_finalize_launch": (False, "a bc_gn_finalize launch per GroupNorm instead of the finalize in the consumer's prologue"),
     "halo_ctas": (0, "workgroups a split-K convolution pass aims for (0: 128 on conv_wreg, 256 on conv_halo)"),
@@ -26,6 +27,7 @@
     "ctx_fold_maxb": (2, "largest UNet batch that takes the prompt-folded cross-attention"),
     "gn_pass_min_requests": (4, "edit requests per batch from which a ResBlock convolution runs as GroupNorm pass + plain conv_wreg (0: never)"),
     "gn_pass_min_cin": (320, "... and fewest input channels of such a convolution"),
+    "ups_phase_min_rows": (2048, "fewest output rows M of an unsplit upsample convolution that takes the phase form (every unsplit level of the step: DESIGN 9)"),
     "g256_min_tiles": (64, "fewest 256 x 256 tiles for gemm256.hip (a quarter of the CUs: the other queue has the rest)"),
 }
 
diff --git a/blobctrl_amd/weights.py b/blobctrl_amd/weights.py
--- a/blobctrl_amd/weights.py
+++ b/blobctrl_amd/weights.py
@@ -61,6 +61,57 @@
     return torch.cat(parts).reshape(N, K + Cs)
 
 
+UPS_TAPS = (((0,), (1, 2)), ((0, 1), (2,)))
+
+
+def ups_phase_weights(w: torch.Tensor) -> torch.Tensor:
+    N, K = w.shape
+    Cin = K // 9
+    v = w.reshape(N, 3, 3, Cin)
+    out = torch.empty(4, N, 2, 2, Cin, dtype=w.dtype, device=w.device)
+    for a in range(2):
+        for b in range(2):
+            for dy in range(2):
+                for dx in range(2):
+                    rows = []
+                    for ky in UPS_TAPS[a][dy]:
+                        kxs = UPS_TAPS[b][dx]
+                        r = v[:, ky, kxs[0]]
+                        rows.append(r if len(kxs) == 1 else r + v[:, ky, kxs[1]])
+                    out[2 * a + b, :, dy, dx] = rows[0] if len(rows) == 1 else rows[0] + rows[1]
+    return out.reshape(4, N, 4 * Cin)
+
+
+def pack_conv_wreg_ups(w: torch.Tensor) -> torch.Tensor:
+    N, K = w.shape
+    Cin = K // 9
+    assert w.dtype == torch.float16 and N % 160 == 0 and Cin % 64 == 0 and K == 9 * Cin, (w.dtype, N, K)
+    wp = ups_phase_weights(w.float()).half()
+    nch = Cin // 64
+    parts = []
+    for ph in range(4):
+        v = wp[ph].reshape(N // 160, 10, 16, 2, 2, nch, 2, 4, 8)
+        for blk in range(N // 160):
+            for t0, nt in WREG_TILES:
+                parts.append(v[blk, t0:t0 + nt].permute(5, 4, 3, 2, 0, 6, 1, 7).reshape(-1))
+    return torch.cat(parts).reshape(4, N, 4 * Cin)
+
+
+def unpack_conv_wreg_ups(s: torch.Tensor) -> torch.Tensor:
+    _, N, K4 = s.shape
+    nch = K4 // 4 // 64
+    flat, off = s.reshape(-1), 0
+    out = torch.empty(4, N // 160, 10, 16, 2, 2, nch, 2, 4, 8, dtype=s.dtype, device=s.device)
+    for ph in range(4):
+        for blk in range(N // 160):
+            for t0, nt in WREG_TILES:
+                n = nt * 16 * 4 * nch * 64
+                g = flat[off:off + n].reshape(2, nch, 2, 2, nt, 4, 16, 8)
+                out[ph, blk, t0:t0 + nt] = g.permute(4, 6, 3, 2, 1, 0, 5, 7)
+                off += n
+    return out.reshape(4, N, K4)
+
+
 def pack_matrix(w: torch.Tensor) -> torch.Tensor:
     w = w.reshape(w.shape[0], -1)
     co, ci = w.shape
@@ -154,6 +205,12 @@
         k2 = key + "_wreg"
         if k2 not in self.h:
             self.h[k2] = pack_conv_wreg(self.h[key])
+        return k2
+
+    def wreg_ups(self, key: str) -> str:
+        k2 = key + "_wreg_ups"
+        if k2 not in self.h:
+            self.h[k2] = pack_conv_wreg_ups(self.h[key])
         return k2
 
     def wreg_sc(self, conv: str, sc: str):
diff --git a/include/blobctrl_hip.h b/include/blobctrl_hip.h
--- a/include/blobctrl_hip.h
+++ b/include/blobctrl_hip.h
@@ -68,6 +68,7 @@
     int sm_group, sm_valid, sm_keep;
     const bc_half* S; const bc_half* S2;
     int lds, lds2, S1, Cs;
+    int ups_phase;
 } BcGemm;
 
 int bc_gemm(const BcGemm* p, bc_stream stream);
@@ -85,6 +86,8 @@
 int bc_conv_wreg_pack(const bc_half* w, int N, int Cin, bc_half* out, bc_stream stream);
 int bc_conv_wreg_pack_sc(const bc_half* w, int N, int Cin, const bc_half* wsc, int Cs, bc_half* out, bc_stream stream);
 int bc_conv_wreg_pack_host(const bc_half* w, int N, int Cin, const bc_half* wsc, int Cs, bc_half* out);
+int bc_conv_wreg_pack_ups(const bc_half* w, int N, int Cin, bc_half* out, bc_stream stream);
+int bc_conv_wreg_pack_ups_host(const bc_half* w, int N, int Cin, bc_half* out);
 int bc_conv_wreg_sc_eligible(int Cin, int N, int H, int W, int Cs, int S1, int reserved);
 int bc_conv_halo_eligible(int Cin, int C1, int N, int Hin, int Win, int Hout, int Wout, int stride);
 int bc_conv_halo_max_chunks(void);
```

Measured after the change: 2.400, median of 6. About the same (+0.5%).
